# blackle/Megalania

Hardware: NVIDIA B200
Metric: neighbour_cost_evals_per_sec (higher is better)
Workload: dtype u16 probabilities / u64 cost (integer)

## Files before the change

### include/megalania_cuda.h

```cpp
#ifndef MEGALANIA_CUDA_H
#define MEGALANIA_CUDA_H

#include <stddef.h>
#include <stdint.h>

#include "output_interface.h"

#if defined(__GNUC__)
#define MG_API __attribute__((visibility("default")))
#else
#define MG_API
#endif

#ifdef __cplusplus
extern "C" {
#endif


#ifndef MG_HAVE_LZMA_PACKET
#define MG_HAVE_LZMA_PACKET
#define INVALID 0
#define LITERAL 1
#define MATCH 2
#define SHORT_REP 3
// ... 34 lines not shown


MG_API int mg_ctx_create(const uint8_t* data, size_t n, LZMAProperties props, int device, mg_ctx** out);
MG_API void mg_ctx_destroy(mg_ctx* ctx);
MG_API size_t mg_ctx_size(const mg_ctx* ctx);
MG_API int mg_ctx_device(const mg_ctx* ctx);
MG_API int mg_ctx_set_finder_limits(mg_ctx* ctx, size_t window, uint32_t max_occurrences);
MG_API uint32_t mg_ctx_full_wave(const mg_ctx* ctx);
MG_API uint32_t mg_ctx_sm_clock_khz(const mg_ctx* ctx);


MG_API int mg_score_slabs(mg_ctx* ctx, const LZMAPacket* slabs, size_t nslabs, uint64_t* out_cost);


MG_API int mg_find_topk(mg_ctx* ctx, const LZMAPacket* slab, int state_mode, const uint64_t* positions,
                 size_t npos, int k, LZMAPacket* out_pops, uint32_t* out_prices, int32_t* out_counts);

MG_API int mg_find_topk_stats(const mg_ctx* ctx, double* kernel_ms, uint64_t* candidates);


MG_API int mg_encode_slab(mg_ctx* ctx, const LZMAPacket* slab, OutputInterface* out);
MG_API int mg_encode_slab_buffer(mg_ctx* ctx, const LZMAPacket* slab, uint8_t* out, size_t cap, size_t* out_len);
MG_API int mg_encode_stats(const mg_ctx* ctx, double* kernel_ms, uint64_t* events);


MG_API int mg_decode_stream(mg_ctx* ctx, const uint8_t* stream, size_t len, LZMAPacket* out_slab);
MG_API int mg_decode_stats(const mg_ctx* ctx, double* kernel_ms, uint64_t* events);


enum {
	MG_SCHEDULE_REFERENCE = 0,
	MG_SCHEDULE_TEMPERATURE = 1
};

typedef struct {
	uint32_t chains;
	uint32_t top_k;
	uint32_t checkpoint_stride;
	uint32_t edit_log_capacity;
	uint32_t track_best;
	uint32_t trace_capacity;
	uint64_t seed;
} mg_anneal_params;

typedef struct {
	uint32_t evals;
	uint32_t max_attempts;
	uint32_t schedule;
	uint32_t step;
	uint32_t num_iters;
	uint32_t first_eval;
	const float* temperatures;
	uint64_t packet_budget;
	uint32_t no_early_exit;
	uint32_t suspend;
	uint64_t cycle_budget;
	const uint32_t* regions;
} mg_anneal_run_params;
#define MG_CONTINUE_EVALS 0xffffffffu

typedef struct {
	uint64_t evals;
	uint64_t attempts;
	uint64_t accepted;
	uint64_t new_best;
	uint64_t packets_scored;
	uint64_t bits_scored;
	uint64_t slab_bytes_read;
	uint64_t checkpoint_bytes;
	uint64_t finder_calls;
	uint64_t finder_candidates;
	uint64_t edits;
	uint64_t log_overflows;
	uint64_t rejoined;
	uint64_t finder_cycles;
	uint64_t chain_cycles;
	uint64_t finder_chunks;
	uint64_t max_chain_cycles;
	uint64_t finder_gave_up;
	double kernel_ms;
	uint32_t launches;
} mg_anneal_stats;

typedef struct {
	uint64_t cost;
	uint32_t flags;
	uint32_t undo_count;
} mg_trace_rec;

MG_API int mg_anneal_create(mg_ctx* ctx, const mg_anneal_params* params, mg_anneal** out);
MG_API void mg_anneal_destroy(mg_anneal* an);
MG_API size_t mg_anneal_chain_bytes(const mg_ctx* ctx, const mg_anneal_params* params);

MG_API int mg_anneal_set_slab(mg_anneal* an, uint32_t first, uint32_t count, const LZMAPacket* slab,
                       int adopt_cost, int reset_best);

MG_API int mg_anneal_greedy_init(mg_anneal* an, uint32_t nregions, uint32_t dst_chain, uint64_t* cost_out);

MG_API int mg_anneal_optimal_init(mg_anneal* an, uint32_t nregions, uint32_t max_occ, uint32_t dst_chain,
                                  uint64_t* cost_out);
MG_API int mg_optimal_stats(const mg_ctx* ctx, double* kernel_ms, uint64_t* nodes);

MG_API int mg_anneal_merge_regions(mg_anneal* an, uint32_t nregions, const uint32_t* bounds, const uint32_t* owners,
                                   uint32_t dst_chain, uint64_t* cost_out);
#define MG_NO_OWNER 0xffffffffu
MG_API int mg_anneal_merge_export(mg_anneal* an, uint32_t nregions, const uint32_t* bounds, const uint32_t* owners,
                                  void* dev_slab, void* dev_abs);
MG_API int mg_anneal_merge_import(mg_anneal* an, const void* dev_slab, const void* dev_abs, uint32_t dst_chain,
                                  uint64_t* cost_out);
MG_API int mg_anneal_broadcast_chain(mg_anneal* an, uint32_t src_chain);

MG_API int mg_anneal_run(mg_anneal* an, const mg_anneal_run_params* run, mg_anneal_stats* stats);

MG_API int mg_anneal_costs(mg_anneal* an, uint64_t* cur_cost, uint64_t* best_cost);
MG_API int mg_anneal_get_slab(mg_anneal* an, uint32_t chain, int which, LZMAPacket* out_slab);
MG_API int mg_anneal_get_trace(mg_anneal* an, uint32_t chain, mg_trace_rec* out, size_t cap, size_t* count);
MG_API int mg_anneal_swap_chains(mg_anneal* an, uint32_t a, uint32_t b);
MG_API int mg_anneal_device_slab(mg_anneal* an, uint32_t chain, int which, void** dev_ptr, size_t* bytes);
MG_API int mg_anneal_export_slab(mg_anneal* an, uint32_t chain, int which, void* dev_dst);
MG_API int mg_anneal_import_slab(mg_anneal* an, uint32_t chain, const void* dev_src, int adopt_cost);
MG_API int mg_anneal_refresh_chain(mg_anneal* an, uint32_t chain, int adopt_cost);

MG_API int mg_anneal_oneshot(mg_ctx* ctx, const mg_anneal_params* params, const mg_anneal_run_params* run,
                      const LZMAPacket* init, LZMAPacket* best_slab_out, uint64_t* best_cost,
                      mg_anneal_stats* stats);


#define MG_COMM_ID_BYTES 128
MG_API int mg_comm_unique_id(void* id_out);
MG_API int mg_comm_init(mg_ctx* ctx, int rank, int nranks, const void* nccl_id);
MG_API void mg_comm_destroy(mg_ctx* ctx);
MG_API int mg_comm_rank(const mg_ctx* ctx);
MG_API int mg_comm_size(const mg_ctx* ctx);
MG_API int mg_comm_exchange_best(mg_anneal* an, int* winner_rank, uint64_t* best_cost, uint32_t* chain_out);
MG_API int mg_comm_temper_exchange(mg_anneal* an, float* temps, uint32_t round_index, uint64_t seed);
MG_API int mg_temper_decide(const uint64_t* costs, const float* temps, size_t count, uint32_t round_index,
                            uint64_t seed, float* out_temps);
MG_API int mg_comm_merge_regions(mg_anneal* an, uint32_t nregions, const uint32_t* bounds, const uint32_t* owners,
                                 uint32_t dst_chain, uint64_t* cost_out);
MG_API int mg_comm_broadcast_chain(mg_anneal* an, int root, uint32_t src_chain, uint32_t dst_chain);
MG_API int mg_comm_allgather_u64(mg_ctx* ctx, uint64_t value, uint64_t* out);
MG_API int mg_comm_stats(const mg_ctx* ctx, uint64_t* exchanges, uint64_t* installs_by_copy, uint64_t* installs_by_rescore);


typedef struct {
	uint16_t probs[2615];
	uint8_t ctx_state;
	uint32_t dists[4];
	uint64_t position;
	uint64_t cost;
} mg_model_dump;
MG_API int mg_debug_model_after_prefix(mg_ctx* ctx, const LZMAPacket* slab, size_t stop, mg_model_dump* out);
MG_API int mg_debug_index(mg_ctx* ctx, uint32_t* occ_start, uint32_t* occ);

#ifdef __cplusplus
}
#endif
#endif
```

### megalania_b200/api.py

```python
from __future__ import annotations

import ctypes as C
import os

import numpy as np

from . import build as _build

PACKET_DTYPE = np.dtype({"names": ["type", "dist", "len"], "formats": ["u1", "<u4", "<u2"],
                         "offsets": [0, 4, 8], "itemsize": 12})
TRACE_DTYPE = np.dtype([("cost", "<u8"), ("flags", "<u4"), ("undo_count", "<u4")])
MODEL_DTYPE = np.dtype({"names": ["probs", "ctx_state", "dists", "position", "cost"],
                        "formats": [("<u2", 2615), "u1", ("<u4", 4), "<u8", "<u8"],
                        "offsets": [0, 5230, 5232, 5248, 5256], "itemsize": 5264})
INVALID, LITERAL, MATCH, SHORT_REP, LONG_REP = 0, 1, 2, 3, 4
SCHEDULE_REFERENCE, SCHEDULE_TEMPERATURE = 0, 1
CONTINUE_EVALS = 0xFFFFFFFF
NO_OWNER = 0xFFFFFFFF

ERRORS = {-1: "MG_EINVAL", -2: "MG_ECUDA", -3: "MG_ENOMEM", -4: "MG_ESLAB", -5: "MG_EOUTPUT", -6: "MG_ESTATE"}


class MegalaniaError(RuntimeError):
    def __init__(self, code: int, message: str):
        super().__init__(f"{ERRORS.get(code, code)}: {message}")
        self.code = code


class LZMAProperties(C.Structure):
    _fields_ = [("lc", C.c_uint8), ("lp", C.c_uint8), ("pb", C.c_uint8)]


class AnnealParams(C.Structure):
    _fields_ = [("chains", C.c_uint32), ("top_k", C.c_uint32), ("checkpoint_stride", C.c_uint32),
                ("edit_log_capacity", C.c_uint32), ("track_best", C.c_uint32), ("trace_capacity", C.c_uint32),
                ("seed", C.c_uint64)]


class AnnealRunParams(C.Structure):
    _fields_ = [("evals", C.c_uint32), ("max_attempts", C.c_uint32), ("schedule", C.c_uint32),
                ("step", C.c_uint32), ("num_iters", C.c_uint32), ("first_eval", C.c_uint32),
                ("temperatures", C.POINTER(C.c_float)), ("packet_budget", C.c_uint64), ("no_early_exit", C.c_uint32),
                ("suspend", C.c_uint32), ("cycle_budget", C.c_uint64), ("regions", C.POINTER(C.c_uint32))]


class AnnealStats(C.Structure):
    _fields_ = [(name, C.c_uint64) for name in (
        "evals", "attempts", "accepted", "new_best", "packets_scored", "bits_scored", "slab_bytes_read",
        "checkpoint_bytes", "finder_calls", "finder_candidates", "edits", "log_overflows", "rejoined", "finder_cycles", "chain_cycles",
        "finder_chunks", "max_chain_cycles", "finder_gave_up")] + [
        ("kernel_ms", C.c_double), ("launches", C.c_uint32)]

    def as_dict(self) -> dict:
        return {name: getattr(self, name) for name, _ in self._fields_}


WRITE_FN = C.CFUNCTYPE(C.c_bool, C.c_void_p, C.c_void_p, C.c_size_t)


class OutputInterface(C.Structure):
    _fields_ = [("write", WRITE_FN), ("private_data", C.c_void_p)]


EXPORTS = [
    "mg_last_error", "mg_version", "mg_ctx_create", "mg_ctx_destroy", "mg_ctx_size", "mg_ctx_device",
    "mg_score_slabs", "mg_find_topk", "mg_encode_slab", "mg_encode_slab_buffer", "mg_anneal_create",
    "mg_anneal_destroy", "mg_anneal_chain_bytes", "mg_anneal_set_slab", "mg_anneal_run", "mg_anneal_costs",
    "mg_anneal_get_slab", "mg_anneal_get_trace", "mg_anneal_swap_chains", "mg_anneal_device_slab",
    "mg_anneal_refresh_chain", "mg_anneal_oneshot", "mg_debug_model_after_prefix", "mg_anneal_export_slab",
    "mg_anneal_import_slab", "mg_anneal_merge_regions", "mg_anneal_broadcast_chain", "mg_find_topk_stats",
    "mg_anneal_merge_export", "mg_anneal_merge_import", "mg_debug_index", "mg_encode_stats", "mg_ctx_full_wave", "mg_ctx_sm_clock_khz",
    "mg_comm_unique_id", "mg_comm_init", "mg_comm_destroy", "mg_comm_rank", "mg_comm_size", "mg_comm_exchange_best",
    "mg_comm_temper_exchange", "mg_temper_decide", "mg_comm_merge_regions", "mg_comm_stats", "mg_pool_trim",
    "mg_comm_broadcast_chain", "mg_comm_allgather_u64", "mg_ctx_set_finder_limits", "mg_anneal_greedy_init",
    "mg_decode_stream", "mg_decode_stats", "mg_anneal_optimal_init", "mg_optimal_stats",
]

_lib = None


def library_path() -> str:
    return os.environ.get("MEGALANIA_CUDA_LIB") or _build.LIB


def load_library(build_if_missing: bool = True) -> C.CDLL:
    global _lib
    if _lib is not None:
        return _lib
    path = library_path()
    if not os.path.exists(path):
        if not build_if_missing:
            raise MegalaniaError(-2, f"{path} is missing: run `python -m megalania_b200.build`")
        _build.build_library()
    L = C.CDLL(path)
    vp, sz, u32, u64, i32 = C.c_void_p, C.c_size_t, C.c_uint32, C.c_uint64, C.c_int
    L.mg_last_error.restype = C.c_char_p
    L.mg_version.restype = u32
    L.mg_ctx_create.argtypes = [vp, sz, LZMAProperties, i32, C.POINTER(vp)]
    L.mg_ctx_destroy.argtypes = [vp]
    L.mg_ctx_destroy.restype = None
    L.mg_ctx_size.argtypes = [vp]
    L.mg_ctx_size.restype = sz
    L.mg_ctx_device.argtypes = [vp]
    L.mg_ctx_set_finder_limits.argtypes = [vp, sz, u32]
    L.mg_ctx_full_wave.argtypes = [vp]
    L.mg_ctx_full_wave.restype = u32
    L.mg_ctx_sm_clock_khz.argtypes = [vp]
    L.mg_ctx_sm_clock_khz.restype = u32
    L.mg_score_slabs.argtypes = [vp, vp, sz, vp]
    L.mg_find_topk.argtypes = [vp, vp, i32, vp, sz, i32, vp, vp, vp]
    L.mg_find_topk_stats.argtypes = [vp, C.POINTER(C.c_double), C.POINTER(u64)]
    L.mg_encode_slab.argtypes = [vp, vp, C.POINTER(OutputInterface)]
    L.mg_encode_slab_buffer.argtypes = [vp, vp, vp, sz, C.POINTER(sz)]
    L.mg_anneal_create.argtypes = [vp, C.POINTER(AnnealParams), C.POINTER(vp)]
    L.mg_anneal_destroy.argtypes = [vp]
    L.mg_anneal_destroy.restype = None
    L.mg_anneal_chain_bytes.argtypes = [vp, C.POINTER(AnnealParams)]
    L.mg_anneal_chain_bytes.restype = sz
    L.mg_anneal_set_slab.argtypes = [vp, u32, u32, vp, i32, i32]
    L.mg_anneal_run.argtypes = [vp, C.POINTER(AnnealRunParams), C.POINTER(AnnealStats)]
    L.mg_anneal_costs.argtypes = [vp, vp, vp]
    L.mg_anneal_get_slab.argtypes = [vp, u32, i32, vp]
    L.mg_anneal_get_trace.argtypes = [vp, u32, vp, sz, C.POINTER(sz)]
    L.mg_anneal_swap_chains.argtypes = [vp, u32, u32]
    L.mg_anneal_device_slab.argtypes = [vp, u32, i32, C.POINTER(vp), C.POINTER(sz)]
    L.mg_anneal_refresh_chain.argtypes = [vp, u32, i32]
    L.mg_anneal_merge_regions.argtypes = [vp, u32, vp, vp, u32, C.POINTER(u64)]
    L.mg_anneal_broadcast_chain.argtypes = [vp, u32]
    L.mg_anneal_greedy_init.argtypes = [vp, u32, u32, C.POINTER(u64)]
    L.mg_anneal_merge_export.argtypes = [vp, u32, vp, vp, vp, vp]
    L.mg_anneal_merge_import.argtypes = [vp, vp, vp, u32, C.POINTER(u64)]
    L.mg_anneal_export_slab.argtypes = [vp, u32, i32, vp]
    L.mg_anneal_import_slab.argtypes = [vp, u32, vp, i32]
    L.mg_anneal_oneshot.argtypes = [vp, C.POINTER(AnnealParams), C.POINTER(AnnealRunParams), vp, vp,
                                    C.POINTER(u64), C.POINTER(AnnealStats)]
    L.mg_debug_model_after_prefix.argtypes = [vp, vp, sz, vp]
    L.mg_debug_index.argtypes = [vp, vp, vp]
    L.mg_pool_trim.restype = None
    L.mg_comm_unique_id.argtypes = [vp]
    L.mg_comm_init.argtypes = [vp, i32, i32, vp]
    L.mg_comm_destroy.argtypes = [vp]
    L.mg_comm_destroy.restype = None
    L.mg_comm_rank.argtypes = [vp]
    L.mg_comm_size.argtypes = [vp]
    L.mg_comm_exchange_best.argtypes = [vp, C.POINTER(i32), C.POINTER(u64), C.POINTER(u32)]
    L.mg_comm_temper_exchange.argtypes = [vp, vp, u32, u64]
    L.mg_temper_decide.argtypes = [vp, vp, sz, u32, u64, vp]
    L.mg_comm_merge_regions.argtypes = [vp, u32, vp, vp, u32, C.POINTER(u64)]
    L.mg_comm_stats.argtypes = [vp, C.POINTER(u64), C.POINTER(u64), C.POINTER(u64)]
    L.mg_comm_broadcast_chain.argtypes = [vp, i32, u32, u32]
    L.mg_comm_allgather_u64.argtypes = [vp, u64, vp]
    L.mg_encode_stats.argtypes = [vp, C.POINTER(C.c_double), C.POINTER(u64)]
    L.mg_decode_stream.argtypes = [vp, vp, sz, vp]
    L.mg_decode_stats.argtypes = [vp, C.POINTER(C.c_double), C.POINTER(u64)]
    L.mg_anneal_optimal_init.argtypes = [vp, u32, u32, u32, C.POINTER(u64)]
    L.mg_optimal_stats.argtypes = [vp, C.POINTER(C.c_double), C.POINTER(u64)]
    _lib = L
    return L


def _check(rc: int) -> None:
    if rc != 0:
        raise MegalaniaError(rc, load_library().mg_last_error().decode(errors="replace"))


def literal_slab(n: int) -> np.ndarray:
    slab = np.zeros(n, dtype=PACKET_DTYPE)
    slab["type"] = LITERAL
    slab["len"] = 1
    return slab


def as_slab(slab: np.ndarray) -> np.ndarray:
    if slab.dtype == PACKET_DTYPE and slab.flags["C_CONTIGUOUS"]:
        return slab
    out = np.zeros(slab.shape, dtype=PACKET_DTYPE)
    for name in ("type", "dist", "len"):
        out[name] = slab[name]
    return out


def _slab_ptr(slab: np.ndarray, n: int, count: int = 1):
    if slab.dtype != PACKET_DTYPE or not slab.flags["C_CONTIGUOUS"] or slab.size != n * count:
        raise ValueError(f"slab must be a contiguous PACKET_DTYPE array of {n * count} packets")
    return slab.ctypes.data_as(C.c_void_p)


class Context:

    def __init__(self, data: bytes, device: int = 0):
        self._lib = load_library()
        self._data = np.ascontiguousarray(np.frombuffer(bytes(data), dtype=np.uint8))
        self.n = int(self._data.size)
        self._h = C.c_void_p()
        self._children = []
        _check(self._lib.mg_ctx_create(self._data.ctypes.data_as(C.c_void_p), self.n, LZMAProperties(0, 0, 0),
                                       device, C.byref(self._h)))

    def close(self) -> None:
        if getattr(self, "_h", None):
            for ref in self._children:
                child = ref()
                if child is not None:
                    child.close()
            self._children = []
            self._lib.mg_ctx_destroy(self._h)
            self._h = None

    def __del__(self):
        try:
            self.close()
        except Exception:
            pass

    def __enter__(self):
        return self

    def __exit__(self, *exc):
        self.close()

    def score_slabs(self, slabs: np.ndarray) -> np.ndarray:
        slabs = as_slab(np.asarray(slabs))
        count = slabs.size // self.n
        out = np.zeros(count, dtype=np.uint64)
        _check(self._lib.mg_score_slabs(self._h, _slab_ptr(slabs.reshape(-1), self.n, count), count,
                                        out.ctypes.data_as(C.c_void_p)))
        return out

    def score_slab(self, slab: np.ndarray) -> int:
        return int(self.score_slabs(slab)[0])

    def find_topk(self, slab: np.ndarray, positions, state_mode: int = 0, k: int = 20):
        pos = np.ascontiguousarray(positions, dtype=np.uint64)
        slab = as_slab(slab)
        pops = np.zeros((pos.size, k), dtype=PACKET_DTYPE)
        prices = np.zeros((pos.size, k), dtype=np.uint32)
        counts = np.zeros(pos.size, dtype=np.int32)
        _check(self._lib.mg_find_topk(self._h, _slab_ptr(slab, self.n), state_mode, pos.ctypes.data_as(C.c_void_p),
                                      pos.size, k, pops.ctypes.data_as(C.c_void_p),
                                      prices.ctypes.data_as(C.c_void_p), counts.ctypes.data_as(C.c_void_p)))
        return pops, prices, counts

    def find_topk_stats(self) -> dict:
        ms, cand = C.c_double(0), C.c_uint64(0)
        _check(self._lib.mg_find_topk_stats(self._h, C.byref(ms), C.byref(cand)))
        return {"kernel_ms": ms.value, "candidates": int(cand.value)}

    def encode_slab(self, slab: np.ndarray) -> bytes:
        chunks: list[bytes] = []

        def _write(_iface, ptr, size):
            chunks.append(C.string_at(ptr, size))
            return True

        iface = OutputInterface(WRITE_FN(_write), None)
        _check(self._lib.mg_encode_slab(self._h, _slab_ptr(slab, self.n), C.byref(iface)))
        return b"".join(chunks)

    def encode_stats(self) -> dict:
        ms, ev = C.c_double(0), C.c_uint64(0)
        _check(self._lib.mg_encode_stats(self._h, C.byref(ms), C.byref(ev)))
        return {"kernel_ms": ms.value, "events": int(ev.value)}

    def encode_slab_buffer(self, slab: np.ndarray) -> bytes:
        cap = self.n * 2 + 8192
        out = np.zeros(cap, dtype=np.uint8)
        got = C.c_size_t(0)
        _check(self._lib.mg_encode_slab_buffer(self._h, _slab_ptr(slab, self.n), out.ctypes.data_as(C.c_void_p), cap,
                                               C.byref(got)))
        return out[:got.value].tobytes()

    def decode_stream(self, stream: bytes) -> np.ndarray:
        buf = np.ascontiguousarray(np.frombuffer(bytes(stream), dtype=np.uint8))
        out = np.zeros(self.n, dtype=PACKET_DTYPE)
        _check(self._lib.mg_decode_stream(self._h, buf.ctypes.data_as(C.c_void_p), buf.size,
                                          out.ctypes.data_as(C.c_void_p)))
        return out

    def decode_stats(self) -> dict:
        ms, ev = C.c_double(0), C.c_uint64(0)
        _check(self._lib.mg_decode_stats(self._h, C.byref(ms), C.byref(ev)))
        return {"kernel_ms": ms.value, "events": int(ev.value)}

    def optimal_stats(self) -> dict:
        ms, nodes = C.c_double(0), C.c_uint64(0)
        _check(self._lib.mg_optimal_stats(self._h, C.byref(ms), C.byref(nodes)))
        return {"kernel_ms": ms.value, "nodes": int(nodes.value)}

    def model_after_prefix(self, slab: np.ndarray, stop: int):
        out = np.zeros(1, dtype=MODEL_DTYPE)
        _check(self._lib.mg_debug_model_after_prefix(self._h, _slab_ptr(slab, self.n), stop,
                                                     out.ctypes.data_as(C.c_void_p)))
        return out[0]

    @staticmethod
    def comm_unique_id() -> bytes:
        buf = C.create_string_buffer(128)
        _check(load_library().mg_comm_unique_id(buf))
        return buf.raw

    def comm_init(self, rank: int, nranks: int, unique_id: bytes) -> None:
        if len(unique_id) != 128:
            raise ValueError("an NCCL unique id is 128 bytes")
        _check(self._lib.mg_comm_init(self._h, rank, nranks, C.c_char_p(unique_id)))

    def comm_allgather(self, value: int) -> np.ndarray:
        size = int(self._lib.mg_comm_size(self._h))
        out = np.zeros(size, dtype=np.uint64)
        _check(self._lib.mg_comm_allgather_u64(self._h, int(value), out.ctypes.data_as(C.c_void_p)))
        return out

    def comm_stats(self) -> dict:
        a, b, c = C.c_uint64(0), C.c_uint64(0), C.c_uint64(0)
        _check(self._lib.mg_comm_stats(self._h, C.byref(a), C.byref(b), C.byref(c)))
        return {"exchanges": int(a.value), "installs_by_copy": int(b.value), "installs_by_rescore": int(c.value)}

    def set_finder_limits(self, window: int = 0, max_occurrences: int = 0) -> None:
        _check(self._lib.mg_ctx_set_finder_limits(self._h, window, max_occurrences))

    def full_wave(self) -> int:
        return int(self._lib.mg_ctx_full_wave(self._h))

    def sm_clock_khz(self) -> int:
        return int(self._lib.mg_ctx_sm_clock_khz(self._h))

    def bigram_index(self):
        start = np.zeros(65537, dtype=np.uint32)
        occ = np.zeros(max(1, self.n - 1), dtype=np.uint32)
        _check(self._lib.mg_debug_index(self._h, start.ctypes.data_as(C.c_void_p), occ.ctypes.data_as(C.c_void_p)))
        return start, occ[:max(0, self.n - 1)]

    def chain_bytes(self, **params) -> int:
        p = AnnealParams(**params)
        return int(self._lib.mg_anneal_chain_bytes(self._h, C.byref(p)))


class Annealer:

    def __init__(self, ctx: Context, chains: int, *, top_k: int = 20, checkpoint_stride: int = 0,
                 edit_log_capacity: int = 0, track_best: bool = True, trace_capacity: int = 0, seed: int = 1673551):
        self.ctx = ctx
        self._lib = ctx._lib
        self.chains = chains
        self.params = AnnealParams(chains, top_k, checkpoint_stride, edit_log_capacity, int(track_best),
                                   trace_capacity, seed)
        self._h = C.c_void_p()
        _check(self._lib.mg_anneal_create(ctx._h, C.byref(self.params), C.byref(self._h)))
        import weakref
        ctx._children.append(weakref.ref(self))

    def close(self) -> None:
        if getattr(self, "_h", None):
            self._lib.mg_anneal_destroy(self._h)
            self._h = None

    def __del__(self):
        try:
            self.close()
        except Exception:
            pass

    def set_slab(self, slab: np.ndarray | None = None, first: int = 0, count: int | None = None,
                 adopt_cost: bool | None = None, reset_best: bool = True) -> None:
        if count is None:
            count = self.chains - first
        if adopt_cost is None:
            adopt_cost = slab is not None
        ptr = _slab_ptr(slab, self.ctx.n) if slab is not None else None
        _check(self._lib.mg_anneal_set_slab(self._h, first, count, ptr, int(adopt_cost), int(reset_best)))

    def run(self, evals: int, *, schedule: int = SCHEDULE_REFERENCE, step: int = 0, num_iters: int = 0,
            first_eval: int = 0, max_attempts: int = 0, temperatures=None, packet_budget: int = 0,
            early_exit: bool = True, suspend: bool = False, cycle_budget: int = 0, regions=None) -> dict:
        temps = None
        tptr = None
        if temperatures is not None:
            temps = np.ascontiguousarray(temperatures, dtype=np.float32)
            if temps.size != self.chains:
                raise ValueError("one temperature per chain")
            tptr = temps.ctypes.data_as(C.POINTER(C.c_float))
        rptr = None
        if regions is not None:
            regs = np.ascontiguousarray(regions, dtype=np.uint32)
            if regs.shape != (self.chains, 2):
                raise ValueError("regions must be a [chains][2] array of byte ranges")
            rptr = regs.ctypes.data_as(C.POINTER(C.c_uint32))
        rp = AnnealRunParams(evals, max_attempts, schedule, step, num_iters, first_eval, tptr, packet_budget,
                             0 if early_exit else 1, int(suspend), cycle_budget, rptr)
        st = AnnealStats()
        _check(self._lib.mg_anneal_run(self._h, C.byref(rp), C.byref(st)))
        return st.as_dict()

    def costs(self):
        cur = np.zeros(self.chains, dtype=np.uint64)
        best = np.zeros(self.chains, dtype=np.uint64)
        _check(self._lib.mg_anneal_costs(self._h, cur.ctypes.data_as(C.c_void_p), best.ctypes.data_as(C.c_void_p)))
        return cur, best

    def get_slab(self, chain: int, best: bool = False) -> np.ndarray:
        out = np.zeros(self.ctx.n, dtype=PACKET_DTYPE)
        _check(self._lib.mg_anneal_get_slab(self._h, chain, int(best), out.ctypes.data_as(C.c_void_p)))
        return out

    def trace(self, chain: int) -> np.ndarray:
        cap = self.params.trace_capacity
        out = np.zeros(cap, dtype=TRACE_DTYPE)
        count = C.c_size_t(0)
        _check(self._lib.mg_anneal_get_trace(self._h, chain, out.ctypes.data_as(C.c_void_p), cap, C.byref(count)))
        return out[:min(cap, count.value)]

    def swap_chains(self, a: int, b: int) -> None:
        _check(self._lib.mg_anneal_swap_chains(self._h, a, b))

    def device_slab(self, chain: int, best: bool = False):
        ptr, size = C.c_void_p(), C.c_size_t()
        _check(self._lib.mg_anneal_device_slab(self._h, chain, int(best), C.byref(ptr), C.byref(size)))
        return ptr.value, size.value

    def export_slab(self, chain: int, best: bool, device_ptr: int) -> None:
        _check(self._lib.mg_anneal_export_slab(self._h, chain, int(best), C.c_void_p(device_ptr)))

    def import_slab(self, chain: int, device_ptr: int, adopt_cost: bool = True) -> None:
        _check(self._lib.mg_anneal_import_slab(self._h, chain, C.c_void_p(device_ptr), int(adopt_cost)))

    def merge_regions(self, bounds, owners, dst_chain: int = 0) -> int:
        b = np.ascontiguousarray(bounds, dtype=np.uint32)
        o = np.ascontiguousarray(owners, dtype=np.uint32)
        if b.size != o.size + 1:
            raise ValueError("bounds must hold one more entry than owners")
        cost = C.c_uint64(0)
        _check(self._lib.mg_anneal_merge_regions(self._h, o.size, b.ctypes.data_as(C.c_void_p), o.ctypes.data_as(C.c_void_p),
                                                 dst_chain, C.byref(cost)))
        return int(cost.value)

    def merge_export(self, bounds, owners, dev_slab_ptr: int, dev_abs_ptr: int) -> None:
        b = np.ascontiguousarray(bounds, dtype=np.uint32)
        o = np.ascontiguousarray(owners, dtype=np.uint32)
        if b.size != o.size + 1:
            raise ValueError("bounds must hold one more entry than owners")
        _check(self._lib.mg_anneal_merge_export(self._h, o.size, b.ctypes.data_as(C.c_void_p), o.ctypes.data_as(C.c_void_p),
                                                C.c_void_p(dev_slab_ptr), C.c_void_p(dev_abs_ptr)))

    def merge_import(self, dev_slab_ptr: int, dev_abs_ptr: int, dst_chain: int = 0) -> int:
        cost = C.c_uint64(0)
        _check(self._lib.mg_anneal_merge_import(self._h, C.c_void_p(dev_slab_ptr), C.c_void_p(dev_abs_ptr), dst_chain,
                                                C.byref(cost)))
        return int(cost.value)

    def comm_exchange_best(self):
        w, c, ch = C.c_int(-1), C.c_uint64(0), C.c_uint32(0)
        _check(self._lib.mg_comm_exchange_best(self._h, C.byref(w), C.byref(c), C.byref(ch)))
        return int(w.value), int(c.value), int(ch.value)

    def comm_broadcast_chain(self, root: int, src_chain: int, dst_chain: int) -> None:
        _check(self._lib.mg_comm_broadcast_chain(self._h, root, src_chain, dst_chain))

    def comm_temper_exchange(self, temps: np.ndarray, round_index: int, seed: int = 0) -> np.ndarray:
        t = np.ascontiguousarray(temps, dtype=np.float32).copy()
        if t.size != self.chains:
            raise ValueError("one temperature per chain")
        _check(self._lib.mg_comm_temper_exchange(self._h, t.ctypes.data_as(C.c_void_p), round_index, seed))
        return t

    def comm_merge_regions(self, bounds, owners, dst_chain: int = 0) -> int:
        b = np.ascontiguousarray(bounds, dtype=np.uint32)
        o = np.ascontiguousarray(owners, dtype=np.uint32)
        cost = C.c_uint64(0)
        _check(self._lib.mg_comm_merge_regions(self._h, o.size, b.ctypes.data_as(C.c_void_p), o.ctypes.data_as(C.c_void_p),
                                               dst_chain, C.byref(cost)))
        return int(cost.value)

    def broadcast_chain(self, src_chain: int) -> None:
        _check(self._lib.mg_anneal_broadcast_chain(self._h, src_chain))

    def greedy_init(self, nregions: int = 1, dst_chain: int = 0) -> int:
        cost = C.c_uint64(0)
        _check(self._lib.mg_anneal_greedy_init(self._h, nregions, dst_chain, C.byref(cost)))
        return int(cost.value)

    def optimal_init(self, nregions: int = 1, max_occ: int = 0, dst_chain: int = 0) -> int:
        cost = C.c_uint64(0)
        _check(self._lib.mg_anneal_optimal_init(self._h, nregions, max_occ, dst_chain, C.byref(cost)))
        return int(cost.value)

# ... 27 lines not shown
```

### megalania_b200/csrc/mg_api.cu

```cuda
#include <cmath>
#include <cstdarg>
#include <cstdio>
#include <cstdlib>
#include <cstring>
#include <algorithm>
#include <new>
#include <vector>
#include <unistd.h>

#include "../../include/megalania_cuda.h"
#include "mg_kernels.cuh"

using namespace mg;

static thread_local char g_err[512] = "";

static int fail(int code, const char* fmt, ...)
{
	va_list ap;
	va_start(ap, fmt);
	vsnprintf(g_err, sizeof(g_err), fmt, ap);
	va_end(ap);
	return code;
}

#define CU(call)                                                                                   \
	do {                                                                                           \
		cudaError_t e_ = (call);                                                                   \
		if (e_ != cudaSuccess)                                                                     \
			return fail(e_ == cudaErrorMemoryAllocation ? MG_ENOMEM : MG_ECUDA, "%s: %s", #call,   \
			            cudaGetErrorString(e_));                                                   \
	} while (0)

extern "C" MG_API const char* mg_last_error(void) { return g_err; }
#include <map>
#include <mutex>
#include <unordered_map>
namespace {
struct DevicePool {
	std::mutex lock;
	std::unordered_map<void*, std::pair<int, size_t>> live;
	std::multimap<std::pair<int, size_t>, void*> cached;
};
DevicePool& pool()
{
	static DevicePool* p = new DevicePool;
	return *p;
}
void pool_release_device(int device)
{
	DevicePool& P = pool();
	for (auto it = P.cached.begin(); it != P.cached.end();) {
		if (device < 0 || it->first.first == device) {
			cudaFree(it->second);
			it = P.cached.erase(it);
		} else {
			++it;
		}
	}
}
}

static cudaError_t pool_malloc_raw(void** out, size_t bytes)
{
	if (bytes == 0) bytes = 16;
	int device = 0;
	cudaError_t e = cudaGetDevice(&device);
	if (e != cudaSuccess) return e;
	DevicePool& P = pool();
	std::lock_guard<std::mutex> g(P.lock);
	auto hit = P.cached.find({device, bytes});
	if (hit != P.cached.end()) {
		*out = hit->second;
		P.cached.erase(hit);
	} else {
		e = cudaMalloc(out, bytes);
		if (e == cudaErrorMemoryAllocation) {
			cudaGetLastError();
			pool_release_device(device);
			e = cudaMalloc(out, bytes);
		}
		if (e != cudaSuccess) return e;
	}
	P.live[*out] = {device, bytes};
	return cudaSuccess;
}
template <class T> static cudaError_t pool_malloc(T** out, size_t bytes) { return pool_malloc_raw(reinterpret_cast<void**>(out), bytes); }

static void pool_free(void* p)
{
	if (!p) return;
	DevicePool& P = pool();
	std::lock_guard<std::mutex> g(P.lock);
	auto it = P.live.find(p);
	if (it == P.live.end()) {
		cudaFree(p);
		return;
	}
	P.cached.insert({it->second, p});
	P.live.erase(it);
}

extern "C" MG_API void mg_pool_trim(void)
{
	DevicePool& P = pool();
	std::lock_guard<std::mutex> g(P.lock);
	int device = 0;
	cudaGetDevice(&device);
	for (auto it = P.cached.begin(); it != P.cached.end();) {
		cudaSetDevice(it->first.first);
		cudaFree(it->second);
		it = P.cached.erase(it);
	}
	cudaSetDevice(device);
}

extern "C" MG_API uint32_t mg_version(void) { return (0u << 16) | 3u; }

struct mg_comm_state;

struct mg_ctx {
	mg_comm_state* comm = nullptr;
	int device = 0;
	uint32_t n = 0;
	cudaStream_t stream = nullptr;
	uint8_t* d_data = nullptr;
	uint32_t* d_occ_start = nullptr;
	uint32_t* d_occ = nullptr;
	uint32_t* d_trans = nullptr;
	uint32_t* d_recip = nullptr;
	uint4* d_litq = nullptr;
	Tables tables{};
	int sm_count = 0;
	double index_ms = 0;
	std::vector<mg_anneal*> annealers;
	double last_topk_ms = 0;
	unsigned long long last_topk_candidates = 0;
	FindLimits limits{0, 0};
	double last_encode_ms = 0;
	unsigned long long last_encode_events = 0;
	double last_decode_ms = 0;
	unsigned long long last_decode_events = 0;
	double last_optimal_ms = 0;
	unsigned long long last_optimal_nodes = 0;
};

struct DevBuf {
	void* p = nullptr;
	~DevBuf() { if (p) pool_free(p); }
	template <class T> T* as() { return static_cast<T*>(p); }
};

static int dev_alloc(DevBuf& b, size_t bytes)
{
	CU(pool_malloc(&b.p, bytes ? bytes : 16));
	return 0;
}

static int grid_for(size_t items, int threads, int cap)
{
	size_t g = (items + threads - 1) / threads;
	if (g > (size_t)cap) g = cap;
	return g ? (int)g : 1;
}

static int set_smem_attrs()
{
	CU(cudaFuncSetAttribute(score_kernel, cudaFuncAttributeMaxDynamicSharedMemorySize, (int)sizeof(CtaShared)));
	CU(cudaFuncSetAttribute(topk_kernel, cudaFuncAttributeMaxDynamicSharedMemorySize, (int)sizeof(CtaShared)));
	CU(cudaFuncSetAttribute(anneal_kernel, cudaFuncAttributeMaxDynamicSharedMemorySize, (int)sizeof(CtaShared)));
	CU(cudaFuncSetAttribute(greedy_kernel, cudaFuncAttributeMaxDynamicSharedMemorySize, (int)sizeof(CtaShared)));
	CU(cudaFuncSetAttribute(encode_kernel, cudaFuncAttributeMaxDynamicSharedMemorySize, (int)sizeof(EncodeShared)));
	CU(cudaFuncSetAttribute(score_kernel, cudaFuncAttributePreferredSharedMemoryCarveout, cudaSharedmemCarveoutMaxShared));
	CU(cudaFuncSetAttribute(topk_kernel, cudaFuncAttributePreferredSharedMemoryCarveout, cudaSharedmemCarveoutMaxShared));
	CU(cudaFuncSetAttribute(anneal_kernel, cudaFuncAttributePreferredSharedMemoryCarveout, cudaSharedmemCarveoutMaxShared));
	CU(cudaFuncSetAttribute(greedy_kernel, cudaFuncAttributePreferredSharedMemoryCarveout, cudaSharedmemCarveoutMaxShared));
	return 0;
}

static int build_index(mg_ctx* ctx)
{
	const uint32_t n = ctx->n;
	CU(pool_malloc(&ctx->d_occ_start, sizeof(uint32_t) * (INDEX_KEYS + 1)));
	CU(pool_malloc(&ctx->d_occ, sizeof(uint32_t) * (size_t)(n ? n : 1)));
	if (n < 2) {
		CU(cudaMemsetAsync(ctx->d_occ_start, 0, sizeof(uint32_t) * (INDEX_KEYS + 1), ctx->stream));
		return 0;
	}
	const uint32_t total = n - 1;
	uint32_t nwarps = 256;
	uint32_t per_warp = (total + nwarps - 1) / nwarps;
	per_warp = (per_warp + 31) & ~31u;
	if (per_warp < 32) per_warp = 32;
	nwarps = (total + per_warp - 1) / per_warp;
	DevBuf rows, totals;
	if (int rc = dev_alloc(rows, sizeof(uint32_t) * (size_t)nwarps * INDEX_KEYS)) return rc;
	if (int rc = dev_alloc(totals, sizeof(uint32_t) * INDEX_KEYS)) return rc;
	cudaEvent_t e0, e1;
	CU(cudaEventCreate(&e0));
	CU(cudaEventCreate(&e1));
	CU(cudaEventRecord(e0, ctx->stream));
	CU(cudaMemsetAsync(rows.p, 0, sizeof(uint32_t) * (size_t)nwarps * INDEX_KEYS, ctx->stream));
	const int threads = 128;
	const int blocks = (int)((nwarps * 32 + threads - 1) / threads);
	index_count_kernel<<<blocks, threads, 0, ctx->stream>>>(ctx->d_data, n, rows.as<uint32_t>(), per_warp);
	index_prefix_kernel<<<INDEX_KEYS / 256, 256, 0, ctx->stream>>>(rows.as<uint32_t>(), nwarps, totals.as<uint32_t>());
	index_scan_kernel<<<1, 1024, 0, ctx->stream>>>(totals.as<uint32_t>(), ctx->d_occ_start);
	index_scatter_kernel<<<blocks, threads, 0, ctx->stream>>>(ctx->d_data, n, rows.as<uint32_t>(), per_warp,
	                                                          ctx->d_occ_start, ctx->d_occ);
	CU(cudaEventRecord(e1, ctx->stream));
	CU(cudaStreamSynchronize(ctx->stream));
	CU(cudaGetLastError());
	float ms = 0;
	cudaEventElapsedTime(&ms, e0, e1);
	ctx->index_ms = ms;
	cudaEventDestroy(e0);
	cudaEventDestroy(e1);
	return 0;
}

extern "C" MG_API int mg_ctx_create(const uint8_t* data, size_t n, LZMAProperties props, int device, mg_ctx** out)
{
	if (!data || !out || n == 0) return fail(MG_EINVAL, "mg_ctx_create: data, out and a non-zero size are required");
	if (props.lc || props.lp || props.pb) return fail(MG_EINVAL, "only lc = lp = pb = 0 is supported (as in the reference)");
	if (n >= 0x7fffff00ull) return fail(MG_EINVAL, "inputs of 2 GiB and more are not supported");
	int count = 0;
	cudaError_t probe = cudaErrorUnknown;
	for (int attempt = 0; attempt < 5; attempt++) {
		probe = cudaGetDeviceCount(&count);
		if (probe == cudaSuccess && count > 0) break;
		if (probe == cudaErrorNoDevice || probe == cudaErrorInsufficientDriver) break;
		cudaGetLastError();
		usleep(200 * 1000);
	}
	if (probe != cudaSuccess || count == 0)
		return fail(MG_ECUDA, "no CUDA device available (this library has no CPU path): %s", cudaGetErrorString(probe));
	if (device < 0 || device >= count) return fail(MG_EINVAL, "device %d out of range (%d devices)", device, count);
	CU(cudaSetDevice(device));
	mg_ctx* ctx = new (std::nothrow) mg_ctx;
	if (!ctx) return fail(MG_ENOMEM, "out of host memory");
	ctx->device = device;
	ctx->n = (uint32_t)n;
	cudaDeviceProp prop;
	CU(cudaGetDeviceProperties(&prop, device));
	ctx->sm_count = prop.multiProcessorCount;
	int rc = 0;
	do {
		if ((rc = set_smem_attrs())) break;
#define CUB(call)                                                                 \
	if (cudaError_t e_ = (call); e_ != cudaSuccess) {                             \
		rc = fail(MG_ECUDA, "%s: %s", #call, cudaGetErrorString(e_));             \
		break;                                                                    \
	}
		CUB(cudaStreamCreateWithFlags(&ctx->stream, cudaStreamNonBlocking));
		CUB(pool_malloc(&ctx->d_data, n + 32));
		CUB(cudaMemsetAsync(ctx->d_data + n, 0, 32, ctx->stream));
		CUB(cudaMemcpyAsync(ctx->d_data, data, n, cudaMemcpyHostToDevice, ctx->stream));
		std::vector<uint32_t> price(2048);
		price[0] = 0;
		for (int i = 1; i < 2048; i++) price[i] = (uint32_t)(-(long)(std::log2((double)i / 2048.0) * 2048.0));
		auto step = [&](uint32_t p, uint32_t bit, uint32_t& cost) {
			cost += bit ? price[(2048u - p) & 2047u] : price[p];
			return bit ? p - (p >> 5) : p + ((2048u - p) >> 5);
		};
		std::vector<uint32_t> trans(TRANS_WORDS, 0);
		for (uint32_t p = 1; p < 2048; p++) {
			for (uint32_t bit = 0; bit < 2; bit++) {
				uint32_t cost = 0;
				const uint32_t p1 = step(p, bit, cost);
				trans[bit * 2048 + p] = (p1 << PROB_SHIFT) | (cost << 16);
			}
			for (uint32_t ab = 0; ab < 4; ab++) {
				uint32_t cost = 0;
				const uint32_t p2 = step(step(p, ab >> 1, cost), ab & 1, cost);
				trans[(2 + ab) * 2048 + p] = (p2 << PROB_SHIFT) | (cost << 16);
			}
		}
		std::vector<uint32_t> recip(RECIP_ENTRIES, 0);
		for (uint32_t i = 1; i < RECIP_ENTRIES; i++) recip[i] = 0xffffffffu / i + 1u;
		CUB(pool_malloc(&ctx->d_trans, TRANS_WORDS * sizeof(uint32_t)));
		CUB(pool_malloc(&ctx->d_recip, RECIP_ENTRIES * sizeof(uint32_t)));
		CUB(cudaMemcpyAsync(ctx->d_trans, trans.data(), TRANS_WORDS * sizeof(uint32_t), cudaMemcpyHostToDevice, ctx->stream));
		CUB(cudaMemcpyAsync(ctx->d_recip, recip.data(), RECIP_ENTRIES * sizeof(uint32_t), cudaMemcpyHostToDevice, ctx->stream));
		const uint32_t nwin = (uint32_t)(n / 32);
		if (nwin != 0 && !getenv("MEGALANIA_NO_LITQ")) {
			CUB(pool_malloc(&ctx->d_litq, (size_t)nwin * QUEUE_BLOCKS * 32 * sizeof(uint4)));
			litq_build_kernel<<<(nwin + 7) / 8, 256, 0, ctx->stream>>>(ctx->d_data, (uint32_t)n, nwin, ctx->d_litq);
			CUB(cudaGetLastError());
		}
		CUB(cudaStreamSynchronize(ctx->stream));
		ctx->tables.trans = ctx->d_trans;
		ctx->tables.litq = ctx->d_litq;
		ctx->tables.recip = ctx->d_recip;
		rc = build_index(ctx);
#undef CUB
	} while (0);
	if (rc) {
		mg_ctx_destroy(ctx);
		return rc;
	}
	*out = ctx;
	return MG_OK;
}

extern "C" MG_API void mg_ctx_destroy(mg_ctx* ctx)
{
	if (!ctx) return;
	cudaSetDevice(ctx->device);
	mg_comm_destroy(ctx);
	while (!ctx->annealers.empty()) mg_anneal_destroy(ctx->annealers.back());
	if (ctx->stream) cudaStreamSynchronize(ctx->stream);
	pool_free(ctx->d_data);
	pool_free(ctx->d_occ_start);
	pool_free(ctx->d_occ);
	pool_free(ctx->d_trans);
	pool_free(ctx->d_recip);
	pool_free(ctx->d_litq);
	if (ctx->stream) cudaStreamDestroy(ctx->stream);
	delete ctx;
}

extern "C" MG_API size_t mg_ctx_size(const mg_ctx* ctx) { return ctx ? ctx->n : 0; }
extern "C" MG_API int mg_find_topk_stats(const mg_ctx* ctx, double* kernel_ms, uint64_t* candidates)
{
	if (!ctx) return fail(MG_EINVAL, "mg_find_topk_stats: null context");
	if (kernel_ms) *kernel_ms = ctx->last_topk_ms;
	if (candidates) *candidates = ctx->last_topk_candidates;
	return MG_OK;
}
extern "C" MG_API int mg_ctx_device(const mg_ctx* ctx) { return ctx ? ctx->device : -1; }
extern "C" MG_API int mg_ctx_set_finder_limits(mg_ctx* ctx, size_t window, uint32_t max_occurrences)
{
	if (!ctx) return fail(MG_EINVAL, "mg_ctx_set_finder_limits: null context");
	ctx->limits.window = window > 0xffffffffull ? 0xffffffffu : (uint32_t)window;
	ctx->limits.max_occ = max_occurrences;
	return MG_OK;
}
extern "C" MG_API uint32_t mg_ctx_full_wave(const mg_ctx* ctx) { return ctx ? (uint32_t)ctx->sm_count * (uint32_t)WARPS_PER_CTA : 0u; }
extern "C" MG_API uint32_t mg_ctx_sm_clock_khz(const mg_ctx* ctx)
{
	int khz = 0;
	if (!ctx || cudaDeviceGetAttribute(&khz, cudaDevAttrClockRate, ctx->device) != cudaSuccess || khz <= 0) return 0u;
	return (uint32_t)khz;
}
extern "C" MG_API int mg_encode_stats(const mg_ctx* ctx, double* kernel_ms, uint64_t* events)
{
	if (!ctx) return fail(MG_EINVAL, "mg_encode_stats: null context");
	if (kernel_ms) *kernel_ms = ctx->last_encode_ms;
	if (events) *events = ctx->last_encode_events;
	return MG_OK;
}

extern "C" MG_API int mg_debug_index(mg_ctx* ctx, uint32_t* occ_start, uint32_t* occ)
{
	if (!ctx || !occ_start || !occ) return fail(MG_EINVAL, "mg_debug_index: null argument");
	CU(cudaSetDevice(ctx->device));
	CU(cudaMemcpyAsync(occ_start, ctx->d_occ_start, sizeof(uint32_t) * (INDEX_KEYS + 1), cudaMemcpyDeviceToHost, ctx->stream));
	if (ctx->n > 1) CU(cudaMemcpyAsync(occ, ctx->d_occ, sizeof(uint32_t) * (size_t)(ctx->n - 1), cudaMemcpyDeviceToHost, ctx->stream));
	CU(cudaStreamSynchronize(ctx->stream));
	return MG_OK;
}

static int upload_packed(mg_ctx* ctx, const LZMAPacket* host, size_t count, uint64_t* dst)
{
	static_assert(sizeof(LZMAPacket) == 12, "LZMAPacket must keep the reference layout");
	const size_t chunk = (size_t)8 << 20;
	DevBuf raw;
	const size_t stage = count < chunk ? count : chunk;
	if (int rc = dev_alloc(raw, stage * 12)) return rc;
	for (size_t off = 0; off < count; off += stage) {
		const size_t c = count - off < stage ? count - off : stage;
		CU(cudaMemcpyAsync(raw.p, host + off, c * 12, cudaMemcpyHostToDevice, ctx->stream));
		pack_kernel<<<grid_for(c, 256, ctx->sm_count * 8), 256, 0, ctx->stream>>>(raw.as<uint32_t>(), dst + off, c);
		CU(cudaStreamSynchronize(ctx->stream));
	}
	CU(cudaGetLastError());
	return 0;
}

static int download_unpacked(mg_ctx* ctx, const uint64_t* src, size_t count, LZMAPacket* host)
{
	DevBuf raw;
	if (int rc = dev_alloc(raw, count * 12)) return rc;
	unpack_kernel<<<grid_for(count, 256, ctx->sm_count * 8), 256, 0, ctx->stream>>>(src, raw.as<uint32_t>(), count);
	CU(cudaGetLastError());
	CU(cudaMemcpyAsync(host, raw.p, count * 12, cudaMemcpyDeviceToHost, ctx->stream));
	CU(cudaStreamSynchronize(ctx->stream));
	return 0;
}

static const char* walk_error(uint32_t err)
{
	if (err & ERR_BAD_PACKET) return "slab holds a packet that cannot be coded at its position";
	if (err & ERR_NOT_BOUNDARY) return "position is not a live packet boundary of the slab";
	if (err & ERR_OUTPUT_FULL) return "output buffer too small";
	return "unknown";
}

static uint32_t default_stride(uint32_t n)
{
	uint32_t s = n / 256;
	if (s < 512) s = 512;
	return (s + 31) & ~31u;
}

static int score_device(mg_ctx* ctx, const uint64_t* d_slabs, uint32_t nslabs, uint32_t stop_pos, uint64_t* d_cost,
                        uint32_t* d_count, uint32_t* d_err, Record* ck, uint32_t* ck_pos, CkMeta* ck_meta,
                        uint32_t stride, uint32_t nslots, Record* final_model)
{
	ScoreArgs a;
	a.data = ctx->d_data;
	a.n = ctx->n;
	a.slabs = d_slabs;
	a.nslabs = nslabs;
	a.stop_pos = stop_pos;
	a.out_cost = d_cost;
	a.out_count = d_count;
	a.out_err = d_err;
	a.ck = ck;
	a.ck_pos = ck_pos;
	a.ck_meta = ck_meta;
	a.stride = stride;
	a.nslots = nslots ? nslots : 1;
	a.ck_chain_stride = a.nslots - 1;
	a.final_model = final_model;
	a.tables = ctx->tables;
	const int blocks = (int)((nslabs + WARPS_PER_CTA - 1) / WARPS_PER_CTA);
	score_kernel<<<blocks, CTA_THREADS, sizeof(CtaShared), ctx->stream>>>(a);
	CU(cudaGetLastError());
	return 0;
}

extern "C" MG_API int mg_score_slabs(mg_ctx* ctx, const LZMAPacket* slabs, size_t nslabs, uint64_t* out_cost)
{
	if (!ctx || !slabs || !out_cost) return fail(MG_EINVAL, "mg_score_slabs: null argument");
	if (nslabs == 0) return MG_OK;
	CU(cudaSetDevice(ctx->device));
	const size_t n = ctx->n;
	size_t batch = ((size_t)2 << 30) / (n * 8);
	if (batch < 1) batch = 1;
	if (batch > nslabs) batch = nslabs;
	DevBuf packed, cost, err;
	if (int rc = dev_alloc(packed, batch * n * 8)) return rc;
	if (int rc = dev_alloc(cost, batch * 8)) return rc;
	if (int rc = dev_alloc(err, batch * 4)) return rc;
	std::vector<uint32_t> herr(batch);
	for (size_t off = 0; off < nslabs; off += batch) {
		const size_t c = nslabs - off < batch ? nslabs - off : batch;
		if (int rc = upload_packed(ctx, slabs + off * n, c * n, packed.as<uint64_t>())) return rc;
		if (int rc = score_device(ctx, packed.as<uint64_t>(), (uint32_t)c, ctx->n, cost.as<uint64_t>(), nullptr,
		                          err.as<uint32_t>(), nullptr, nullptr, nullptr, default_stride(ctx->n), 1, nullptr))
			return rc;
		CU(cudaMemcpyAsync(out_cost + off, cost.p, c * 8, cudaMemcpyDeviceToHost, ctx->stream));
		CU(cudaMemcpyAsync(herr.data(), err.p, c * 4, cudaMemcpyDeviceToHost, ctx->stream));
		CU(cudaStreamSynchronize(ctx->stream));
		for (size_t i = 0; i < c; i++)
			if (herr[i]) return fail(MG_ESLAB, "slab %zu: %s", off + i, walk_error(herr[i]));
	}
	return MG_OK;
}

static void export_model(const Record& r, mg_model_dump* out)
{
	for (int i = 0; i < 2615; i++) out->probs[i] = 1024;
	auto put = [&](uint32_t ref_index, uint32_t slot) { out->probs[ref_index] = (uint16_t)(r.probs[slot] >> PROB_SHIFT); };
	for (uint32_t node = 0; node < 768; node++)
		if (node & 0xff) put(node, lit_slot(node));
	const uint32_t ref_len[2] = {768, 768 + 514};
	const uint32_t dev_len[2] = {S_LEN, S_REPLEN};
	for (int t = 0; t < 2; t++) {
		put(ref_len[t] + 0, dev_len[t] + 0);
		put(ref_len[t] + 1, dev_len[t] + 1);
		for (uint32_t i = 0; i < 8; i++) {
			put(ref_len[t] + 2 + i, dev_len[t] + LEN_LOW + i);
			put(ref_len[t] + 2 + 128 + i, dev_len[t] + LEN_MID + i);
		}
		for (uint32_t i = 0; i < 256; i++) put(ref_len[t] + 2 + 256 + i, dev_len[t] + LEN_HIGH + i);
	}
	const uint32_t ref_dist = 768 + 2 * 514;
	for (uint32_t i = 0; i < 256 + 16 + 115; i++) put(ref_dist + i, S_POSSLOT + i);
	const uint32_t ref_ctx = ref_dist + 387;
	for (uint32_t s = 0; s < 12; s++) {
		put(ref_ctx + (s << 4), S_ISMATCH + s);
		put(ref_ctx + 192 + s, S_ISREP + s);
		put(ref_ctx + 204 + s, S_ISREPG0 + s);
		put(ref_ctx + 216 + s, S_ISREPG1 + s);
		put(ref_ctx + 228 + s, S_ISREPG2 + s);
		put(ref_ctx + 240 + (s << 4), S_ISREP0LONG + s);
	}
	out->ctx_state = (uint8_t)r.ctx;
	for (int i = 0; i < 4; i++) out->dists[i] = r.rep[i];
	out->position = r.pos;
	out->cost = r.cost;
}

extern "C" MG_API int mg_debug_model_after_prefix(mg_ctx* ctx, const LZMAPacket* slab, size_t stop, mg_model_dump* out)
{
	if (!ctx || !slab || !out || stop > ctx->n) return fail(MG_EINVAL, "mg_debug_model_after_prefix: bad argument");
	CU(cudaSetDevice(ctx->device));
	DevBuf packed, cost, err, model;
	if (int rc = dev_alloc(packed, (size_t)ctx->n * 8)) return rc;
	if (int rc = dev_alloc(cost, 8)) return rc;
	if (int rc = dev_alloc(err, 4)) return rc;
	if (int rc = dev_alloc(model, sizeof(Record))) return rc;
	if (int rc = upload_packed(ctx, slab, ctx->n, packed.as<uint64_t>())) return rc;
	if (int rc = score_device(ctx, packed.as<uint64_t>(), 1, (uint32_t)stop, cost.as<uint64_t>(), nullptr, err.as<uint32_t>(),
	                          nullptr, nullptr, nullptr, default_stride(ctx->n), 1, model.as<Record>()))
		return rc;
	Record r;
	uint32_t herr = 0;
	CU(cudaMemcpyAsync(&r, model.p, sizeof(Record), cudaMemcpyDeviceToHost, ctx->stream));
	CU(cudaMemcpyAsync(&herr, err.p, 4, cudaMemcpyDeviceToHost, ctx->stream));
	CU(cudaStreamSynchronize(ctx->stream));
	if (herr) return fail(MG_ESLAB, "%s", walk_error(herr));
	memset(out, 0, sizeof(*out));
	export_model(r, out);
	return MG_OK;
}

extern "C" MG_API int mg_find_topk(mg_ctx* ctx, const LZMAPacket* slab, int state_mode, const uint64_t* positions,
                            size_t npos, int k, LZMAPacket* out_pops, uint32_t* out_prices, int32_t* out_counts)
{
	if (!ctx || !slab || !positions || !out_pops || !out_counts) return fail(MG_EINVAL, "mg_find_topk: null argument");
	if (k < 1 || k > MAX_K) return fail(MG_EINVAL, "mg_find_topk: k must be in 1..%d", MAX_K);
	if (state_mode != 0 && state_mode != 1) return fail(MG_EINVAL, "mg_find_topk: state_mode must be 0 or 1");
	if (npos == 0) return MG_OK;
	if (npos > 0xffffffffull / (size_t)k) return fail(MG_EINVAL, "mg_find_topk: too many queries");
	CU(cudaSetDevice(ctx->device));
	const uint32_t n = ctx->n;
	std::vector<uint32_t> pos32(npos);
	for (size_t i = 0; i < npos; i++) {
		if (positions[i] >= n) return fail(MG_EINVAL, "mg_find_topk: position %llu outside the input", (unsigned long long)positions[i]);
		pos32[i] = (uint32_t)positions[i];
	}
	const uint32_t stride = default_stride(n);
	const uint32_t nslots = (n + stride - 1) / stride;
	DevBuf packed, dpos, opk, oprice, ocount, oerr, cost, serr, ck, ckpos, cand;
	if (int rc = dev_alloc(packed, (size_t)n * 8)) return rc;
	if (int rc = dev_alloc(dpos, npos * 4)) return rc;
	if (int rc = dev_alloc(opk, npos * k * 8)) return rc;
	if (int rc = dev_alloc(oprice, npos * k * 4)) return rc;
	if (int rc = dev_alloc(ocount, npos * 4)) return rc;
	if (int rc = dev_alloc(oerr, npos * 4)) return rc;
	if (int rc = dev_alloc(cand, 8)) return rc;
	if (int rc = upload_packed(ctx, slab, n, packed.as<uint64_t>())) return rc;
	CU(cudaMemcpyAsync(dpos.p, pos32.data(), npos * 4, cudaMemcpyHostToDevice, ctx->stream));
	CU(cudaMemsetAsync(cand.p, 0, 8, ctx->stream));
	if (state_mode == 1) {
		if (int rc = dev_alloc(cost, 8)) return rc;
		if (int rc = dev_alloc(serr, 4)) return rc;
		if (int rc = dev_alloc(ck, sizeof(Record) * (size_t)nslots)) return rc;
		if (int rc = dev_alloc(ckpos, 4 * (size_t)nslots)) return rc;
		if (int rc = score_device(ctx, packed.as<uint64_t>(), 1, n, cost.as<uint64_t>(), nullptr, serr.as<uint32_t>(),
		                          ck.as<Record>(), ckpos.as<uint32_t>(), nullptr, stride, nslots, nullptr))
			return rc;
		uint32_t herr = 0;
		CU(cudaMemcpyAsync(&herr, serr.p, 4, cudaMemcpyDeviceToHost, ctx->stream));
		CU(cudaStreamSynchronize(ctx->stream));
		if (herr) return fail(MG_ESLAB, "mg_find_topk: %s", walk_error(herr));
	}
	TopkArgs a;
	a.data = ctx->d_data;
	a.n = n;
	a.occ_start = ctx->d_occ_start;
	a.occ = ctx->d_occ;
	a.slab = packed.as<uint64_t>();
	a.state_mode = state_mode;
	a.positions = dpos.as<uint32_t>();
	a.npos = (uint32_t)npos;
	a.k = (uint32_t)k;
	a.ck = ck.as<Record>();
	a.ck_pos = ckpos.as<uint32_t>();
	a.nslots = nslots;
	a.stride = stride;
	a.out_pk = opk.as<uint64_t>();
	a.out_price = oprice.as<uint32_t>();
	a.out_count = ocount.as<int32_t>();
	a.out_err = oerr.as<uint32_t>();
	a.candidates = cand.as<unsigned long long>();
	a.limits = ctx->limits;
	a.tables = ctx->tables;
	size_t blocks = (npos + WARPS_PER_CTA - 1) / WARPS_PER_CTA;
	const size_t cap = (size_t)ctx->sm_count * 4 * 8;
	if (blocks > cap) blocks = cap;
	cudaEvent_t t0, t1;
	CU(cudaEventCreate(&t0));
	CU(cudaEventCreate(&t1));
	CU(cudaEventRecord(t0, ctx->stream));
	topk_kernel<<<(int)blocks, CTA_THREADS, sizeof(CtaShared), ctx->stream>>>(a);
	CU(cudaEventRecord(t1, ctx->stream));
	CU(cudaGetLastError());
	std::vector<uint64_t> hpk(npos * k);
	std::vector<uint32_t> hprice(npos * k), herr(npos);
	CU(cudaMemcpyAsync(hpk.data(), opk.p, npos * k * 8, cudaMemcpyDeviceToHost, ctx->stream));
	CU(cudaMemcpyAsync(hprice.data(), oprice.p, npos * k * 4, cudaMemcpyDeviceToHost, ctx->stream));
	CU(cudaMemcpyAsync(out_counts, ocount.p, npos * 4, cudaMemcpyDeviceToHost, ctx->stream));
	CU(cudaMemcpyAsync(herr.data(), oerr.p, npos * 4, cudaMemcpyDeviceToHost, ctx->stream));
	CU(cudaMemcpyAsync(&ctx->last_topk_candidates, cand.p, 8, cudaMemcpyDeviceToHost, ctx->stream));
	CU(cudaStreamSynchronize(ctx->stream));
	{
		float ms = 0;
		cudaEventElapsedTime(&ms, t0, t1);
		ctx->last_topk_ms = ms;
		cudaEventDestroy(t0);
		cudaEventDestroy(t1);
	}
	for (size_t q = 0; q < npos; q++) {
		if (herr[q]) return fail(MG_ESLAB, "mg_find_topk: query %zu (position %u): %s", q, pos32[q], walk_error(herr[q]));
		for (int i = 0; i < k; i++) {
			LZMAPacket p;
			memset(&p, 0, sizeof(p));
			uint32_t price = 0;
			if (i < out_counts[q]) {
				const uint64_t v = hpk[q * k + i];
				p.type = (uint8_t)pk_type(v);
				p.dist = pk_dist(v);
				p.len = (uint16_t)pk_len(v);
				price = hprice[q * k + i];
			}
			out_pops[q * k + i] = p;
			if (out_prices) out_prices[q * k + i] = price;
		}
	}
	return MG_OK;
}

static int encode_to_host(mg_ctx* ctx, const LZMAPacket* slab, std::vector<uint8_t>& payload)
{
	const uint32_t n = ctx->n;
	const uint32_t cap = n + n / 2 + 4096;
	DevBuf packed, out, len, err;
	if (int rc = dev_alloc(packed, (size_t)n * 8)) return rc;
	if (int rc = dev_alloc(out, cap)) return rc;
	if (int rc = dev_alloc(len, 32)) return rc;
	if (int rc = dev_alloc(err, 4)) return rc;
	if (int rc = upload_packed(ctx, slab, n, packed.as<uint64_t>())) return rc;
	EncodeArgs a;
	a.data = ctx->d_data;
	a.n = n;
	a.slab = packed.as<uint64_t>();
	a.out = out.as<uint8_t>();
	a.cap = cap;
	a.out_len = len.as<uint32_t>();
	a.out_err = err.as<uint32_t>();
	a.out_events = len.as<uint32_t>() + 1;
	const bool debug_wait = getenv("MEGALANIA_ENCODE_DEBUG") != nullptr;
	a.out_wait = debug_wait ? reinterpret_cast<unsigned long long*>(len.as<uint32_t>() + 2) : nullptr;
	a.tables = ctx->tables;
	cudaEvent_t t0, t1;
	CU(cudaEventCreate(&t0));
	CU(cudaEventCreate(&t1));
	CU(cudaEventRecord(t0, ctx->stream));
	encode_kernel<<<1, 96, sizeof(EncodeShared), ctx->stream>>>(a);
	CU(cudaEventRecord(t1, ctx->stream));
	CU(cudaGetLastError());
	uint32_t hlen2[8] = {0, 0, 0, 0, 0, 0, 0, 0}, herr = 0;
	CU(cudaMemcpyAsync(hlen2, len.p, 32, cudaMemcpyDeviceToHost, ctx->stream));
	CU(cudaMemcpyAsync(&herr, err.p, 4, cudaMemcpyDeviceToHost, ctx->stream));
	CU(cudaStreamSynchronize(ctx->stream));
	{
		float ms = 0;
		cudaEventElapsedTime(&ms, t0, t1);
		ctx->last_encode_ms = ms;
		ctx->last_encode_events = hlen2[1];
		if (debug_wait) {
			unsigned long long w[3];
			memcpy(w, hlen2 + 2, sizeof(w));
			fprintf(stderr, "mg_encode_slab: %.2f ms, %u events; clocks waiting: producer %llu, range %llu, low %llu\n", ms, hlen2[1], w[0], w[1], w[2]);
		}
		cudaEventDestroy(t0);
		cudaEventDestroy(t1);
	}
	const uint32_t hlen = hlen2[0];
	if (herr) return fail(MG_ESLAB, "mg_encode_slab: %s", walk_error(herr));
	payload.resize(hlen);
	CU(cudaMemcpyAsync(payload.data(), out.p, hlen, cudaMemcpyDeviceToHost, ctx->stream));
	CU(cudaStreamSynchronize(ctx->stream));
	return 0;
}

static void make_header(const mg_ctx* ctx, uint8_t hdr[13])
{
	hdr[0] = 0;
	uint32_t dict = 0x400000;
	while (dict < ctx->n && dict < 0x80000000u) dict <<= 1;
	for (int i = 0; i < 4; i++) hdr[1 + i] = (uint8_t)(dict >> (8 * i));
	const uint64_t size = ctx->n;
	for (int i = 0; i < 8; i++) hdr[5 + i] = (uint8_t)(size >> (8 * i));
}

extern "C" MG_API int mg_encode_slab(mg_ctx* ctx, const LZMAPacket* slab, OutputInterface* out)
{
	if (!ctx || !slab || !out || !out->write) return fail(MG_EINVAL, "mg_encode_slab: null argument");
	CU(cudaSetDevice(ctx->device));
	std::vector<uint8_t> payload;
	if (int rc = encode_to_host(ctx, slab, payload)) return rc;
	uint8_t hdr[13];
	make_header(ctx, hdr);
	bool ok = out->write(out, hdr, 1) && out->write(out, hdr + 1, 4) && out->write(out, hdr + 5, 8);
	if (ok && !payload.empty()) ok = out->write(out, payload.data(), payload.size());
	if (!ok) return fail(MG_EOUTPUT, "mg_encode_slab: OutputInterface.write failed");
	return MG_OK;
}

extern "C" MG_API int mg_encode_slab_buffer(mg_ctx* ctx, const LZMAPacket* slab, uint8_t* out, size_t cap, size_t* out_len)
{
	if (!ctx || !slab || !out_len || (!out && cap)) return fail(MG_EINVAL, "mg_encode_slab_buffer: null argument");
	CU(cudaSetDevice(ctx->device));
	std::vector<uint8_t> payload;
	if (int rc = encode_to_host(ctx, slab, payload)) return rc;
	*out_len = 13 + payload.size();
	if (*out_len > cap) return fail(MG_EINVAL, "mg_encode_slab_buffer: need %zu bytes, have %zu", *out_len, cap);
	make_header(ctx, out);
	memcpy(out + 13, payload.data(), payload.size());
	return MG_OK;
}

static const char* decode_error(uint32_t err)
// ... 225 lines not shown
		if (e_ != cudaSuccess) rc = fail(MG_ECUDA, "mg_anneal_create: %s", cudaGetErrorString(e_));
	}
	if (rc) {
		mg_anneal_destroy(an);
		return rc;
	}
	an->have_slab.assign(C, 0);
	ctx->annealers.push_back(an);
	*out = an;
	return MG_OK;
}

static int replicate(mg_ctx* ctx, const void* src, void* dst, size_t bytes, size_t stride_bytes, uint32_t copies)
{
	if (copies == 0 || bytes == 0) return 0;
	const bool aligned = (((uintptr_t)src | (uintptr_t)dst | bytes | stride_bytes) & 15) == 0;
	if (aligned) {
		const size_t words = bytes / 16;
		replicate_kernel<<<grid_for(words, 256, ctx->sm_count * 16), 256, 0, ctx->stream>>>(
		    static_cast<const uint4*>(src), static_cast<uint4*>(dst), words, stride_bytes / 16, copies);
		CU(cudaGetLastError());
		return 0;
	}
	for (uint32_t c = 0; c < copies; c++)
		CU(cudaMemcpyAsync(static_cast<char*>(dst) + (size_t)c * stride_bytes, src, bytes, cudaMemcpyDeviceToDevice, ctx->stream));
	return 0;
}

static int refresh_chains(mg_anneal* an, uint32_t first, uint32_t count, int adopt_cost, int reset_best)
{
	mg_ctx* ctx = an->ctx;
	const size_t n = ctx->n, nck = an->nck;
	CU(cudaMemsetAsync(an->d_bad, 0, 4, ctx->stream));
	for (uint32_t c = first; c < first + count; c++)
		validate_kernel<<<grid_for(n, 256, ctx->sm_count * 4), 256, 0, ctx->stream>>>(an->d_slabs + (size_t)c * n, ctx->n, an->d_bad);
	CU(cudaGetLastError());
	for (uint32_t c = first; c < first + count; c++) {
		ScoreArgs a;
		a.data = ctx->d_data;
		a.n = ctx->n;
		a.slabs = an->d_slabs + (size_t)c * n;
		a.nslabs = 1;
		a.stop_pos = ctx->n;
		a.out_cost = an->d_cost + c;
		a.out_count = an->d_count + c;
		a.out_err = an->d_err + c;
		a.ck = an->d_ck + (size_t)c * 2 * nck;
		a.ck_pos = nullptr;
		a.ck_meta = an->d_ck_meta + (size_t)c * 2 * nck;
		a.stride = an->stride;
		a.nslots = an->nslots;
		a.ck_chain_stride = 0;
		a.final_model = nullptr;
		a.tables = ctx->tables;
		score_kernel<<<1, CTA_THREADS, sizeof(CtaShared), ctx->stream>>>(a);
	}
	CU(cudaGetLastError());
	CU(cudaMemsetAsync(an->d_ck_live + (size_t)first * nck, 0, (size_t)count * nck, ctx->stream));
	std::vector<uint64_t> cost(count);
	std::vector<uint32_t> live(count), err(count);
	uint32_t bad = 0;
	CU(cudaMemcpyAsync(cost.data(), an->d_cost + first, count * 8, cudaMemcpyDeviceToHost, ctx->stream));
	CU(cudaMemcpyAsync(live.data(), an->d_count + first, count * 4, cudaMemcpyDeviceToHost, ctx->stream));
	CU(cudaMemcpyAsync(err.data(), an->d_err + first, count * 4, cudaMemcpyDeviceToHost, ctx->stream));
	CU(cudaMemcpyAsync(&bad, an->d_bad, 4, cudaMemcpyDeviceToHost, ctx->stream));
	std::vector<ChainState> st(count);
	CU(cudaMemcpyAsync(st.data(), an->d_state + first, count * sizeof(ChainState), cudaMemcpyDeviceToHost, ctx->stream));
	CU(cudaStreamSynchronize(ctx->stream));
	if (bad) return fail(MG_ESLAB, "slab holds %u undecodable slot(s)", bad);
	for (uint32_t i = 0; i < count; i++) {
		if (err[i]) return fail(MG_ESLAB, "chain %u: %s", first + i, walk_error(err[i]));
		st[i].cur_cost = adopt_cost ? cost[i] : 0;
		st[i].slab_cost = cost[i];
		st[i].live_count = live[i];
		st[i].err = 0;
		st[i].eval_index = 0;
		st[i].susp_slot = 0;
		st[i].journal_count = 0;
		st[i].journal_overflow = reset_best ? 0 : 1;
		if (reset_best) st[i].best_cost = 0;
	}
	CU(cudaMemcpyAsync(an->d_state + first, st.data(), count * sizeof(ChainState), cudaMemcpyHostToDevice, ctx->stream));
	CU(cudaStreamSynchronize(ctx->stream));
	for (uint32_t i = 0; i < count; i++) an->have_slab[first + i] = 1;
	return 0;
}

extern "C" MG_API int mg_anneal_set_slab(mg_anneal* an, uint32_t first, uint32_t count, const LZMAPacket* slab,
                                  int adopt_cost, int reset_best)
{
	if (!an) return fail(MG_EINVAL, "mg_anneal_set_slab: null handle");
	if (count == 0 || first >= an->p.chains || count > an->p.chains - first)
		return fail(MG_EINVAL, "mg_anneal_set_slab: chain range out of bounds");
	mg_ctx* ctx = an->ctx;
	CU(cudaSetDevice(ctx->device));
	const size_t n = ctx->n;
	uint64_t* dst0 = an->d_slabs + (size_t)first * n;
	if (slab) {
		if (int rc = upload_packed(ctx, slab, n, dst0)) return rc;
	} else {
		fill_literal_kernel<<<grid_for(n, 256, ctx->sm_count * 8), 256, 0, ctx->stream>>>(dst0, n);
		CU(cudaGetLastError());
	}
	if (int rc = replicate(ctx, dst0, dst0 + n, n * 8, n * 8, count - 1)) return rc;
	if (an->d_bests && reset_best)
		if (int rc = replicate(ctx, dst0, an->d_bests + (size_t)first * n, n * 8, n * 8, count)) return rc;
	if (int rc = refresh_chains(an, first, 1, adopt_cost, reset_best)) return rc;
	if (count > 1) {
		const size_t nck = an->nck;
		if (int rc = replicate(ctx, an->d_ck + (size_t)first * 2 * nck, an->d_ck + (size_t)(first + 1) * 2 * nck,
		                       nck * sizeof(Record), 2 * nck * sizeof(Record), count - 1))
			return rc;
		if (int rc = replicate(ctx, an->d_ck_meta + (size_t)first * 2 * nck, an->d_ck_meta + (size_t)(first + 1) * 2 * nck,
		                       nck * sizeof(CkMeta), 2 * nck * sizeof(CkMeta), count - 1))
			return rc;
		CU(cudaMemsetAsync(an->d_ck_live + (size_t)first * nck, 0, (size_t)count * nck, ctx->stream));
		std::vector<ChainState> st(count);
		CU(cudaMemcpyAsync(st.data(), an->d_state + first, count * sizeof(ChainState), cudaMemcpyDeviceToHost, ctx->stream));
		CU(cudaStreamSynchronize(ctx->stream));
		for (uint32_t i = 1; i < count; i++) {
			st[i].cur_cost = st[0].cur_cost;
			st[i].slab_cost = st[0].slab_cost;
			st[i].live_count = st[0].live_count;
			st[i].err = 0;
			st[i].eval_index = 0;
			st[i].susp_slot = 0;
			st[i].journal_count = 0;
			st[i].journal_overflow = reset_best ? 0 : 1;
			if (reset_best) st[i].best_cost = 0;
			an->have_slab[first + i] = 1;
		}
		CU(cudaMemcpyAsync(an->d_state + first, st.data(), count * sizeof(ChainState), cudaMemcpyHostToDevice, ctx->stream));
		CU(cudaStreamSynchronize(ctx->stream));
	}
	return MG_OK;
}

extern "C" MG_API int mg_anneal_refresh_chain(mg_anneal* an, uint32_t chain, int adopt_cost)
{
	if (!an || chain >= an->p.chains) return fail(MG_EINVAL, "mg_anneal_refresh_chain: bad argument");
	CU(cudaSetDevice(an->ctx->device));
	if (int rc = refresh_chains(an, chain, 1, adopt_cost, 0)) return rc;
	return MG_OK;
}

static void anneal_common_args(mg_anneal* an, AnnealArgs& a)
{
	mg_ctx* ctx = an->ctx;
	const uint32_t C = an->p.chains;
	a.data = ctx->d_data;
	a.n = ctx->n;
	a.occ_start = ctx->d_occ_start;
	a.occ = ctx->d_occ;
	a.tables = ctx->tables;
	a.limits = ctx->limits;
	a.chains = C;
	a.k = an->p.top_k;
	a.stride = an->stride;
	a.nslots = an->nck + 1;
	a.log_cap = an->p.edit_log_capacity;
	a.track_best = an->p.track_best && an->d_bests;
	a.slabs = an->d_slabs;
	a.bests = an->d_bests;
	a.ck = an->d_ck;
	a.ck_meta = an->d_ck_meta;
	a.ck_live = an->d_ck_live;
	a.logs = an->d_logs;
	a.journal = an->d_journal;
	a.state = an->d_state;
	a.stats = an->d_stats;
	a.trace = an->d_trace;
	a.trace_cap = an->p.trace_capacity;
	a.attempts_out = an->d_attempts;
	a.regions = nullptr;
	a.abs_dist = nullptr;
	a.chain_first = 0;
	a.repair_only = 0;
	a.suspend = 0;
	a.cycle_budget = 0;
	a.packet_budget = 0;
	a.early_exit = 0;
	a.temps = nullptr;
	a.schedule = 0;
	a.step = 0;
	a.num_iters = ctx->n;
	a.first_eval = 0xffffffffu;
	a.evals = 0;
	a.max_attempts = 0;
	if (an->nslots <= 1) a.nslots = 1;
}

extern "C" MG_API int mg_anneal_run(mg_anneal* an, const mg_anneal_run_params* run, mg_anneal_stats* stats)
{
	if (!an || !run) return fail(MG_EINVAL, "mg_anneal_run: null argument");
	mg_ctx* ctx = an->ctx;
	for (uint8_t h : an->have_slab)
		if (!h) return fail(MG_ESTATE, "mg_anneal_run: every chain needs mg_anneal_set_slab first");
	if (run->schedule > 1) return fail(MG_EINVAL, "mg_anneal_run: unknown schedule");
	if (run->schedule == MG_SCHEDULE_TEMPERATURE && !run->temperatures)
		return fail(MG_EINVAL, "mg_anneal_run: temperatures required");
	CU(cudaSetDevice(ctx->device));
	const uint32_t C = an->p.chains;
	if (run->temperatures) CU(cudaMemcpyAsync(an->d_temps, run->temperatures, (size_t)C * 4, cudaMemcpyHostToDevice, ctx->stream));
	AnnealArgs a;
	anneal_common_args(an, a);
	a.evals = run->evals;
	a.max_attempts = run->max_attempts ? run->max_attempts : run->evals * 64u + 1024u;
	a.schedule = run->schedule;
	a.step = run->step;
	a.num_iters = run->num_iters ? run->num_iters : ctx->n;
	a.first_eval = run->first_eval;
	a.packet_budget = run->packet_budget;
	a.early_exit = run->no_early_exit ? 0u : 1u;
	a.suspend = run->suspend ? 1u : 0u;
	a.cycle_budget = run->cycle_budget;
	a.temps = run->temperatures ? an->d_temps : nullptr;
	if (run->regions) {
		for (uint32_t c = 0; c < C; c++)
			if (run->regions[2 * c] >= run->regions[2 * c + 1] || run->regions[2 * c + 1] > ctx->n)
				return fail(MG_EINVAL, "mg_anneal_run: chain %u has an empty or out-of-range region", c);
		if (!an->d_regions) CU(pool_malloc(&an->d_regions, (size_t)C * 8));
		CU(cudaMemcpyAsync(an->d_regions, run->regions, (size_t)C * 8, cudaMemcpyHostToDevice, ctx->stream));
		a.regions = an->d_regions;
	}
	int blocks = (int)((C + WARPS_PER_CTA - 1) / WARPS_PER_CTA);
	if (blocks < ctx->sm_count) blocks = (int)(C < (uint32_t)ctx->sm_count ? C : (uint32_t)ctx->sm_count);
	CU(cudaEventRecord(an->e0, ctx->stream));
	anneal_kernel<<<blocks, CTA_THREADS, sizeof(CtaShared), ctx->stream>>>(a);
	CU(cudaEventRecord(an->e1, ctx->stream));
	CU(cudaGetLastError());
	CU(cudaStreamSynchronize(ctx->stream));
	float ms = 0;
	CU(cudaEventElapsedTime(&ms, an->e0, an->e1));
	std::vector<ChainStats> cs(C);
	std::vector<ChainState> st(C);
	CU(cudaMemcpy(cs.data(), an->d_stats, (size_t)C * sizeof(ChainStats), cudaMemcpyDeviceToHost));
	CU(cudaMemcpy(st.data(), an->d_state, (size_t)C * sizeof(ChainState), cudaMemcpyDeviceToHost));
	for (uint32_t c = 0; c < C; c++)
		if (st[c].err) return fail(MG_ESLAB, "mg_anneal_run: chain %u stopped: %s", c, walk_error(st[c].err));
	if (stats) {
		memset(stats, 0, sizeof(*stats));
		for (uint32_t c = 0; c < C; c++) {
			stats->evals += cs[c].evals;
			stats->attempts += cs[c].attempts;
			stats->accepted += cs[c].accepted;
			stats->new_best += cs[c].new_best;
			stats->packets_scored += cs[c].packets;
			stats->bits_scored += cs[c].bits;
			stats->slab_bytes_read += cs[c].slab_bytes;
			stats->checkpoint_bytes += cs[c].ck_bytes;
			stats->finder_calls += cs[c].finds;
			stats->finder_candidates += cs[c].candidates;
			stats->edits += cs[c].edits;
			stats->log_overflows += cs[c].overflows;
			stats->rejoined += cs[c].rejoined;
			stats->finder_cycles += cs[c].find_cycles;
			stats->finder_chunks += cs[c].chunks;
			stats->finder_gave_up += cs[c].gave_up;
			stats->chain_cycles += cs[c].chain_cycles;
			if (cs[c].chain_cycles > stats->max_chain_cycles) stats->max_chain_cycles = cs[c].chain_cycles;
		}
		stats->kernel_ms = ms;
		stats->launches = 1;
	}
	return MG_OK;
}

extern "C" MG_API int mg_anneal_costs(mg_anneal* an, uint64_t* cur_cost, uint64_t* best_cost)
{
	if (!an) return fail(MG_EINVAL, "mg_anneal_costs: null handle");
	CU(cudaSetDevice(an->ctx->device));
	const uint32_t C = an->p.chains;
	std::vector<ChainState> st(C);
	CU(cudaStreamSynchronize(an->ctx->stream));
	CU(cudaMemcpy(st.data(), an->d_state, (size_t)C * sizeof(ChainState), cudaMemcpyDeviceToHost));
	for (uint32_t c = 0; c < C; c++) {
		if (cur_cost) cur_cost[c] = st[c].cur_cost;
		if (best_cost) best_cost[c] = st[c].best_cost;
	}
	return MG_OK;
}

extern "C" MG_API int mg_anneal_get_slab(mg_anneal* an, uint32_t chain, int which, LZMAPacket* out_slab)
{
	if (!an || !out_slab || chain >= an->p.chains) return fail(MG_EINVAL, "mg_anneal_get_slab: bad argument");
	if (which == 1 && !an->d_bests) return fail(MG_ESTATE, "mg_anneal_get_slab: chains were created without track_best");
	CU(cudaSetDevice(an->ctx->device));
	const size_t n = an->ctx->n;
	const uint64_t* src = (which == 1 ? an->d_bests : an->d_slabs) + (size_t)chain * n;
	if (int rc = download_unpacked(an->ctx, src, n, out_slab)) return rc;
	return MG_OK;
}

extern "C" MG_API int mg_anneal_get_trace(mg_anneal* an, uint32_t chain, mg_trace_rec* out, size_t cap, size_t* count)
{
	if (!an || chain >= an->p.chains || !count) return fail(MG_EINVAL, "mg_anneal_get_trace: bad argument");
	if (!an->d_trace) return fail(MG_ESTATE, "mg_anneal_get_trace: chains were created without trace_capacity");
	CU(cudaSetDevice(an->ctx->device));
	uint32_t attempts = 0;
	CU(cudaMemcpy(&attempts, an->d_attempts + chain, 4, cudaMemcpyDeviceToHost));
	*count = attempts;
	size_t c = attempts < an->p.trace_capacity ? attempts : an->p.trace_capacity;
	if (c > cap) c = cap;
	static_assert(sizeof(mg_trace_rec) == sizeof(TraceRec), "trace record layout");
	if (c && out)
		CU(cudaMemcpy(out, an->d_trace + (size_t)chain * an->p.trace_capacity, c * sizeof(TraceRec), cudaMemcpyDeviceToHost));
// ... 33 lines not shown

extern "C" MG_API int mg_anneal_swap_chains(mg_anneal* an, uint32_t x, uint32_t y)
{
	if (!an || x >= an->p.chains || y >= an->p.chains) return fail(MG_EINVAL, "mg_anneal_swap_chains: bad argument");
	if (x == y) return MG_OK;
	mg_ctx* ctx = an->ctx;
	CU(cudaSetDevice(ctx->device));
	const size_t n = ctx->n, nck = an->nck;
	DevBuf tmp;
	size_t big = n * 8;
	if (2 * nck * sizeof(Record) > big) big = 2 * nck * sizeof(Record);
	if (int rc = dev_alloc(tmp, big)) return rc;
	auto swap_region = [&](void* pa, void* pb, size_t bytes) -> cudaError_t {
		cudaError_t e = cudaMemcpyAsync(tmp.p, pa, bytes, cudaMemcpyDeviceToDevice, ctx->stream);
		if (e == cudaSuccess) e = cudaMemcpyAsync(pa, pb, bytes, cudaMemcpyDeviceToDevice, ctx->stream);
		if (e == cudaSuccess) e = cudaMemcpyAsync(pb, tmp.p, bytes, cudaMemcpyDeviceToDevice, ctx->stream);
		return e;
	};
	CU(swap_region(an->d_slabs + (size_t)x * n, an->d_slabs + (size_t)y * n, n * 8));
	CU(swap_region(an->d_ck + (size_t)x * 2 * nck, an->d_ck + (size_t)y * 2 * nck, 2 * nck * sizeof(Record)));
	CU(swap_region(an->d_ck_meta + (size_t)x * 2 * nck, an->d_ck_meta + (size_t)y * 2 * nck, 2 * nck * sizeof(CkMeta)));
	CU(swap_region(an->d_ck_live + (size_t)x * nck, an->d_ck_live + (size_t)y * nck, nck));
	ChainState sx, sy;
	CU(cudaStreamSynchronize(ctx->stream));
	CU(cudaMemcpy(&sx, an->d_state + x, sizeof(ChainState), cudaMemcpyDeviceToHost));
	CU(cudaMemcpy(&sy, an->d_state + y, sizeof(ChainState), cudaMemcpyDeviceToHost));
	ChainState nx = sx, ny = sy;
	nx.cur_cost = sy.cur_cost;
	nx.slab_cost = sy.slab_cost;
	nx.live_count = sy.live_count;
	ny.cur_cost = sx.cur_cost;
	ny.slab_cost = sx.slab_cost;
	ny.live_count = sx.live_count;
	nx.journal_count = ny.journal_count = 0;
	nx.susp_slot = ny.susp_slot = 0;
	nx.journal_overflow = ny.journal_overflow = 1;
	CU(cudaMemcpy(an->d_state + x, &nx, sizeof(ChainState), cudaMemcpyHostToDevice));
	CU(cudaMemcpy(an->d_state + y, &ny, sizeof(ChainState), cudaMemcpyHostToDevice));
	return MG_OK;
}

extern "C" MG_API int mg_anneal_merge_export(mg_anneal* an, uint32_t nregions, const uint32_t* bounds, const uint32_t* owners,
                                      void* dev_slab, void* dev_abs)
{
	if (!an || !bounds || !owners || nregions == 0 || !dev_slab || !dev_abs)
		return fail(MG_EINVAL, "mg_anneal_merge_export: bad argument");
	mg_ctx* ctx = an->ctx;
	const size_t n = ctx->n;
	if (bounds[0] != 0 || bounds[nregions] != n) return fail(MG_EINVAL, "mg_anneal_merge_export: regions must cover the input");
	for (uint32_t r = 0; r < nregions; r++) {
		if (bounds[r] >= bounds[r + 1]) return fail(MG_EINVAL, "mg_anneal_merge_export: region %u is empty", r);
		if (owners[r] != MG_NO_OWNER && owners[r] >= an->p.chains)
			return fail(MG_EINVAL, "mg_anneal_merge_export: region %u has no such owner", r);
	}
	CU(cudaSetDevice(ctx->device));
	DevBuf d_bounds, d_owners;
	if (int rc = dev_alloc(d_bounds, (size_t)(nregions + 1) * 4)) return rc;
	if (int rc = dev_alloc(d_owners, (size_t)nregions * 4)) return rc;
	CU(cudaMemcpyAsync(d_bounds.p, bounds, (size_t)(nregions + 1) * 4, cudaMemcpyHostToDevice, ctx->stream));
	CU(cudaMemcpyAsync(d_owners.p, owners, (size_t)nregions * 4, cudaMemcpyHostToDevice, ctx->stream));
	CU(cudaMemsetAsync(dev_slab, 0, n * 8, ctx->stream));
	CU(cudaMemsetAsync(dev_abs, 0, n * 4, ctx->stream));
	region_abs_reps_kernel<<<grid_for(nregions, 128, 1 << 20), 128, 0, ctx->stream>>>(
	    an->d_slabs, (uint32_t)n, d_bounds.as<uint32_t>(), d_owners.as<uint32_t>(), nregions, an->d_ck, an->d_ck_meta, an->d_ck_live,
	    (uint32_t)an->nck, an->nslots > 1 ? 1u : 0u, an->stride, static_cast<uint32_t*>(dev_abs));
	CU(cudaGetLastError());
	merge_regions_kernel<<<grid_for(nregions, 1, ctx->sm_count * 8), 256, 0, ctx->stream>>>(
	    an->d_slabs, (uint32_t)n, d_bounds.as<uint32_t>(), d_owners.as<uint32_t>(), nregions, static_cast<uint64_t*>(dev_slab));
	CU(cudaGetLastError());
	CU(cudaStreamSynchronize(ctx->stream));
	return MG_OK;
}

extern "C" MG_API int mg_anneal_merge_import(mg_anneal* an, const void* dev_slab, const void* dev_abs, uint32_t dst_chain,
                                      uint64_t* cost_out)
{
	if (!an || !dev_slab || !dev_abs || dst_chain >= an->p.chains) return fail(MG_EINVAL, "mg_anneal_merge_import: bad argument");
	mg_ctx* ctx = an->ctx;
	const size_t n = ctx->n;
	CU(cudaSetDevice(ctx->device));
	CU(cudaMemsetAsync(an->d_bad, 0, 4, ctx->stream));
	validate_kernel<<<grid_for(n, 256, ctx->sm_count * 4), 256, 0, ctx->stream>>>(static_cast<const uint64_t*>(dev_slab), ctx->n, an->d_bad);
	CU(cudaGetLastError());
	uint32_t bad = 0;
	CU(cudaMemcpyAsync(&bad, an->d_bad, 4, cudaMemcpyDeviceToHost, ctx->stream));
	CU(cudaMemcpyAsync(an->d_slabs + (size_t)dst_chain * n, dev_slab, n * 8, cudaMemcpyDeviceToDevice, ctx->stream));
	ChainState st;
	CU(cudaStreamSynchronize(ctx->stream));
	if (bad) return fail(MG_ESLAB, "mg_anneal_merge_import: merged slab holds %u undecodable slot(s)", bad);
	CU(cudaMemcpy(&st, an->d_state + dst_chain, sizeof(ChainState), cudaMemcpyDeviceToHost));
	st.susp_slot = 0;
	st.journal_count = 0;
	st.journal_overflow = 1;
	st.err = 0;
	CU(cudaMemcpy(an->d_state + dst_chain, &st, sizeof(ChainState), cudaMemcpyHostToDevice));
	AnnealArgs a;
	anneal_common_args(an, a);
	a.chains = 1;
	a.chain_first = dst_chain;
	a.repair_only = 1;
	a.abs_dist = static_cast<const uint32_t*>(dev_abs);
	a.evals = 1;
	a.max_attempts = 1;
	anneal_kernel<<<1, CTA_THREADS, sizeof(CtaShared), ctx->stream>>>(a);
	CU(cudaGetLastError());
	CU(cudaStreamSynchronize(ctx->stream));
	CU(cudaMemcpy(&st, an->d_state + dst_chain, sizeof(ChainState), cudaMemcpyDeviceToHost));
	if (st.err) return fail(MG_ESLAB, "mg_anneal_merge_import: merged slab: %s", walk_error(st.err));
	an->have_slab[dst_chain] = 1;
	if (cost_out) *cost_out = st.slab_cost;
	return MG_OK;
}

extern "C" MG_API int mg_anneal_merge_regions(mg_anneal* an, uint32_t nregions, const uint32_t* bounds, const uint32_t* owners,
                                       uint32_t dst_chain, uint64_t* cost_out)
{
	if (!an || !bounds || !owners || nregions == 0 || dst_chain >= an->p.chains)
		return fail(MG_EINVAL, "mg_anneal_merge_regions: bad argument");
	for (uint32_t r = 0; r < nregions; r++)
		if (owners[r] == MG_NO_OWNER) return fail(MG_EINVAL, "mg_anneal_merge_regions: region %u has no owner", r);
	CU(cudaSetDevice(an->ctx->device));
	DevBuf slab, abs;
	if (int rc = dev_alloc(slab, (size_t)an->ctx->n * 8)) return rc;
	if (int rc = dev_alloc(abs, (size_t)an->ctx->n * 4)) return rc;
	if (int rc = mg_anneal_merge_export(an, nregions, bounds, owners, slab.p, abs.p)) return rc;
	return mg_anneal_merge_import(an, slab.p, abs.p, dst_chain, cost_out);
}

extern "C" MG_API int mg_anneal_greedy_init(mg_anneal* an, uint32_t nregions, uint32_t dst_chain, uint64_t* cost_out)
{
	if (!an || dst_chain >= an->p.chains) return fail(MG_EINVAL, "mg_anneal_greedy_init: bad argument");
	mg_ctx* ctx = an->ctx;
	const uint32_t n = ctx->n;
	if (nregions == 0) nregions = 1;
	if (nregions > n / 64 + 1) nregions = n / 64 + 1;
	CU(cudaSetDevice(ctx->device));
	std::vector<uint32_t> bounds(nregions + 1);
	for (uint32_t r = 0; r <= nregions; r++) bounds[r] = (uint32_t)((uint64_t)n * r / nregions);
	DevBuf slab, abs, dbounds, derr;
	if (int rc = dev_alloc(slab, (size_t)n * 8)) return rc;
	if (int rc = dev_alloc(abs, (size_t)n * 4)) return rc;
	if (int rc = dev_alloc(dbounds, sizeof(uint32_t) * (nregions + 1))) return rc;
	if (int rc = dev_alloc(derr, 4)) return rc;
	CU(cudaMemcpyAsync(dbounds.p, bounds.data(), sizeof(uint32_t) * (nregions + 1), cudaMemcpyHostToDevice, ctx->stream));
	CU(cudaMemsetAsync(abs.p, 0, (size_t)n * 4, ctx->stream));
	CU(cudaMemsetAsync(derr.p, 0, 4, ctx->stream));
	fill_literal_kernel<<<grid_for(n, 256, ctx->sm_count * 8), 256, 0, ctx->stream>>>(slab.as<uint64_t>(), n);
	CU(cudaGetLastError());
	GreedyArgs g;
	g.data = ctx->d_data;
	g.n = n;
	g.occ_start = ctx->d_occ_start;
	g.occ = ctx->d_occ;
	g.tables = ctx->tables;
	g.limits = ctx->limits;
	g.k = an->p.top_k;
	g.bounds = dbounds.as<uint32_t>();
	g.nregions = nregions;
	g.slab = slab.as<uint64_t>();
	g.abs_dist = abs.as<uint32_t>();
	g.err = derr.as<uint32_t>();
	int blocks = (int)((nregions + WARPS_PER_CTA - 1) / WARPS_PER_CTA);
	if (blocks > ctx->sm_count) blocks = ctx->sm_count;
	greedy_kernel<<<blocks, CTA_THREADS, sizeof(CtaShared), ctx->stream>>>(g);
	CU(cudaGetLastError());
	uint32_t herr = 0;
	CU(cudaMemcpyAsync(&herr, derr.p, 4, cudaMemcpyDeviceToHost, ctx->stream));
	CU(cudaStreamSynchronize(ctx->stream));
	if (herr) return fail(MG_ESLAB, "mg_anneal_greedy_init: %s", walk_error(herr));
	return mg_anneal_merge_import(an, slab.p, abs.p, dst_chain, cost_out);
}

extern "C" MG_API int mg_anneal_optimal_init(mg_anneal* an, uint32_t nregions, uint32_t max_occ, uint32_t dst_chain,
                                             uint64_t* cost_out)
{
	if (!an || dst_chain >= an->p.chains) return fail(MG_EINVAL, "mg_anneal_optimal_init: bad argument");
	mg_ctx* ctx = an->ctx;
	const uint32_t n = ctx->n;
	if (nregions == 0) nregions = 1;
	if (nregions > n / 64 + 1) nregions = n / 64 + 1;
	if (max_occ == 0) max_occ = 64;
	CU(cudaSetDevice(ctx->device));
	std::vector<uint32_t> bounds(nregions + 1);
	for (uint32_t r = 0; r <= nregions; r++) bounds[r] = (uint32_t)((uint64_t)n * r / nregions);
	uint32_t blocks = (uint32_t)ctx->sm_count * 8;
	if (blocks > nregions) blocks = nregions;
	DevBuf slab, abs, dbounds, lists, counts, nodes, dnodes;
	if (int rc = dev_alloc(slab, (size_t)n * 8)) return rc;
	if (int rc = dev_alloc(abs, (size_t)n * 4)) return rc;
	if (int rc = dev_alloc(dbounds, sizeof(uint32_t) * (nregions + 1))) return rc;
	if (int rc = dev_alloc(lists, (size_t)n * OPT_LIST * sizeof(uint2))) return rc;
	if (int rc = dev_alloc(counts, n)) return rc;
	if (int rc = dev_alloc(nodes, (size_t)blocks * (OPT_BLOCK + 1) * 2 * sizeof(uint4))) return rc;
	if (int rc = dev_alloc(dnodes, sizeof(unsigned long long))) return rc;
	CU(cudaMemcpyAsync(dbounds.p, bounds.data(), sizeof(uint32_t) * (nregions + 1), cudaMemcpyHostToDevice, ctx->stream));
	CU(cudaMemsetAsync(abs.p, 0, (size_t)n * 4, ctx->stream));
	CU(cudaMemsetAsync(dnodes.p, 0, sizeof(unsigned long long), ctx->stream));
	fill_literal_kernel<<<grid_for(n, 256, ctx->sm_count * 8), 256, 0, ctx->stream>>>(slab.as<uint64_t>(), n);
	CU(cudaGetLastError());
	MatchListArgs ml;
	ml.data = ctx->d_data;
	ml.n = n;
	ml.occ_start = ctx->d_occ_start;
	ml.occ = ctx->d_occ;
	ml.max_occ = max_occ;
	ml.lists = lists.as<uint2>();
	ml.counts = counts.as<uint8_t>();
	OptimalArgs o;
	o.data = ctx->d_data;
	o.n = n;
	o.trans = ctx->d_trans;
	o.lists = lists.as<uint2>();
	o.counts = counts.as<uint8_t>();
	o.bounds = dbounds.as<uint32_t>();
	o.nregions = nregions;
	o.nodes = nodes.as<uint4>();
	o.slab = slab.as<uint64_t>();
	o.abs_dist = abs.as<uint32_t>();
	o.nodes_relaxed = dnodes.as<unsigned long long>();
	cudaEvent_t t0, t1;
	CU(cudaEventCreate(&t0));
	CU(cudaEventCreate(&t1));
	CU(cudaEventRecord(t0, ctx->stream));
	matchlist_kernel<<<grid_for((size_t)n * 32, 256, ctx->sm_count * 64), 256, 0, ctx->stream>>>(ml);
	optimal_kernel<<<blocks, 32, 0, ctx->stream>>>(o);
	CU(cudaEventRecord(t1, ctx->stream));
	CU(cudaGetLastError());
	unsigned long long relaxed = 0;
	CU(cudaMemcpyAsync(&relaxed, dnodes.p, sizeof(relaxed), cudaMemcpyDeviceToHost, ctx->stream));
	CU(cudaStreamSynchronize(ctx->stream));
	{
		float ms = 0;
		cudaEventElapsedTime(&ms, t0, t1);
		ctx->last_optimal_ms = ms;
		ctx->last_optimal_nodes = relaxed;
		cudaEventDestroy(t0);
		cudaEventDestroy(t1);
	}
	return mg_anneal_merge_import(an, slab.p, abs.p, dst_chain, cost_out);
}

extern "C" MG_API int mg_optimal_stats(const mg_ctx* ctx, double* kernel_ms, uint64_t* nodes)
{
	if (!ctx) return fail(MG_EINVAL, "mg_optimal_stats: null context");
	if (kernel_ms) *kernel_ms = ctx->last_optimal_ms;
	if (nodes) *nodes = ctx->last_optimal_nodes;
	return MG_OK;
}

extern "C" MG_API int mg_anneal_broadcast_chain(mg_anneal* an, uint32_t src_chain)
{
	if (!an || src_chain >= an->p.chains) return fail(MG_EINVAL, "mg_anneal_broadcast_chain: bad argument");
	mg_ctx* ctx = an->ctx;
	CU(cudaSetDevice(ctx->device));
	const size_t n = ctx->n, nck = an->nck;
	const uint32_t C = an->p.chains;
	if (C == 1) return MG_OK;
	if (src_chain != 0) {
		CU(cudaMemcpyAsync(an->d_slabs, an->d_slabs + (size_t)src_chain * n, n * 8, cudaMemcpyDeviceToDevice, ctx->stream));
		if (nck) {
			CU(cudaMemcpyAsync(an->d_ck, an->d_ck + (size_t)src_chain * 2 * nck, 2 * nck * sizeof(Record), cudaMemcpyDeviceToDevice, ctx->stream));
			CU(cudaMemcpyAsync(an->d_ck_meta, an->d_ck_meta + (size_t)src_chain * 2 * nck, 2 * nck * sizeof(CkMeta), cudaMemcpyDeviceToDevice, ctx->stream));
			CU(cudaMemcpyAsync(an->d_ck_live, an->d_ck_live + (size_t)src_chain * nck, nck, cudaMemcpyDeviceToDevice, ctx->stream));
		}
	}
	if (int rc = replicate(ctx, an->d_slabs, an->d_slabs + n, n * 8, n * 8, C - 1)) return rc;
	if (nck) {
		if (int rc = replicate(ctx, an->d_ck, an->d_ck + 2 * nck, 2 * nck * sizeof(Record), 2 * nck * sizeof(Record), C - 1)) return rc;
		if (int rc = replicate(ctx, an->d_ck_meta, an->d_ck_meta + 2 * nck, 2 * nck * sizeof(CkMeta), 2 * nck * sizeof(CkMeta), C - 1)) return rc;
		if (int rc = replicate(ctx, an->d_ck_live, an->d_ck_live + nck, nck, nck, C - 1)) return rc;
	}
	std::vector<ChainState> st(C);
	CU(cudaStreamSynchronize(ctx->stream));
	CU(cudaMemcpy(st.data(), an->d_state, (size_t)C * sizeof(ChainState), cudaMemcpyDeviceToHost));
	const ChainState src = st[src_chain];
	for (uint32_t c = 0; c < C; c++) {
		st[c].cur_cost = src.slab_cost;
		st[c].slab_cost = src.slab_cost;
		st[c].live_count = src.live_count;
		st[c].susp_slot = 0;
		st[c].err = 0;
		st[c].journal_count = 0;
		st[c].journal_overflow = 1;
		an->have_slab[c] = 1;
	}
	CU(cudaMemcpy(an->d_state, st.data(), (size_t)C * sizeof(ChainState), cudaMemcpyHostToDevice));
	return MG_OK;
}

extern "C" MG_API int mg_anneal_oneshot(mg_ctx* ctx, const mg_anneal_params* params, const mg_anneal_run_params* run,
                                 const LZMAPacket* init, LZMAPacket* best_slab_out, uint64_t* best_cost,
                                 mg_anneal_stats* stats)
{
	if (!ctx || !params || !run || !best_slab_out) return fail(MG_EINVAL, "mg_anneal_oneshot: null argument");
	mg_anneal_params p = *params;
	p.track_best = 1;
	mg_anneal* an = nullptr;
	int rc = mg_anneal_create(ctx, &p, &an);
	if (rc) return rc;
	rc = mg_anneal_set_slab(an, 0, p.chains, init, init ? 1 : 0, 1);
	if (!rc) rc = mg_anneal_run(an, run, stats);
	if (!rc) {
		std::vector<uint64_t> best(p.chains);
		rc = mg_anneal_costs(an, nullptr, best.data());
		if (!rc) {
			uint32_t arg = 0;
// ... 16 lines not shown
```

### megalania_b200/csrc/mg_finder.cuh

```cuda
#pragma once
#include "mg_device.cuh"

namespace mg {

constexpr int MAX_K = 32;
struct FindLimits {
	uint32_t window;
	uint32_t max_occ;
};
constexpr uint32_t FIND_GAVE_UP = 0xffffffffu;
constexpr uint32_t MAX_MATCH = 273;
#ifndef MG_FINDER_PM
#define MG_FINDER_PM 1
#endif

struct FindScratch {
	uint64_t ent_pk[MAX_K];
	uint32_t ent_price[MAX_K];
	uint32_t len_price[2][MAX_MATCH - 1];
	uint32_t hkey[MAX_K];
	uint8_t pop_order[MAX_K];
	uint32_t count;
	uint32_t pops;
	uint32_t candidates;
	uint32_t chunks;
};

constexpr uint32_t QUEUE_ROUNDS = 16;
constexpr uint32_t MATCH_DESC_OFFSET = 0;
constexpr uint32_t STAGE_OFFSET = MATCH_DESC_OFFSET + 32 * 16;
constexpr uint32_t STAGE_BYTES = 32 * 8 + 32;
static_assert(STAGE_OFFSET % 16 == 0 && STAGE_OFFSET + STAGE_BYTES <= sizeof(uint32_t) * 2 * (MAX_MATCH - 1), "window mirrors must fit in len_price");

__device__ __forceinline__ uint32_t per_byte(uint32_t cost, uint32_t len, SmemU32 recip)
{
	return len == 1 ? cost : __umulhi(cost, recip.get(len));
}


__device__ __forceinline__ void heap_sink(FindScratch* fs, uint32_t p, uint32_t key, uint32_t count)
{
	const uint32_t price = key >> 5;
	for (;;) {
		const uint32_t l = 2 * p + 1;
		if (l >= count) break;
		const uint32_t kl = fs->hkey[l];
		const uint32_t kr = l + 1 < count ? fs->hkey[l + 1] : 0u;
		uint32_t big = l, kb = kl;
		if ((kr >> 5) > (kl >> 5)) {
			big = l + 1;
			kb = kr;
		}
		if ((kb >> 5) <= price) break;
		fs->hkey[p] = kb;
		p = big;
	}
	fs->hkey[p] = key;
}

__device__ __forceinline__ void heap_rise(FindScratch* fs, uint32_t p, uint32_t key)
{
	const uint32_t price = key >> 5;
	while (p > 0) {
		const uint32_t parent = (p - 1) / 2;
		const uint32_t kp = fs->hkey[parent];
		if (price <= (kp >> 5)) break;
		fs->hkey[p] = kp;
		p = parent;
	}
	fs->hkey[p] = key;
}

__device__ __noinline__ void heap_offer(FindScratch* fs, uint32_t k, uint64_t pk, uint32_t price, uint64_t excluded)
{
	if (pk == excluded) return;
	const uint32_t count = fs->count;
	if (count < k) {
		fs->ent_pk[count] = pk;
		fs->ent_price[count] = price;
		fs->count = count + 1;
		heap_rise(fs, count, (price << 5) | count);
		return;
	}
	const uint32_t top = fs->hkey[0];
	if (price <= (top >> 5)) {
		const uint32_t en = top & 31u;
		fs->ent_pk[en] = pk;
		fs->ent_price[en] = price;
		heap_sink(fs, 0, (price << 5) | en, count);
	}
}

__device__ __forceinline__ uint32_t tree_price(SmemU16 probs, SmemU32 price, uint32_t base,
                                               uint32_t nbits, uint32_t value)
{
	uint32_t c = 0, node = 1;
	for (uint32_t i = nbits; i-- > 0;) {
		uint32_t bit = (value >> i) & 1;
		c += bit_price(probs, price, base + node, bit);
		node = (node << 1) | bit;
	}
	return c;
}

__device__ __forceinline__ uint32_t length_price(SmemU16 probs, SmemU32 price, uint32_t base,
                                                 uint32_t len)
{
	uint32_t v = len - 2;
	if (v < 8) return bit_price(probs, price, base, 0) + tree_price(probs, price, base + LEN_LOW, 3, v);
	uint32_t c = bit_price(probs, price, base, 1);
	if (v < 16) return c + bit_price(probs, price, base + 1, 0) + tree_price(probs, price, base + LEN_MID, 3, v - 8);
	return c + bit_price(probs, price, base + 1, 1) + tree_price(probs, price, base + LEN_HIGH, 8, v - 16);
}

__device__ __forceinline__ uint32_t literal_price(SmemU16 probs, SmemU32 price, uint32_t ctx,
                                                  uint32_t byte, uint32_t mbyte)
{
	uint32_t c = bit_price(probs, price, S_ISMATCH + ctx, 0);
	for (uint32_t d = 0; d < 8; d++) {
		uint32_t slot, bit;
		lit_event(d, byte, ctx >= 7, mbyte, slot, bit);
		c += bit_price(probs, price, slot, bit);
	}
	return c;
}

__device__ __forceinline__ uint32_t dist_tail_price(SmemU16 probs, SmemU32 price, const DistParts& d)
{
	uint32_t c = d.direct << 11, node = 1, v = d.low;
	for (uint32_t i = 0; i < d.rbits; i++) {
		uint32_t bit = v & 1;
		c += bit_price(probs, price, d.rbase + node, bit);
		node = (node << 1) | bit;
		v >>= 1;
	}
	return c;
}

__device__ __forceinline__ uint32_t load_u32_unaligned(const uint8_t* __restrict__ p)
{
	const uintptr_t a = reinterpret_cast<uintptr_t>(p);
	const uint32_t* w = reinterpret_cast<const uint32_t*>(a & ~(uintptr_t)3);
	return __funnelshift_r(w[0], w[1], (uint32_t)(a & 3) * 8);
}

__device__ __noinline__ uint32_t warp_find(int lane, SmemU16 probs, SmemU32 price,
                                           SmemU32 recip, FindScratch* fs, const uint8_t* __restrict__ data,
                                           uint32_t n, const uint32_t* __restrict__ occ_start,
                                           const uint32_t* __restrict__ occ, const Model m, uint64_t excluded,
                                           uint32_t k, long long give_up_at = 0, FindLimits limits = FindLimits{0, 0})
{
	uint32_t candidates = 0, chunks = 0;
	asm volatile("cp.async.wait_group 0;" ::: "memory");
	__syncwarp();
	const uint32_t pos = m.pos, ctx = m.ctx;
	if (lane == 0) {
		fs->count = 0;
		fs->pops = 0;
	}
	const uint32_t p_match = bit_price(probs, price, S_ISMATCH + ctx, 1);
	const uint32_t hdr_match = p_match + bit_price(probs, price, S_ISREP + ctx, 0);
	const uint32_t hdr_rep = p_match + bit_price(probs, price, S_ISREP + ctx, 1);
	const uint32_t g0_0 = bit_price(probs, price, S_ISREPG0 + ctx, 0), g0_1 = bit_price(probs, price, S_ISREPG0 + ctx, 1);
	const uint32_t g1_0 = bit_price(probs, price, S_ISREPG1 + ctx, 0), g1_1 = bit_price(probs, price, S_ISREPG1 + ctx, 1);
	const uint32_t g2_0 = bit_price(probs, price, S_ISREPG2 + ctx, 0), g2_1 = bit_price(probs, price, S_ISREPG2 + ctx, 1);
	const uint32_t r0l_0 = bit_price(probs, price, S_ISREP0LONG + ctx, 0);
	const uint32_t r0l_1 = bit_price(probs, price, S_ISREP0LONG + ctx, 1);
	const uint32_t hdr_lrep0 = hdr_rep + g0_0 + r0l_1;
	const uint32_t hdr_lrep1 = hdr_rep + g0_1 + g1_0;
	const uint32_t hdr_lrep2 = hdr_rep + g0_1 + g1_1 + g2_0;
	const uint32_t hdr_lrep3 = hdr_rep + g0_1 + g1_1 + g2_1;

	const uint32_t byte = data[pos];
	const uint32_t rep_byte = pos > 0 ? data[pos - m.rep0 - 1] : 0;
	__syncwarp();
	if (lane == 0) {
		heap_offer(fs, k, PK_LITERAL, literal_price(probs, price, ctx, byte, rep_byte), excluded);
		if (pos > 0 && byte == rep_byte) heap_offer(fs, k, PK_SHORT_REP, hdr_rep + g0_0 + r0l_0, excluded);
	}
	if (lane == 0) candidates += 1 + (pos > 0 && byte == rep_byte);
	__syncwarp();

	if (pos != 0 && pos != n - 1) {
		const uint32_t key = ((uint32_t)byte << 8) | data[pos + 1];
		uint32_t begin = occ_start[key];
		const uint32_t end = occ_start[key + 1];
		if (limits.window | limits.max_occ) {
			auto first_at_least = [&](uint32_t value) {
				uint32_t lo = begin, hi = end;
				while (lo < hi) {
					const uint32_t mid = lo + (hi - lo) / 2;
					if (occ[mid] < value) lo = mid + 1;
					else hi = mid;
				}
				return lo;
			};
			const uint32_t upper = first_at_least(pos);
			if (limits.window != 0 && pos > limits.window) begin = first_at_least(pos - limits.window);
			if (limits.max_occ != 0 && upper - begin > limits.max_occ) begin = upper - limits.max_occ;
		}
		const uint32_t max_len = n - pos < MAX_MATCH ? n - pos : MAX_MATCH;
		uint32_t have_len[2] = {1, 1};
		uint32_t min_lp[2] = {0xffffffffu, 0xffffffffu};
		uint32_t slot_cached = 0xffffffffu, slot_price2 = 0, slot_price3 = 0, slot_price4 = 0, slot_price5 = 0;
		int32_t pm_prefix = INT32_MAX, pm_short = INT32_MAX;
		int32_t pm_t2 = INT32_MAX, pm_t3 = INT32_MAX, pm_t4 = INT32_MAX;
		uint32_t pm_root = 0xffffffffu, pm_have = 0;
		DistParts ap;
		ap.pslot = 14;
		ap.nlow = 4;
		ap.low = (uint32_t)lane & 15;
		ap.rbase = S_ALIGN;
		ap.rbits = 4;
		ap.direct = 0;
		const uint32_t align_tab = dist_tail_price(probs, price, ap);
		const uint32_t q2 = load_u32_unaligned(data + pos + 2);
		uint32_t o_next = begin + (uint32_t)lane < end ? occ[begin + (uint32_t)lane] : 0xffffffffu;
		uint32_t r2_next = o_next < pos ? load_u32_unaligned(data + o_next + 2) : 0u;
		for (uint32_t chunk = begin; chunk < end; chunk += 32) {
			const uint32_t o = o_next, r2 = r2_next;
			{
				const uint32_t idxn = chunk + 32u + (uint32_t)lane;
				o_next = idxn < end ? occ[idxn] : 0xffffffffu;
				r2_next = o_next < pos ? load_u32_unaligned(data + o_next + 2) : 0u;
			}
			const bool valid = o < pos;
			const uint32_t valid_mask = __ballot_sync(FULL, valid);
			if (valid_mask == 0) break;
			chunks++;
			if (give_up_at != 0 && (chunks & 63u) == 0 && clock64() >= give_up_at) {
				__syncwarp();
				return FIND_GAVE_UP;
			}
			uint32_t L = 0;
			if (valid) {
				const uint32_t x2 = q2 ^ r2;
				if (x2) {
					L = 2 + (((uint32_t)__ffs((int)x2) - 1u) >> 3);
				} else {
					L = 6;
					const uint8_t* q = data + pos;
					const uint8_t* r = data + o;
					while (L < max_len) {
						const uint32_t x = load_u32_unaligned(q + L) ^ load_u32_unaligned(r + L);
						if (x) {
							L += ((uint32_t)__ffs((int)x) - 1u) >> 3;
							break;
						}
						L += 4;
					}
				}
				L = L < max_len ? L : max_len;
			}
			const uint32_t dist = pos - o - 1;
			uint32_t rep_mask = 0;
			if (valid) {
				rep_mask = (dist == m.rep0 ? 1u : 0u) | (dist == m.rep1 ? 2u : 0u) | (dist == m.rep2 ? 4u : 0u) |
				           (dist == m.rep3 ? 8u : 0u);
			}
			const uint32_t need0 = __reduce_max_sync(FULL, L);
			const uint32_t need1 = __reduce_max_sync(FULL, rep_mask ? L : 0u);
			if (need0 > have_len[0]) {
				uint32_t mn = 0xffffffffu;
				for (uint32_t l = have_len[0] + 1 + (uint32_t)lane; l <= need0; l += 32) {
					const uint32_t v = length_price(probs, price, S_LEN, l);
					fs->len_price[0][l - 2] = v;
					mn = min(mn, v);
				}
				min_lp[0] = min(min_lp[0], __reduce_min_sync(FULL, mn));
				have_len[0] = need0;
			}
			if (need1 > have_len[1]) {
				uint32_t mn = 0xffffffffu;
				for (uint32_t l = have_len[1] + 1 + (uint32_t)lane; l <= need1; l += 32) {
					const uint32_t v = length_price(probs, price, S_REPLEN, l);
					fs->len_price[1][l - 2] = v;
					mn = min(mn, v);
				}
				min_lp[1] = min(min_lp[1], __reduce_min_sync(FULL, mn));
				have_len[1] = need1;
			}
			__syncwarp();
			const DistParts dp = dist_parts(valid ? dist : 0);
			const uint32_t align_price = __shfl_sync(FULL, align_tab, (int)(dp.low & 15));
			uint32_t base2 = 0, base3 = 0, base4 = 0, base5 = 0;
			if (valid) {
				uint32_t tail = hdr_match;
				if (dp.pslot >= 14)
					tail += (dp.direct << 11) + align_price;
				else
					tail += dist_tail_price(probs, price, dp);
				if (dp.pslot != slot_cached) {
					slot_cached = dp.pslot;
					slot_price2 = tree_price(probs, price, S_POSSLOT, 6, dp.pslot);
					slot_price3 = tree_price(probs, price, S_POSSLOT + 64, 6, dp.pslot);
					slot_price4 = tree_price(probs, price, S_POSSLOT + 128, 6, dp.pslot);
					slot_price5 = tree_price(probs, price, S_POSSLOT + 192, 6, dp.pslot);
				}
				base2 = tail + slot_price2;
				base3 = tail + slot_price3;
				base4 = tail + slot_price4;
				base5 = tail + slot_price5;
			}
			const uint32_t hdr_r0 = hdr_lrep0, hdr_r1 = hdr_lrep1, hdr_r2 = hdr_lrep2, hdr_r3 = hdr_lrep3;
			const bool full = fs->count >= k;
			const uint32_t root = full ? fs->hkey[0] >> 5 : 0xffffffffu;
			if (MG_FINDER_PM && full && (root != pm_root || have_len[0] != pm_have)) {
				int32_t q = INT32_MIN, s5 = INT32_MIN;
				pm_t2 = pm_t3 = pm_t4 = INT32_MAX;
				if (root < 0x400000u) {
					for (uint32_t j = 0; j < 9; j++) {
						const uint32_t len = 2u + 9u * (uint32_t)lane + j;
						if (len <= have_len[0]) q = max(q, (int32_t)((root + 1u) * len - 1u) - (int32_t)fs->len_price[0][len - 2]);
					}
					if (lane >= 5 && (uint32_t)lane <= have_len[0])
						s5 = (int32_t)((root + 1u) * (uint32_t)lane - 1u) - (int32_t)fs->len_price[0][lane - 2];
					if (have_len[0] >= 2) pm_t2 = (int32_t)((root + 1u) * 2u - 1u) - (int32_t)fs->len_price[0][0];
					if (have_len[0] >= 3) pm_t3 = (int32_t)((root + 1u) * 3u - 1u) - (int32_t)fs->len_price[0][1];
					if (have_len[0] >= 4) pm_t4 = (int32_t)((root + 1u) * 4u - 1u) - (int32_t)fs->len_price[0][2];
				} else {
					q = INT32_MAX;
					s5 = lane >= 5 ? INT32_MAX : INT32_MIN;
				}
				for (int o = 1; o < 32; o <<= 1) {
					const int32_t t = __shfl_up_sync(FULL, q, o);
					const int32_t t5 = __shfl_up_sync(FULL, s5, o);
					if (lane >= o) {
						q = max(q, t);
						s5 = max(s5, t5);
					}
				}
				pm_prefix = q;
				pm_short = s5;
				pm_root = root;
				pm_have = have_len[0];
			}
			const int32_t pm_at = __shfl_sync(FULL, pm_prefix, valid ? (int)((L - 2u) / 9u) : 0);
			const int32_t pm_sh = __shfl_sync(FULL, pm_short, valid && L < 31u ? (int)L : 31);
			uint32_t cheapest = 0xffffffffu;
			uint32_t live_lens = 0;
			uint32_t first_live = 2;
			if (valid) {
				uint32_t rep_hdr_best = 0xffffffffu;
				if (rep_mask & 1) rep_hdr_best = min(rep_hdr_best, hdr_r0);
				if (rep_mask & 2) rep_hdr_best = min(rep_hdr_best, hdr_r1);
				if (rep_mask & 4) rep_hdr_best = min(rep_hdr_best, hdr_r2);
				if (rep_mask & 8) rep_hdr_best = min(rep_hdr_best, hdr_r3);
				uint32_t lo = base2;
				if (L > 2) lo = min(lo, base3);
				if (L > 3) lo = min(lo, base4);
				if (L > 4) lo = min(lo, base5);
				uint32_t bound = per_byte(lo + min_lp[0], L, recip);
				if (rep_mask) bound = min(bound, per_byte(rep_hdr_best + min_lp[1], L, recip));
				if (!full) {
					cheapest = 0;
					live_lens = 0xffffffffu;
				} else if (bound <= root &&
				           (!MG_FINDER_PM || rep_mask != 0 || pm_root != root ||
				            (L > 31u ? (int32_t)lo <= pm_at
				                     : ((int32_t)base2 <= pm_t2 || (L >= 3u && (int32_t)base3 <= pm_t3) || (L >= 4u && (int32_t)base4 <= pm_t4) ||
				                        (L >= 5u && (int32_t)base5 <= pm_sh))))) {
					first_live = 0xffffffffu;
					for (uint32_t len = 2; len <= L; len++) {
						const uint32_t b = len == 2 ? base2 : len == 3 ? base3 : len == 4 ? base4 : base5;
						const uint32_t pm = per_byte(b + fs->len_price[0][len - 2], len, recip);
						uint32_t pr = 0xffffffffu;
						if (rep_mask) pr = per_byte(rep_hdr_best + fs->len_price[1][len - 2], len, recip);
						cheapest = min(cheapest, min(pm, pr));
						if (min(pm, pr) <= root) {
							live_lens |= 1u << ((len - 2) & 31);
							first_live = min(first_live, len);
						}
					}
				}
				candidates += (L - 1) * (1 + __popc(rep_mask));
			}
			uint32_t pass = __ballot_sync(FULL, valid && cheapest <= root);
			const uint32_t ex_type = pk_type(excluded), ex_idx = pk_dist(excluded), ex_len = pk_len(excluded);
			const bool ex_here = valid && ex_len >= 2 && ex_len <= L &&
			                     ((ex_type == T_MATCH && ex_idx == dist) ||
			                      (ex_type == T_LONG_REP && ex_idx < 4 && ((rep_mask >> ex_idx) & 1u)));
			if (full && pass && !__any_sync(FULL, ex_here)) {
				const uint32_t less = __ballot_sync(FULL, valid && cheapest < root);
				if (less == 0) {
					const int who = 31 - __clz((int)pass);
					uint32_t done = 0;
					if (lane == who) {
						uint64_t last = 0;
						for (uint32_t len = 2; len <= L; len++) {
							const uint32_t b = len == 2 ? base2 : len == 3 ? base3 : len == 4 ? base4 : base5;
							if (per_byte(b + fs->len_price[0][len - 2], len, recip) == root && pk_pack(T_MATCH, dist, len) != excluded)
								last = pk_pack(T_MATCH, dist, len);
							if (rep_mask) {
								const uint32_t lp = fs->len_price[1][len - 2];
								if ((rep_mask & 1) && per_byte(hdr_r0 + lp, len, recip) == root && pk_pack(T_LONG_REP, 0, len) != excluded) last = pk_pack(T_LONG_REP, 0, len);
								if ((rep_mask & 2) && per_byte(hdr_r1 + lp, len, recip) == root && pk_pack(T_LONG_REP, 1, len) != excluded) last = pk_pack(T_LONG_REP, 1, len);
								if ((rep_mask & 4) && per_byte(hdr_r2 + lp, len, recip) == root && pk_pack(T_LONG_REP, 2, len) != excluded) last = pk_pack(T_LONG_REP, 2, len);
								if ((rep_mask & 8) && per_byte(hdr_r3 + lp, len, recip) == root && pk_pack(T_LONG_REP, 3, len) != excluded) last = pk_pack(T_LONG_REP, 3, len);
							}
						}
						if (last != 0) {
							fs->ent_pk[fs->hkey[0] & 31u] = last;
							done = 1;
						}
					}
					if (__shfl_sync(FULL, done, who)) pass = 0;
					__syncwarp();
				} else {
					pass &= ~((1u << (__ffs((int)less) - 1)) - 1u);
				}
			}
			while (pass) {
				const int who = __ffs(pass) - 1;
				pass &= pass - 1;
				if (lane == who) {
					uint32_t todo = L <= 33 ? live_lens : 0xffffffffu;
					for (uint32_t len = L <= 33 ? 2u : first_live; len <= L; len++) {
						if (L <= 33) {
							if (todo == 0) break;
							len = 2 + (uint32_t)__ffs((int)todo) - 1;
							todo &= todo - 1;
						}
						const uint32_t b = len == 2 ? base2 : len == 3 ? base3 : len == 4 ? base4 : base5;
						heap_offer(fs, k, pk_pack(T_MATCH, dist, len), per_byte(b + fs->len_price[0][len - 2], len, recip),
						           excluded);
						if (rep_mask) {
							const uint32_t lp = fs->len_price[1][len - 2];
							if (rep_mask & 1) heap_offer(fs, k, pk_pack(T_LONG_REP, 0, len), per_byte(hdr_r0 + lp, len, recip), excluded);
							if (rep_mask & 2) heap_offer(fs, k, pk_pack(T_LONG_REP, 1, len), per_byte(hdr_r1 + lp, len, recip), excluded);
							if (rep_mask & 4) heap_offer(fs, k, pk_pack(T_LONG_REP, 2, len), per_byte(hdr_r2 + lp, len, recip), excluded);
							if (rep_mask & 8) heap_offer(fs, k, pk_pack(T_LONG_REP, 3, len), per_byte(hdr_r3 + lp, len, recip), excluded);
						}
					}
				}
				__syncwarp();
			}
			if (valid_mask != FULL) break;
		}
	}
	__syncwarp();
	candidates = __reduce_add_sync(FULL, candidates);
	if (lane == 0) {
		fs->candidates = candidates;
		fs->chunks = chunks;
		uint32_t pops = 0;
		uint32_t count = fs->count;
		while (count > 0) {
			fs->pop_order[pops++] = (uint8_t)(fs->hkey[0] & 31u);
			count--;
			if (count) heap_sink(fs, 0, fs->hkey[count], count);
		}
		fs->count = 0;
		fs->pops = pops;
	}
	__syncwarp();
	return fs->pops;
}

}
```

### megalania_b200/csrc/mg_kernels.cuh

```cuda
#pragma once
#include "mg_device.cuh"
#include "mg_finder.cuh"

namespace mg {

#ifndef MG_WARPS_PER_CTA
#define MG_WARPS_PER_CTA 26
#endif
constexpr int WARPS_PER_CTA = MG_WARPS_PER_CTA;
constexpr int CTA_THREADS = WARPS_PER_CTA * 32;
constexpr uint32_t RECIP_ENTRIES = 288;
#ifndef MG_WALK_VARIANT
#define MG_WALK_VARIANT 0
#endif

struct ChainStats {
	unsigned long long evals, attempts, accepted, new_best, packets, bits, slab_bytes, ck_bytes, finds, candidates,
	    edits, overflows, rejoined, find_cycles, chain_cycles, chunks, gave_up;
};

struct ChainState {
	uint64_t rng;
	uint64_t cur_cost;
	uint64_t best_cost;
// ... 564 lines not shown
				const uint4 d = lds_v4(e.ev_addr + MATCH_DESC_OFFSET + 16u * (k.pos - k.w.base));
				if (d.x != 0) {
					const uint32_t len = meta_len(meta), dist = d.w, amask = d.z & 0x3ffffffu;
					uint32_t shb, mask2, base, sel;
					asm volatile("ld.shared.v4.u32 {%0, %1, %2, %3}, [%4];"
					             : "=r"(shb), "=r"(mask2), "=r"(base), "=r"(sel)
					             : "r"(e.lane_tab_addr));
					const uint32_t nwb = (d.x >> shb) & mask2;
					const uint32_t slot = base + __byte_perm(d.y | k.ctx, 0, sel) + (nwb >> 1);
					if ((amask >> e.lane) & 1u) code_bit(e.probs, e.trans, slot, nwb & 1u, k.t.acc);
					if (e.lane == 0) k.t.acc += (d.z >> 26) << 11;
					k.t.bits += (uint32_t)__popc(amask) - 9u;
					const uint32_t r0 = e.reps.get(0), r1 = e.reps.get(1), r2 = e.reps.get(2);
					e.reps.set(0, dist);
					e.reps.set(1, r0);
					e.reps.set(2, r1);
					e.reps.set(3, r2);
					__syncwarp();
					k.ctx = k.ctx < 7 ? 7 : 10;
					k.pos += len;
					k.delta += len - 1;
					k.mb = MB_UNKNOWN;
					continue;
				}
			}
			Model m = walker_model(e, k);
			uint32_t type = meta_type(meta), len = meta_len(meta), dist = 0;
			const uint32_t byte = meta_byte(meta) & 0xff;
			if (type == T_MATCH || type == T_LONG_REP) dist = window_dist(k.w, k.pos);
			if (MODE == WALK_REPAIR_HEAD && k.pos == override_pos) {
				type = pk_type(override_pk);
				len = pk_len(override_pk);
				dist = pk_dist(override_pk);
			}
			if (MODE != WALK_PLAIN) {
				const uint64_t old = pk_pack(type, dist, len);
				if (type == T_SHORT_REP || type == T_LITERAL) {
					const uint32_t rep_byte = (m.rep0 < m.pos) ? e.data[m.pos - m.rep0 - 1] : 0x100u;
					if (byte == rep_byte) {
						if (MODE == WALK_REPAIR_HEAD) type = T_SHORT_REP;
					} else {
						type = T_LITERAL;
					}
					dist = 0;
					len = 1;
				} else if (type == T_LONG_REP) {
					if (len < 2 || len > e.n - m.pos || dist > 3) {
						err = ERR_BAD_PACKET;
						return WALK_ERROR;
					}
					bool good = model_rep(m, dist) < m.pos && rep_matches(e.lane, e.data, m.pos, model_rep(m, dist), len);
					for (uint32_t idx = 0; idx < 4 && !good; idx++) {
						dist = idx;
						good = model_rep(m, dist) < m.pos && rep_matches(e.lane, e.data, m.pos, model_rep(m, dist), len);
					}
					if (!good && e.abs_dist) {
						const uint32_t d = e.abs_dist[m.pos] - 1u;
						if (d < m.pos && rep_matches(e.lane, e.data, m.pos, d, len)) {
							type = T_MATCH;
							dist = d;
							good = true;
						}
					}
					if (!good) {
						pending = pk_pack(T_LONG_REP, dist, len);
						pending_old = old;
						return WALK_NEED_FIND;
					}
				}
				const uint64_t now = pk_pack(type, dist, len);
				if (now != old) log_put(e.lane, *lg, m.pos, now);
			}
			if (!packet_ok(m, e.n, type, len, dist)) {
				err = ERR_BAD_PACKET;
				return WALK_ERROR;
			}
			walker_apply(e, k, m, type, len, dist, byte);
			break;
		}
	}
}

__device__ __forceinline__ uint64_t walker_bits(const Walker& k, uint32_t pidx_from)
{
	return (uint64_t)(walker_pidx(k) - pidx_from) * 9 + (int64_t)(int32_t)k.t.bits;
}

struct ScoreArgs {
	const uint8_t* data;
	uint32_t n;
	const uint64_t* slabs;
	uint32_t nslabs;
	uint32_t stop_pos;
	uint64_t* out_cost;
	uint32_t* out_count;
	uint32_t* out_err;
	Record* ck;
	uint32_t* ck_pos;
	CkMeta* ck_meta;
	uint32_t stride, nslots;
	uint32_t ck_chain_stride;
	Record* final_model;
	Tables tables;
};

__global__ void __launch_bounds__(CTA_THREADS) score_kernel(ScoreArgs a)
{
	extern __shared__ __align__(128) unsigned char smem_raw[];
	CtaShared* sh = reinterpret_cast<CtaShared*>(smem_raw);
	cta_tables_load(sh, a.tables);
	const int lane = threadIdx.x & 31, warp = threadIdx.x >> 5;
	const uint32_t s = blockIdx.x * WARPS_PER_CTA + warp;
	if (s >= a.nslabs) return;
	WarpShared* ws = warp_block(sh, warp);
	const WalkEnv e = make_env(lane, ws, sh, a.slabs + (size_t)s * a.n, a.data, a.n, a.tables.litq);
	Walker k;
	walker_init(e, k);
	const size_t ckoff = (size_t)s * a.ck_chain_stride;
	CkSink ck;
	ck.ck = a.ck ? a.ck + ckoff : nullptr;
	ck.ck_pos = a.ck_pos ? a.ck_pos + ckoff : nullptr;
	ck.meta = a.ck_meta ? a.ck_meta + ckoff : nullptr;
	ck.live = nullptr;
	ck.nck = 0;
	ck.stride = a.stride;
	ck.next = a.stride;
	ck.written = 0;
	ck.last_pidx = 0;
	ck.last_cost = 0;
	ck.test = 0;
	ck.converged = 0;
	ck.suspend_pidx = 0xffffffffu;
	ck.deadline = 0;
	uint64_t pending = 0, pending_old = 0;
	uint32_t err = 0;
	if (!a.ck) ck.next = 0xffffffffu;
	walk(WALK_PLAIN, e, k, a.stop_pos, 0xffffffffu, ck, nullptr, 0xffffffffu, 0, pending, pending_old, err);
	tally_flush(k.t);
	asm volatile("cp.async.wait_group 0;" ::: "memory");
	if (!err && k.pos != a.stop_pos) err = ERR_NOT_BOUNDARY;
	if (a.final_model) walker_store(e, k, a.final_model + s);
	if (lane == 0) {
		a.out_cost[s] = k.t.total;
		if (a.out_count) a.out_count[s] = walker_pidx(k);
		a.out_err[s] = err;
	}
}

struct TopkArgs {
	const uint8_t* data;
	uint32_t n;
	const uint32_t* occ_start;
	const uint32_t* occ;
	const uint64_t* slab;
	int state_mode;
	const uint32_t* positions;
	uint32_t npos, k;
	const Record* ck;
	const uint32_t* ck_pos;
	uint32_t nslots, stride;
	uint64_t* out_pk;
	uint32_t* out_price;
	int32_t* out_count;
	uint32_t* out_err;
	unsigned long long* candidates;
	FindLimits limits;
	Tables tables;
};

__global__ void __launch_bounds__(CTA_THREADS) topk_kernel(TopkArgs a)
{
	extern __shared__ __align__(128) unsigned char smem_raw[];
	CtaShared* sh = reinterpret_cast<CtaShared*>(smem_raw);
	cta_tables_load(sh, a.tables);
	const int lane = threadIdx.x & 31, warp = threadIdx.x >> 5;
	WarpShared* ws = warp_block(sh, warp);
	const WalkEnv e = make_env(lane, ws, sh, a.slab, a.data, a.n, a.tables.litq);
	uint32_t parity = 0;
	unsigned long long cand = 0;
	for (uint32_t q = blockIdx.x * WARPS_PER_CTA + warp; q < a.npos; q += gridDim.x * WARPS_PER_CTA) {
		const uint32_t qpos = a.positions[q];
		Walker k;
		uint32_t err = 0;
		if (qpos >= a.n) {
			err = ERR_NOT_BOUNDARY;
		} else if (a.state_mode == 0) {
			walker_init(e, k);
			k.pos = k.delta = qpos;
		} else {
			uint32_t below = 0;
			for (uint32_t j = lane; j + 1 < a.nslots; j += 32) below += a.ck_pos[j] <= qpos ? 1u : 0u;
			below = __reduce_add_sync(FULL, below);
			if (below == 0)
				walker_init(e, k);
			else
				walker_load(e, k, a.ck + (below - 1), &ws->bar, parity);
			CkSink ck = {};
			ck.next = 0xffffffffu;
			ck.suspend_pidx = 0xffffffffu;
			ck.deadline = 0;
			uint64_t pending = 0, pending_old = 0;
			walk(WALK_PLAIN, e, k, qpos, 0xffffffffu, ck, nullptr, 0xffffffffu, 0, pending, pending_old, err);
			if (!err && k.pos != qpos) err = ERR_NOT_BOUNDARY;
		}
		uint32_t pops = 0;
		if (!err) {
			pops = warp_find(lane, e.probs, e.trans, e.recip, &ws->fs, a.data, a.n, a.occ_start, a.occ,
			                 walker_model(e, k), a.slab[qpos], a.k, 0, a.limits);
			cand += ws->fs.candidates;
			for (uint32_t i = lane; i < pops; i += 32) {
				const uint32_t en = ws->fs.pop_order[i];
				a.out_pk[(size_t)q * a.k + i] = ws->fs.ent_pk[en];
				a.out_price[(size_t)q * a.k + i] = ws->fs.ent_price[en];
			}
		}
		if (lane == 0) {
			a.out_count[q] = (int32_t)pops;
			a.out_err[q] = err;
		}
		__syncwarp();
	}
	asm volatile("cp.async.wait_group 0;" ::: "memory");
	if (lane == 0 && cand) atomicAdd(a.candidates, cand);
}

struct GreedyArgs {
	const uint8_t* data;
	uint32_t n;
	const uint32_t* occ_start;
	const uint32_t* occ;
	Tables tables;
	FindLimits limits;
	uint32_t k;
	const uint32_t* bounds;
	uint32_t nregions;
	uint64_t* slab;
	uint32_t* abs_dist;
	uint32_t* err;
};

__global__ void __launch_bounds__(CTA_THREADS) greedy_kernel(GreedyArgs a)
{
	extern __shared__ __align__(128) unsigned char smem_raw[];
	CtaShared* sh = reinterpret_cast<CtaShared*>(smem_raw);
	cta_tables_load(sh, a.tables);
	const int lane = threadIdx.x & 31, warp = threadIdx.x >> 5;
	WarpShared* ws = warp_block(sh, warp);
	const WalkEnv e = make_env(lane, ws, sh, a.slab, a.data, a.n, nullptr);
	for (uint32_t r = (uint32_t)warp * gridDim.x + blockIdx.x; r < a.nregions; r += gridDim.x * WARPS_PER_CTA) {
		const uint32_t lo = a.bounds[r], hi = a.bounds[r + 1];
		Walker k;
		walker_init(e, k);
		k.pos = k.delta = lo;
		while (k.pos < hi) {
			Model m = walker_model(e, k);
			const uint32_t count = warp_find(lane, e.probs, e.trans, e.recip, &ws->fs, a.data, a.n, a.occ_start, a.occ, m, 0, a.k, 0,
			                                 a.limits);
			uint64_t pk = count ? ws->fs.ent_pk[ws->fs.pop_order[count - 1]] : PK_LITERAL;
			__syncwarp();
			uint32_t type = pk_type(pk), len = pk_len(pk), dist = pk_dist(pk);
			if (len > hi - k.pos) {
				if ((type == T_MATCH || type == T_LONG_REP) && hi - k.pos >= 2) {
					len = hi - k.pos;
				} else {
					type = T_LITERAL;
					len = 1;
					dist = 0;
				}
				pk = pk_pack(type, dist, len);
			}
			if (!packet_ok(m, a.n, type, len, dist)) {
				if (lane == 0) atomicOr(a.err, ERR_BAD_PACKET);
				break;
			}
			if (lane == 0) {
				a.slab[k.pos] = pk;
				if (type == T_LONG_REP) a.abs_dist[k.pos] = model_rep(m, dist) + 1u;
			}
			walker_apply(e, k, m, type, len, dist, a.data[k.pos]);
		}
	}
}



struct TraceRec {
	uint64_t cost;
	uint32_t flags;
	uint32_t undo_count;
};

struct AnnealArgs {
	const uint8_t* data;
	uint32_t n;
	const uint32_t* occ_start;
	const uint32_t* occ;
	Tables tables;
	FindLimits limits;
	uint32_t chains, k, stride, nslots, log_cap, track_best;
	uint64_t* slabs;
	uint64_t* bests;
	Record* ck;
	CkMeta* ck_meta;
	uint8_t* ck_live;
	Edit* logs;
	Edit* journal;
	ChainState* state;
	ChainStats* stats;
	TraceRec* trace;
	uint32_t trace_cap;
	uint32_t* attempts_out;
	uint32_t evals, max_attempts, schedule, step, num_iters, first_eval;
	unsigned long long packet_budget;
	unsigned long long cycle_budget;
	uint32_t early_exit;
	const uint32_t* abs_dist;
	const uint32_t* regions;
	uint32_t chain_first;
	uint32_t repair_only;
	uint32_t suspend;
	const float* temps;
};

#ifndef MG_ANNEAL_MIN_CTAS
#define MG_ANNEAL_MIN_CTAS 1
#endif
__global__ void __launch_bounds__(CTA_THREADS, MG_ANNEAL_MIN_CTAS) anneal_kernel(AnnealArgs a)
{
	extern __shared__ __align__(128) unsigned char smem_raw[];
	CtaShared* sh = reinterpret_cast<CtaShared*>(smem_raw);
	cta_tables_load(sh, a.tables);
	const int lane = threadIdx.x & 31, warp = threadIdx.x >> 5;
	if ((uint32_t)warp * gridDim.x + blockIdx.x >= a.chains) return;
	const uint32_t c = a.chain_first + (uint32_t)warp * gridDim.x + blockIdx.x;
	WarpShared* ws = warp_block(sh, warp);
	const uint32_t n = a.n, nck = a.nslots - 1;
	const uint32_t reg_lo = a.regions ? a.regions[2 * c] : 0u, reg_hi = a.regions ? a.regions[2 * c + 1] : 0u;
	uint64_t* slab = a.slabs + (size_t)c * n;
	WalkEnv e_init = make_env(lane, ws, sh, slab, a.data, n, a.tables.litq);
	e_init.abs_dist = a.abs_dist;
	WalkEnv e = e_init;
	Record* ck_base = a.ck + (size_t)c * 2 * nck;
	CkMeta* ck_meta = a.ck_meta + (size_t)c * 2 * nck;
	uint8_t* ck_live = a.ck_live + (size_t)c * nck;
	ChainState st = a.state[c];
	uint64_t rng = a.repair_only ? 0x6D65726765ull : st.rng;
	uint32_t parity = 0;
	ChainStats& cs = ws->stats;
	if (lane == 0) cs = ChainStats{0, 0, 0, 0, 0, 0, 0, 0, 0, 0, 0, 0, 0, 0, 0, 0, 0};
	const long long t_start = clock64();
	unsigned long long packets_done = 0;
	EditLog lg;
	lg.e = a.logs + (size_t)c * a.log_cap;
	lg.cap = a.log_cap;
	const float temp = a.temps ? a.temps[c] : 0.f;

	uint32_t done = 0, attempts = 0;
	const uint32_t first_eval = a.first_eval == 0xffffffffu ? st.eval_index : a.first_eval;
	const long long deadline = a.cycle_budget ? t_start + (long long)a.cycle_budget : 0;
	while (done < a.evals && attempts < a.max_attempts && st.err == 0 &&
	       (a.packet_budget == 0 || packets_done < a.packet_budget) && (deadline == 0 || clock64() < deadline)) {
		attempts++;
		const uint64_t rng_at_start = rng;
		Walker k;
		CkSink ck;
		ck.ck = ck_base;
		ck.ck_pos = nullptr;
		ck.meta = ck_meta;
		ck.live = ck_live;
		ck.nck = nck;
		ck.stride = a.stride;
		ck.written = 0;
		ck.converged = 0;
		uint32_t j0 = 0, target = 0;
		uint32_t phase = 0, mode = WALK_PLAIN;
		const bool resumed = st.susp_slot != 0;
		if (resumed) {
			const uint32_t slot = st.susp_slot;
			j0 = st.susp_j0;
			lg.stored = st.susp_stored;
			lg.count = st.susp_count;
			lg.overflow = st.susp_overflow != 0;
			lg.dup_pos = 0xffffffffu;
			lg.dup_index = 0;
			st.susp_slot = 0;
			walker_load(e, k, ck_base + (size_t)(ck_live[slot - 1] ^ 1u) * nck + (slot - 1), &ws->bar, parity);
			if (lane == 0) cs.ck_bytes += sizeof(Record);
			ck.next = (slot + 1) * a.stride;
			ck.last_pidx = walker_pidx(k);
			ck.last_cost = k.t.total;
			ck.test = a.early_exit;
			phase = 2;
			mode = WALK_REPAIR;
		} else {
			lg.stored = lg.count = 0;
			lg.dup_pos = 0xffffffffu;
			lg.dup_index = 0;
			lg.overflow = false;

			const bool by_pos = a.regions != nullptr;
			if (by_pos)
				target = reg_lo + rng31(rng) % (reg_hi - reg_lo);
			else if (!a.repair_only)
				target = rng31(rng) % st.live_count;
			uint32_t pidx0 = 0;
			uint64_t cost0 = 0;
			if (!a.repair_only) {
				uint32_t carry_p = 0;
				uint64_t carry_c = 0;
				for (uint32_t base = 0; base < nck; base += 32) {
					const uint32_t i = base + lane;
					CkMeta mt = {0, 0, 0};
					if (i < nck) mt = ck_meta[(size_t)ck_live[i] * nck + i];
					uint32_t p = mt.dpidx;
					uint64_t cc = mt.dcost;
					for (int o = 1; o < 32; o <<= 1) {
						const uint32_t tp = __shfl_up_sync(FULL, p, o);
						const uint64_t tc = __shfl_up_sync(FULL, cc, o);
						if (lane >= o) {
							p += tp;
							cc += tc;
						}
					}
					p += carry_p;
					cc += carry_c;
					const uint32_t cnt = __popc(__ballot_sync(FULL, i < nck && (by_pos ? mt.pos : p) <= target));
					if (cnt) {
						j0 = base + cnt;
						pidx0 = __shfl_sync(FULL, p, (int)cnt - 1);
						cost0 = __shfl_sync(FULL, cc, (int)cnt - 1);
					}
					carry_p = __shfl_sync(FULL, p, 31);
					carry_c = __shfl_sync(FULL, cc, 31);
					if (cnt < 32) break;
				}
			}
			if (j0 == 0) {
				walker_init(e, k);
			} else {
				walker_load(e, k, ck_base + (size_t)ck_live[j0 - 1] * nck + (j0 - 1), &ws->bar, parity);
				k.delta = k.pos - pidx0;
				k.t.total = cost0;
				if (lane == 0) cs.ck_bytes += sizeof(Record);
			}
			ck.next = 0xffffffffu;
			ck.last_pidx = pidx0;
			ck.last_cost = cost0;
			ck.test = 0;
			if (a.repair_only) {
				ck.next = a.stride;
				phase = 2;
				mode = WALK_REPAIR;
			}
		}
		const uint32_t start_pos = k.pos, start_pidx = walker_pidx(k);
		ck.suspend_pidx = 0xffffffffu;
		ck.deadline = a.suspend ? deadline : 0;
		if (a.suspend && a.packet_budget) {
			const unsigned long long lim = (unsigned long long)start_pidx + (a.packet_budget - packets_done);
			ck.suspend_pidx = lim < 0xffffffffull ? (uint32_t)lim : 0xffffffffu;
		}
		uint64_t pending = 0, pending_old = 0;
		uint32_t err = 0;

		const bool by_pos = a.regions != nullptr;
		uint32_t stop_pidx = (resumed || by_pos || a.repair_only) ? 0xffffffffu : target;
		uint32_t stop_pos = (by_pos && phase == 0) ? target : n;
		uint32_t pos = 0, byte0 = 0;
		uint64_t first = 0, newpk = 0, override_pk = 0, excluded = 0;
		uint32_t override_pos = 0xffffffffu;
		uint32_t want_find = 0;
		bool pick_best = false, failed = false, suspended = false, gave_up = false;
		for (;;) {
			const uint32_t res = walk(mode, e, k, stop_pos, stop_pidx, ck, &lg, override_pos, override_pk, pending, pending_old, err);
			if (res == WALK_ERROR) {
				st.err = err;
				break;
			}
			if (res == WALK_REJOINED) break;
			if (res == WALK_SUSPENDED) {
				suspended = true;
				break;
			}
			if (res == WALK_NEED_FIND) {
				pick_best = rng31(rng) % 4 == 0;
				excluded = pending;
				want_find = 2;
			} else if (phase == 0) {
				if (by_pos && (k.pos >= n || k.pos >= reg_hi)) {
					failed = true;
					break;
				}
				if (k.pos >= n) {
					st.err = ERR_NOT_BOUNDARY;
					break;
				}
				stop_pos = n;
				pos = k.pos;
				if (pos - k.w.base >= 32u) {
					tally_flush(k.t);
					window_seek(lane, k.w, slab, a.data, n, pos, e.stage_addr);
				}
				const uint32_t meta0 = window_meta(k.w, pos);
				const uint32_t dist0 = window_dist(k.w, pos);
				first = pk_pack(meta_type(meta0), dist0, meta_len(meta0));
				byte0 = meta_byte(meta0) & 0xff;
				want_find = 1;
				excluded = first;
				pick_best = false;
				if (pos + 1 < n && rng31(rng) % 2 == 0) {
					const uint64_t second = slab[pos + 1];
					const uint32_t ft = pk_type(first), flen = pk_len(first);
					const uint32_t stype = pk_type(second), slen = pk_len(second), sdist = pk_dist(second);
					if ((ft == T_LONG_REP || ft == T_MATCH) && flen > 2) {
						newpk = PK_LITERAL;
						override_pos = pos + 1;
						override_pk = pk_pack(ft, pk_dist(first), flen - 1);
						log_put(lane, lg, pos, newpk);
						lg.dup_index = lg.stored;
						log_put(lane, lg, pos + 1, override_pk);
						lg.dup_pos = pos + 1;
						want_find = 0;
					} else if ((ft == T_LITERAL || ft == T_SHORT_REP) && (stype == T_MATCH || stype == T_LONG_REP)) {
						const int64_t src =
						    (int64_t)pos - (int64_t)(stype == T_LONG_REP ? model_rep(walker_model(e, k), sdist & 3) : sdist);
						if (slen < MAX_MATCH && src > 0 && byte0 == a.data[src - 1]) {
							newpk = pk_pack(stype, sdist, slen + 1);
							log_put(lane, lg, pos, newpk);
							want_find = 0;
						}
					}
				}
				ck.next = (j0 + 1) * a.stride;
			} else if (phase == 1) {
				phase = 2;
				mode = WALK_REPAIR;
				stop_pidx = 0xffffffffu;
				ck.test = a.early_exit;
				continue;
			} else {
				break;
			}

			if (want_find) {
				if (lane == 0) cs.finds++;
				const long long t_find = clock64();
				const Model fm = walker_model(e, k);
				struct Parked { Walker k; CkSink ck; EditLog lg; ChainState st; } parked = {k, ck, lg, st};
				asm volatile("" ::"l"(&parked) : "memory");
				const uint32_t count = warp_find(lane, e.probs, e.trans, e.recip, &ws->fs, a.data, n, a.occ_start, a.occ, fm,
				                                 excluded, a.k, (a.suspend && attempts > 1) ? deadline : 0, a.limits);
				asm volatile("" ::"l"(&parked) : "memory");
				k = parked.k;
				ck = parked.ck;
				lg = parked.lg;
				st = parked.st;
				e = make_env(lane, ws, sh, slab, a.data, n, a.tables.litq);
				e.abs_dist = a.abs_dist;
				k.w.md_base = WINDOW_NONE;
				k.w.pf_base = WINDOW_NONE;
				if (count == FIND_GAVE_UP) {
					gave_up = true;
					break;
				}
				if (lane == 0) {
					cs.candidates += ws->fs.candidates;
					cs.chunks += ws->fs.chunks;
					cs.find_cycles += (unsigned long long)(clock64() - t_find);
				}
				uint64_t chosen = 0;
				bool have = false;
				if (count != 0) {
					uint32_t choice = rng31(rng) % count;
					for (int i = 1; i < 8; i++) {
						const uint32_t r = rng31(rng) % count;
						choice = r > choice ? r : choice;
					}
					if (rng31(rng) % 8 == 0 || pick_best) choice = count - 1;
					chosen = ws->fs.ent_pk[ws->fs.pop_order[choice]];
					have = true;
				}
				if (want_find == 1) {
					if (!have) {
						failed = true;
						break;
					}
					newpk = chosen;
					log_put(lane, lg, pos, newpk);
				} else {
					newpk = have ? chosen : pending;
					if (newpk != pending_old) log_put(lane, lg, k.pos, newpk);
				}
				want_find = 0;
			}

			{
				const uint32_t type = pk_type(newpk), len = pk_len(newpk), dist = pk_dist(newpk);
				Model m = walker_model(e, k);
				if (!packet_ok(m, n, type, len, dist)) {
					st.err = ERR_BAD_PACKET;
					break;
				}
				const uint32_t byte = phase == 0 ? byte0 : a.data[k.pos];
				walker_apply(e, k, m, type, len, dist, byte);
			}
			if (phase == 0) {
				phase = 1;
				mode = WALK_REPAIR_HEAD;
				stop_pidx = walker_pidx(k) + 3;
			}
		}
		if (st.err) break;
		tally_flush(k.t);
		packets_done += walker_pidx(k) - start_pidx;
		if (lane == 0) {
			cs.packets += walker_pidx(k) - start_pidx;
			cs.bits += walker_bits(k, start_pidx);
			cs.slab_bytes += (uint64_t)(k.pos - start_pos) * 9;
			cs.ck_bytes += (uint64_t)ck.written * sizeof(Record);
		}
		if (gave_up) {
			rng = rng_at_start;
			attempts--;
			if (lane == 0) cs.gave_up++;
			break;
		}
		if (suspended) {
			st.susp_slot = k.pos / a.stride;
			st.susp_j0 = j0;
			st.susp_stored = lg.stored;
			st.susp_count = lg.count;
			st.susp_overflow = lg.overflow ? 1u : 0u;
			attempts--;
			break;
		}
		if (failed) {
			if (a.trace && attempts <= a.trace_cap && lane == 0) {
				TraceRec r = {0, 0, 0};
				a.trace[(size_t)c * a.trace_cap + attempts - 1] = r;
			}
			continue;
		}
		if (lane == 0) cs.edits += lg.count;
		if (lg.overflow) {
			if (lane == 0) cs.overflows++;
			if (a.trace && attempts <= a.trace_cap && lane == 0) {
				TraceRec r = {0, 0, lg.count};
				a.trace[(size_t)c * a.trace_cap + attempts - 1] = r;
			}
			continue;
		}

		uint64_t cost = k.t.total;
		uint32_t live_new = walker_pidx(k);
		uint32_t flip_end = nck;
		if (ck.converged) {
			uint32_t old_pidx;
			uint64_t old_cost;
			ck_absolute(lane, ck_meta, ck_live, nck, ck.converged, old_pidx, old_cost);
			cost += st.slab_cost - old_cost;
			live_new += st.live_count - old_pidx;
			flip_end = ck.converged;
			if (lane == 0) cs.rejoined++;
		}

		const uint32_t r = rng31(rng);
		bool uphill;
		if (a.schedule == 0) {
			const uint64_t i = (uint64_t)first_eval + done;
			const uint64_t mod = i * i + 1 + (uint64_t)a.step * (uint64_t)a.num_iters / 2;
			const uint64_t x = (uint64_t)r % mod;
			uphill = x * x < (uint64_t)a.num_iters;
		} else {
			const float ex = -__logf(((float)r + 0.5f) * (1.0f / 2147483648.0f));
			uphill = (float)(cost - st.cur_cost) <= temp * ex;
		}
		uint32_t flags = 1;
		if (st.cur_cost == 0 || cost < st.cur_cost || uphill || a.repair_only) {
			flags |= 2;
			st.cur_cost = cost;
			st.slab_cost = cost;
			st.live_count = live_new;
			__syncwarp();
			for (uint32_t i = lane; i < lg.stored; i += 32) slab[lg.e[i].pos] = lg.e[i].pk;
			for (uint32_t j = j0 + lane; j < flip_end; j += 32) ck_live[j] ^= 1;
			__syncwarp();
			if (lane == 0) cs.accepted++;
			Edit* jl = a.track_best ? a.journal + (size_t)c * JOURNAL_CAP : nullptr;
			if (jl && !st.journal_overflow) {
				if (st.journal_count + lg.stored <= JOURNAL_CAP) {
					for (uint32_t i = lane; i < lg.stored; i += 32) jl[st.journal_count + i] = lg.e[i];
					st.journal_count += lg.stored;
				} else {
					st.journal_overflow = 1;
				}
			}
			if (st.best_cost == 0 || cost < st.best_cost) {
				st.best_cost = cost;
				flags |= 4;
				if (lane == 0) cs.new_best++;
				if (jl) {
					uint64_t* best = a.bests + (size_t)c * n;
					__syncwarp();
// ... 599 lines not shown
	}
}

__global__ void __launch_bounds__(256) litq_build_kernel(const uint8_t* __restrict__ data, uint32_t n, uint32_t nwin, uint4* __restrict__ out)
{
	const int lane = threadIdx.x & 31;
	const uint32_t w = (blockIdx.x * blockDim.x + threadIdx.x) >> 5;
	if (w >= nwin) return;
	const uint32_t base = w * 32u;
	const uint32_t b = data[base + (uint32_t)lane];
	const uint32_t spare = 2u * (2u * (uint32_t)lane + 1u);
	uint32_t ent[QUEUE_MAX_ROUNDS];
	uint32_t count = 0;
#pragma unroll
	for (uint32_t i = 0; i < QUEUE_MAX_ROUNDS; i++) ent[i] = spare;
	auto put = [&](uint32_t off, uint32_t section) {
#pragma unroll
		for (uint32_t i = 0; i < QUEUE_MAX_ROUNDS; i++)
			if (i == count) ent[i] = off | (section << 13);
		count++;
	};
	auto emit = [&](uint32_t off, uint32_t members, uint32_t bits) {
		while (members) {
			const uint32_t i0 = (uint32_t)__ffs((int)members) - 1u;
			members &= members - 1;
			const uint32_t b0 = (bits >> i0) & 1u;
			if (members) {
				const uint32_t i1 = (uint32_t)__ffs((int)members) - 1u;
				members &= members - 1;
				put(off, 2u + (b0 << 1) + ((bits >> i1) & 1u));
			} else {
				put(off, b0);
			}
		}
	};
	if (lane == 0) emit(2u * S_ISMATCH, FULL, 0);
	for (uint32_t d = 0; d < 8; d++) {
		const uint32_t prefix = b >> (8 - d);
		const uint32_t slot = S_LIT0 + lit0_slot(d, prefix);
		const uint32_t bits = __ballot_sync(FULL, (b >> (7 - d)) & 1u);
		uint32_t todo = FULL;
		while (todo) {
			const int leader = __ffs((int)todo) - 1;
			const uint32_t s = __shfl_sync(FULL, slot, leader);
			const uint32_t members = __ballot_sync(FULL, slot == s);
			todo &= ~members;
			if ((int)((s >> 1) & 31u) == lane) emit(2u * s, members, bits);
		}
	}
	const uint32_t most = __reduce_max_sync(FULL, count);
	if (lane == 0) {
		if (most > QUEUE_MAX_ROUNDS) ent[0] = QUEUE_UNUSABLE;
		else if (most > QUEUE_ROUNDS) ent[0] |= QUEUE_MORE;
	}
	uint4 lo, hi, ex;
	lo.x = ent[0] | ent[1] << 16;
	lo.y = ent[2] | ent[3] << 16;
	lo.z = ent[4] | ent[5] << 16;
	lo.w = ent[6] | ent[7] << 16;
	hi.x = ent[8] | ent[9] << 16;
	hi.y = ent[10] | ent[11] << 16;
	hi.z = ent[12] | ent[13] << 16;
	hi.w = ent[14] | ent[15] << 16;
	ex.x = ent[16] | ent[17] << 16;
	ex.y = ent[18] | ent[19] << 16;
	ex.z = ent[20] | ent[21] << 16;
	ex.w = ent[22] | ent[23] << 16;
	out[(size_t)w * QUEUE_BLOCKS * 32 + (uint32_t)lane] = lo;
	out[(size_t)w * QUEUE_BLOCKS * 32 + 32 + (uint32_t)lane] = hi;
	out[(size_t)w * QUEUE_BLOCKS * 32 + 64 + (uint32_t)lane] = ex;
	(void)n;
}

constexpr uint32_t INDEX_KEYS = 65536;

__device__ __forceinline__ void index_walk(const uint8_t* __restrict__ data, uint32_t n, uint32_t* row, uint32_t begin,
                                           uint32_t end, const uint32_t* start, uint32_t* occ)
{
	const int lane = threadIdx.x & 31;
	const uint32_t lt = (1u << lane) - 1;
	for (uint32_t base = begin; base < end; base += 32) {
		const uint32_t i = base + lane;
		const bool in = i < end;
		const uint32_t key = in ? ((uint32_t)data[i] << 8 | data[i + 1]) : 0xffffffffu;
		const uint32_t peers = __match_any_sync(FULL, key);
		const uint32_t rank = __popc(peers & lt);
		uint32_t slot = 0;
		if (in && rank == 0) {
			slot = row[key];
			row[key] = slot + __popc(peers);
		}
		slot = __shfl_sync(FULL, slot, __ffs(peers) - 1);
		if (in && occ) occ[start[key] + slot + rank] = i;
		__syncwarp();
	}
	(void)n;
}

__global__ void index_count_kernel(const uint8_t* __restrict__ data, uint32_t n, uint32_t* rows, uint32_t per_warp)
{
	const uint32_t wid = (blockIdx.x * blockDim.x + threadIdx.x) >> 5;
	const uint32_t begin = wid * per_warp;
	const uint32_t total = n - 1;
	if (begin >= total) return;
	const uint32_t end = begin + per_warp < total ? begin + per_warp : total;
	index_walk(data, n, rows + (size_t)wid * INDEX_KEYS, begin, end, nullptr, nullptr);
}

__global__ void index_prefix_kernel(uint32_t* rows, uint32_t nwarps, uint32_t* totals)
{
	const uint32_t key = blockIdx.x * blockDim.x + threadIdx.x;
	if (key >= INDEX_KEYS) return;
	uint32_t run = 0;
	for (uint32_t w = 0; w < nwarps; w++) {
		const uint32_t c = rows[(size_t)w * INDEX_KEYS + key];
		rows[(size_t)w * INDEX_KEYS + key] = run;
		run += c;
	}
	totals[key] = run;
}

__global__ void __launch_bounds__(1024) index_scan_kernel(const uint32_t* totals, uint32_t* start)
{
	__shared__ uint32_t part[1024];
	const uint32_t tid = threadIdx.x;
	uint32_t local[64];
	uint32_t sum = 0;
	for (int i = 0; i < 64; i++) {
		local[i] = sum;
		sum += totals[tid * 64 + i];
	}
	part[tid] = sum;
	__syncthreads();
	for (uint32_t off = 1; off < 1024; off <<= 1) {
		uint32_t v = tid >= off ? part[tid - off] : 0;
		__syncthreads();
		part[tid] += v;
		__syncthreads();
	}
	const uint32_t base = part[tid] - sum;
	for (int i = 0; i < 64; i++) start[tid * 64 + i] = base + local[i];
	if (tid == 1023) start[INDEX_KEYS] = part[1023];
}

__global__ void index_scatter_kernel(const uint8_t* __restrict__ data, uint32_t n, uint32_t* rows, uint32_t per_warp,
                                     const uint32_t* start, uint32_t* occ)
{
	const uint32_t wid = (blockIdx.x * blockDim.x + threadIdx.x) >> 5;
	const uint32_t begin = wid * per_warp;
	const uint32_t total = n - 1;
	if (begin >= total) return;
	const uint32_t end = begin + per_warp < total ? begin + per_warp : total;
	index_walk(data, n, rows + (size_t)wid * INDEX_KEYS, begin, end, start, occ);
}

constexpr uint32_t DS_LIT = 0, DS_LEN = 768, DS_REPLEN = DS_LEN + 514, DS_POSSLOT = DS_REPLEN + 514;
constexpr uint32_t DS_ALIGN = DS_POSSLOT + 256, DS_POSCODER = DS_ALIGN + 16, DS_ISMATCH = DS_POSCODER + 115;
constexpr uint32_t DS_ISREP = DS_ISMATCH + 192, DS_ISREPG0 = DS_ISREP + 12, DS_ISREPG1 = DS_ISREPG0 + 12;
constexpr uint32_t DS_ISREPG2 = DS_ISREPG1 + 12, DS_ISREP0LONG = DS_ISREPG2 + 12, DS_TOTAL = DS_ISREP0LONG + 192;
constexpr uint32_t DL_CHOICE2 = 1, DL_LOW = 2, DL_MID = 2 + 128, DL_HIGH = 2 + 256;
static_assert(DS_TOTAL == 2615, "the decoder's model is the reference's");

enum : uint32_t {
	DEC_OK = 0,
	DEC_FIRST_BYTE = 1,
	DEC_LITERAL = 2,
	DEC_SOURCE = 3,
	DEC_PAST_END = 4,
	DEC_COPY = 5,
	DEC_MARKER = 6,
	DEC_SHORT = 7,
	DEC_TRAILING = 8,
	DEC_CODE = 9
};

struct DecodeStatus {
	uint32_t err;
	uint32_t pos;
	unsigned long long events;
	unsigned long long consumed;
};

struct DecodeArgs {
	const uint8_t* data;
	uint32_t n;
	const uint8_t* stream;
	unsigned long long len;
	uint32_t known_size;
	uint64_t* slab;
	DecodeStatus* status;
};

constexpr uint32_t DEC_BUF = 16384;
constexpr uint32_t DEC_MARGIN = 256;

struct RangeDecoder {
	uint16_t* probs;
	const uint8_t* buf;
	unsigned long long base, at, len;
	uint32_t range, code;
	uint32_t short_read;
	unsigned long long events;
};

__device__ __forceinline__ void rd_shift(RangeDecoder& d)
{
	d.range <<= 8;
	uint32_t b = 0;
	if (d.at < d.len && d.at - d.base < DEC_BUF) b = d.buf[d.at++ - d.base];
	else d.short_read = 1;
	d.code = (d.code << 8) | b;
}

__device__ __forceinline__ uint32_t rd_bit(RangeDecoder& d, uint32_t slot)
{
	uint32_t v = d.probs[slot];
	const uint32_t bound = (d.range >> 11) * v;
	uint32_t bit;
	if (d.code < bound) {
		d.range = bound;
		v += (2048u - v) >> 5;
		bit = 0;
	} else {
		d.code -= bound;
		d.range -= bound;
		v -= v >> 5;
		bit = 1;
	}
	d.probs[slot] = (uint16_t)v;
	d.events++;
	if ((d.range & 0xFF000000u) == 0) rd_shift(d);
	return bit;
}

__device__ __forceinline__ uint32_t rd_direct(RangeDecoder& d, uint32_t nbits)
{
	uint32_t value = 0;
	d.events++;
	while (nbits--) {
		d.range >>= 1;
		const uint32_t bit = d.code >= d.range ? 1u : 0u;
		if (bit) d.code -= d.range;
		value = (value << 1) | bit;
		if ((d.range & 0xFF000000u) == 0) rd_shift(d);
	}
	return value;
}

__device__ __forceinline__ uint32_t rd_tree(RangeDecoder& d, uint32_t base, uint32_t nbits)
{
	uint32_t node = 1;
	for (uint32_t i = 0; i < nbits; i++) node = (node << 1) | rd_bit(d, base + node);
	return node - (1u << nbits);
}

__device__ __forceinline__ uint32_t rd_tree_rev(RangeDecoder& d, uint32_t base, uint32_t nbits)
{
	uint32_t node = 1, value = 0;
	for (uint32_t i = 0; i < nbits; i++) {
		const uint32_t bit = rd_bit(d, base + node);
		node = (node << 1) | bit;
		value |= bit << i;
	}
	return value;
}

__device__ __forceinline__ uint32_t rd_length(RangeDecoder& d, uint32_t base)
{
	if (!rd_bit(d, base)) return 2 + rd_tree(d, base + DL_LOW, 3);
	if (!rd_bit(d, base + DL_CHOICE2)) return 10 + rd_tree(d, base + DL_MID, 3);
	return 18 + rd_tree(d, base + DL_HIGH, 8);
}

__device__ __forceinline__ uint32_t rd_distance(RangeDecoder& d, uint32_t len)
{
	const uint32_t lctx = len - 2 < 3 ? len - 2 : 3;
	const uint32_t pslot = rd_tree(d, DS_POSSLOT + lctx * 64, 6);
	if (pslot < 4) return pslot;
	const uint32_t nlow = (pslot >> 1) - 1;
	const uint32_t dist = (2u | (pslot & 1u)) << nlow;
	if (pslot < 14) return dist + rd_tree_rev(d, DS_POSCODER + dist - pslot, nlow);
	const uint32_t mid = rd_direct(d, nlow - 4) << 4;
	return dist + mid + rd_tree_rev(d, DS_ALIGN, 4);
}

__global__ void __launch_bounds__(32) decode_kernel(DecodeArgs a)
{
	__shared__ uint16_t probs[DS_TOTAL];
	__shared__ __align__(16) uint8_t buf[DEC_BUF];
	const uint32_t lane = threadIdx.x;
	for (uint32_t i = lane; i < DS_TOTAL; i += 32) probs[i] = 1024;
	RangeDecoder d;
	d.probs = probs;
	d.buf = buf;
	d.base = 0;
	d.at = 0;
	d.len = a.len;
	d.range = 0xFFFFFFFFu;
	d.code = 0;
	d.short_read = 0;
	d.events = 0;
	const unsigned long long first = a.len < DEC_BUF ? a.len : DEC_BUF;
	for (uint32_t i = lane; i < first; i += 32) buf[i] = a.stream[i];
	__syncwarp();
	uint32_t err = DEC_OK, pos = 0;
	uint32_t ctx = 0, rep0 = 0, rep1 = 0, rep2 = 0, rep3 = 0;
// ... 511 lines not shown
```

Before: 125,400.

## Add byte-run index to walk and bound-skip repeated-byte match candidates in finder

Builds a per-byte index of consecutive occurrence runs (positions inside runs of the same repeated byte) at context creation. When the match finder's key is a doubled byte and the bucket is much larger than the run count, it walks runs instead of individual occurrences. Whole runs whose best possible price cannot beat the current heap root are skipped using bounded distance-slot and length prices. This cuts candidate scanning on highly repetitive data, at the cost of extra index memory, a host-side run count check, and a more complex finder loop.

```diff
diff --git a/include/megalania_cuda.h b/include/megalania_cuda.h
--- a/include/megalania_cuda.h
+++ b/include/megalania_cuda.h
@@ -210,6 +210,7 @@
 } mg_model_dump;
 MG_API int mg_debug_model_after_prefix(mg_ctx* ctx, const LZMAPacket* slab, size_t stop, mg_model_dump* out);
 MG_API int mg_debug_index(mg_ctx* ctx, uint32_t* occ_start, uint32_t* occ);
+MG_API int mg_debug_runs(mg_ctx* ctx, uint32_t* run_start, uint32_t* runs, size_t cap, size_t* count);
 
 #ifdef __cplusplus
 }
diff --git a/megalania_b200/api.py b/megalania_b200/api.py
--- a/megalania_b200/api.py
+++ b/megalania_b200/api.py
@@ -69,7 +69,7 @@
     "mg_anneal_get_slab", "mg_anneal_get_trace", "mg_anneal_swap_chains", "mg_anneal_device_slab",
     "mg_anneal_refresh_chain", "mg_anneal_oneshot", "mg_debug_model_after_prefix", "mg_anneal_export_slab",
     "mg_anneal_import_slab", "mg_anneal_merge_regions", "mg_anneal_broadcast_chain", "mg_find_topk_stats",
-    "mg_anneal_merge_export", "mg_anneal_merge_import", "mg_debug_index", "mg_encode_stats", "mg_ctx_full_wave", "mg_ctx_sm_clock_khz",
+    "mg_anneal_merge_export", "mg_anneal_merge_import", "mg_debug_index", "mg_debug_runs", "mg_encode_stats", "mg_ctx_full_wave", "mg_ctx_sm_clock_khz",
     "mg_comm_unique_id", "mg_comm_init", "mg_comm_destroy", "mg_comm_rank", "mg_comm_size", "mg_comm_exchange_best",
     "mg_comm_temper_exchange", "mg_temper_decide", "mg_comm_merge_regions", "mg_comm_stats", "mg_pool_trim",
     "mg_comm_broadcast_chain", "mg_comm_allgather_u64", "mg_ctx_set_finder_limits", "mg_anneal_greedy_init",
@@ -136,6 +136,7 @@
                                     C.POINTER(u64), C.POINTER(AnnealStats)]
     L.mg_debug_model_after_prefix.argtypes = [vp, vp, sz, vp]
     L.mg_debug_index.argtypes = [vp, vp, vp]
+    L.mg_debug_runs.argtypes = [vp, vp, vp, sz, C.POINTER(sz)]
     L.mg_pool_trim.restype = None
     L.mg_comm_unique_id.argtypes = [vp]
     L.mg_comm_init.argtypes = [vp, i32, i32, vp]
@@ -330,6 +331,15 @@
         _check(self._lib.mg_debug_index(self._h, start.ctypes.data_as(C.c_void_p), occ.ctypes.data_as(C.c_void_p)))
         return start, occ[:max(0, self.n - 1)]
 
+    def run_index(self):
+        start = np.zeros(257, dtype=np.uint32)
+        cap = self.n // 2 + 256
+        runs = np.zeros((cap, 4), dtype=np.uint32)
+        count = C.c_size_t(0)
+        _check(self._lib.mg_debug_runs(self._h, start.ctypes.data_as(C.c_void_p), runs.ctypes.data_as(C.c_void_p), cap,
+                                       C.byref(count)))
+        return start, runs[:count.value]
+
     def chain_bytes(self, **params) -> int:
         p = AnnealParams(**params)
         return int(self._lib.mg_anneal_chain_bytes(self._h, C.byref(p)))
diff --git a/megalania_b200/csrc/mg_api.cu b/megalania_b200/csrc/mg_api.cu
--- a/megalania_b200/csrc/mg_api.cu
+++ b/megalania_b200/csrc/mg_api.cu
@@ -115,7 +115,7 @@
 	cudaSetDevice(device);
 }
 
-extern "C" MG_API uint32_t mg_version(void) { return (0u << 16) | 3u; }
+extern "C" MG_API uint32_t mg_version(void) { return (0u << 16) | 4u; }
 
 struct mg_comm_state;
 
@@ -127,12 +127,15 @@
 	uint8_t* d_data = nullptr;
 	uint32_t* d_occ_start = nullptr;
 	uint32_t* d_occ = nullptr;
+	uint32_t* d_run_start = nullptr;
+	uint4* d_runs = nullptr;
 	uint32_t* d_trans = nullptr;
 	uint32_t* d_recip = nullptr;
 	uint4* d_litq = nullptr;
 	Tables tables{};
 	int sm_count = 0;
 	double index_ms = 0;
+	uint32_t expected_runs = 0;
 	std::vector<mg_anneal*> annealers;
 	double last_topk_ms = 0;
 	unsigned long long last_topk_candidates = 0;
@@ -183,8 +186,11 @@
 	const uint32_t n = ctx->n;
 	CU(pool_malloc(&ctx->d_occ_start, sizeof(uint32_t) * (INDEX_KEYS + 1)));
 	CU(pool_malloc(&ctx->d_occ, sizeof(uint32_t) * (size_t)(n ? n : 1)));
+	CU(pool_malloc(&ctx->d_run_start, sizeof(uint32_t) * 257));
+	CU(pool_malloc(&ctx->d_runs, sizeof(uint4) * ((size_t)n / 2 + 256)));
 	if (n < 2) {
 		CU(cudaMemsetAsync(ctx->d_occ_start, 0, sizeof(uint32_t) * (INDEX_KEYS + 1), ctx->stream));
+		CU(cudaMemsetAsync(ctx->d_run_start, 0, sizeof(uint32_t) * 257, ctx->stream));
 		return 0;
 	}
 	const uint32_t total = n - 1;
@@ -208,9 +214,17 @@
 	index_scan_kernel<<<1, 1024, 0, ctx->stream>>>(totals.as<uint32_t>(), ctx->d_occ_start);
 	index_scatter_kernel<<<blocks, threads, 0, ctx->stream>>>(ctx->d_data, n, rows.as<uint32_t>(), per_warp,
 	                                                          ctx->d_occ_start, ctx->d_occ);
+	run_index_kernel<<<32, 256, 0, ctx->stream>>>(ctx->d_occ_start, ctx->d_occ, 0, totals.as<uint32_t>(), ctx->d_run_start,
+	                                             ctx->d_runs);
+	run_index_kernel<<<32, 256, 0, ctx->stream>>>(ctx->d_occ_start, ctx->d_occ, 1, totals.as<uint32_t>(), ctx->d_run_start,
+	                                             ctx->d_runs);
 	CU(cudaEventRecord(e1, ctx->stream));
-	CU(cudaStreamSynchronize(ctx->stream));
-	CU(cudaGetLastError());
+	uint32_t got_runs = 0;
+	CU(cudaMemcpyAsync(&got_runs, ctx->d_run_start + 256, sizeof(uint32_t), cudaMemcpyDeviceToHost, ctx->stream));
+	CU(cudaStreamSynchronize(ctx->stream));
+	CU(cudaGetLastError());
+	if (got_runs != ctx->expected_runs)
+		return fail(MG_ECUDA, "mg_ctx_create: the device found %u byte runs, %u expected", got_runs, ctx->expected_runs);
 	float ms = 0;
 	cudaEventElapsedTime(&ms, e0, e1);
 	ctx->index_ms = ms;
@@ -241,6 +255,7 @@
 	if (!ctx) return fail(MG_ENOMEM, "out of host memory");
 	ctx->device = device;
 	ctx->n = (uint32_t)n;
+	for (size_t i = 1; i < n; i++) ctx->expected_runs += data[i] == data[i - 1] && (i == 1 || data[i - 2] != data[i]);
 	cudaDeviceProp prop;
 	CU(cudaGetDeviceProperties(&prop, device));
 	ctx->sm_count = prop.multiProcessorCount;
@@ -313,6 +328,8 @@
 	pool_free(ctx->d_data);
 	pool_free(ctx->d_occ_start);
 	pool_free(ctx->d_occ);
+	pool_free(ctx->d_run_start);
+	pool_free(ctx->d_runs);
 	pool_free(ctx->d_trans);
 	pool_free(ctx->d_recip);
 	pool_free(ctx->d_litq);
@@ -357,6 +374,19 @@
 	CU(cudaSetDevice(ctx->device));
 	CU(cudaMemcpyAsync(occ_start, ctx->d_occ_start, sizeof(uint32_t) * (INDEX_KEYS + 1), cudaMemcpyDeviceToHost, ctx->stream));
 	if (ctx->n > 1) CU(cudaMemcpyAsync(occ, ctx->d_occ, sizeof(uint32_t) * (size_t)(ctx->n - 1), cudaMemcpyDeviceToHost, ctx->stream));
+	CU(cudaStreamSynchronize(ctx->stream));
+	return MG_OK;
+}
+
+extern "C" MG_API int mg_debug_runs(mg_ctx* ctx, uint32_t* run_start, uint32_t* runs, size_t cap, size_t* count)
+{
+	if (!ctx || !run_start || !count || (cap && !runs)) return fail(MG_EINVAL, "mg_debug_runs: null argument");
+	CU(cudaSetDevice(ctx->device));
+	CU(cudaMemcpyAsync(run_start, ctx->d_run_start, sizeof(uint32_t) * 257, cudaMemcpyDeviceToHost, ctx->stream));
+	CU(cudaStreamSynchronize(ctx->stream));
+	*count = run_start[256];
+	const size_t take = *count < cap ? *count : cap;
+	if (take) CU(cudaMemcpyAsync(runs, ctx->d_runs, sizeof(uint4) * take, cudaMemcpyDeviceToHost, ctx->stream));
 	CU(cudaStreamSynchronize(ctx->stream));
 	return MG_OK;
 }
@@ -564,6 +594,7 @@
 	a.n = n;
 	a.occ_start = ctx->d_occ_start;
 	a.occ = ctx->d_occ;
+	a.runs = RunIndex{ctx->d_run_start, ctx->d_runs};
 	a.slab = packed.as<uint64_t>();
 	a.state_mode = state_mode;
 	a.positions = dpos.as<uint32_t>();
@@ -1095,6 +1126,7 @@
 	a.n = ctx->n;
 	a.occ_start = ctx->d_occ_start;
 	a.occ = ctx->d_occ;
+	a.runs = RunIndex{ctx->d_run_start, ctx->d_runs};
 	a.tables = ctx->tables;
 	a.limits = ctx->limits;
 	a.chains = C;
@@ -1434,6 +1466,7 @@
 	g.n = n;
 	g.occ_start = ctx->d_occ_start;
 	g.occ = ctx->d_occ;
+	g.runs = RunIndex{ctx->d_run_start, ctx->d_runs};
 	g.tables = ctx->tables;
 	g.limits = ctx->limits;
 	g.k = an->p.top_k;
diff --git a/megalania_b200/csrc/mg_finder.cuh b/megalania_b200/csrc/mg_finder.cuh
--- a/megalania_b200/csrc/mg_finder.cuh
+++ b/megalania_b200/csrc/mg_finder.cuh
@@ -8,6 +8,12 @@
 	uint32_t window;
 	uint32_t max_occ;
 };
+struct RunIndex {
+	const uint32_t* start;
+	const uint4* runs;
+};
+constexpr uint32_t RUN_WALK_MIN_OCC = 4;
+constexpr uint32_t RUN_SKIP_MIN_DIST = 128;
 constexpr uint32_t FIND_GAVE_UP = 0xffffffffu;
 constexpr uint32_t MAX_MATCH = 273;
 #ifndef MG_FINDER_PM
@@ -147,7 +153,7 @@
 __device__ __noinline__ uint32_t warp_find(int lane, SmemU16 probs, SmemU32 price,
                                            SmemU32 recip, FindScratch* fs, const uint8_t* __restrict__ data,
                                            uint32_t n, const uint32_t* __restrict__ occ_start,
-                                           const uint32_t* __restrict__ occ, const Model m, uint64_t excluded,
+                                           const uint32_t* __restrict__ occ, const RunIndex runs, const Model m, uint64_t excluded,
                                            uint32_t k, long long give_up_at = 0, FindLimits limits = FindLimits{0, 0})
 {
 	uint32_t candidates = 0, chunks = 0;
@@ -183,23 +189,50 @@
 
 	if (pos != 0 && pos != n - 1) {
 		const uint32_t key = ((uint32_t)byte << 8) | data[pos + 1];
-		uint32_t begin = occ_start[key];
+		const uint32_t bucket = occ_start[key];
+		uint32_t begin = bucket;
 		const uint32_t end = occ_start[key + 1];
+		auto first_at_least = [&](uint32_t value) {
+			uint32_t lo = begin, hi = end;
+			while (lo < hi) {
+				const uint32_t mid = lo + (hi - lo) / 2;
+				if (occ[mid] < value) lo = mid + 1;
+				else hi = mid;
+			}
+			return lo;
+		};
+		uint32_t upper = end;
 		if (limits.window | limits.max_occ) {
-			auto first_at_least = [&](uint32_t value) {
-				uint32_t lo = begin, hi = end;
-				while (lo < hi) {
-					const uint32_t mid = lo + (hi - lo) / 2;
-					if (occ[mid] < value) lo = mid + 1;
-					else hi = mid;
-				}
-				return lo;
-			};
-			const uint32_t upper = first_at_least(pos);
+			upper = first_at_least(pos);
 			if (limits.window != 0 && pos > limits.window) begin = first_at_least(pos - limits.window);
 			if (limits.max_occ != 0 && upper - begin > limits.max_occ) begin = upper - limits.max_occ;
 		}
 		const uint32_t max_len = n - pos < MAX_MATCH ? n - pos : MAX_MATCH;
+		uint32_t r_next = 0, r_end = 0, run_r = 0, hi = end;
+		bool use_runs = false;
+		if (data[pos + 1] == byte) {
+			const uint32_t rb0 = runs.start[byte], re0 = runs.start[byte + 1];
+			use_runs = end - bucket >= RUN_WALK_MIN_OCC * (re0 - rb0);
+			if (use_runs) {
+				if (!(limits.window | limits.max_occ)) upper = first_at_least(pos);
+				auto first_run_after = [&](uint32_t lo, uint32_t value) {
+					uint32_t h = re0;
+					while (lo < h) {
+						const uint32_t mid = lo + (h - lo) / 2;
+						if (runs.runs[mid].x <= value) lo = mid + 1;
+						else h = mid;
+					}
+					return lo;
+				};
+				const uint32_t after_begin = first_run_after(rb0, begin);
+				r_next = after_begin > rb0 ? after_begin - 1 : rb0;
+				const uint32_t rp = first_run_after(r_next, upper) - 1;
+				r_end = runs.runs[rp].x == upper ? rp : rp + 1;
+				const uint32_t R = runs.runs[rp].z - pos;
+				run_r = R < max_len ? R : max_len;
+				hi = begin;
+			}
+		}
 		uint32_t have_len[2] = {1, 1};
 		uint32_t min_lp[2] = {0xffffffffu, 0xffffffffu};
 		uint32_t slot_cached = 0xffffffffu, slot_price2 = 0, slot_price3 = 0, slot_price4 = 0, slot_price5 = 0;
@@ -214,14 +247,164 @@
 		ap.rbits = 4;
 		ap.direct = 0;
 		const uint32_t align_tab = dist_tail_price(probs, price, ap);
+		auto extend_match_lengths = [&](uint32_t need) {
+			if (need > have_len[0]) {
+				uint32_t mn = 0xffffffffu;
+				for (uint32_t l = have_len[0] + 1 + (uint32_t)lane; l <= need; l += 32) {
+					const uint32_t v = length_price(probs, price, S_LEN, l);
+					fs->len_price[0][l - 2] = v;
+					mn = min(mn, v);
+				}
+				min_lp[0] = min(min_lp[0], __reduce_min_sync(FULL, mn));
+				have_len[0] = need;
+			}
+		};
+		auto refresh_pm = [&](bool full, uint32_t root) {
+			if (MG_FINDER_PM && full && (root != pm_root || have_len[0] != pm_have)) {
+				int32_t q = INT32_MIN, s5 = INT32_MIN;
+				pm_t2 = pm_t3 = pm_t4 = INT32_MAX;
+				if (root < 0x400000u) {
+					for (uint32_t j = 0; j < 9; j++) {
+						const uint32_t len = 2u + 9u * (uint32_t)lane + j;
+						if (len <= have_len[0]) q = max(q, (int32_t)((root + 1u) * len - 1u) - (int32_t)fs->len_price[0][len - 2]);
+					}
+					if (lane >= 5 && (uint32_t)lane <= have_len[0])
+						s5 = (int32_t)((root + 1u) * (uint32_t)lane - 1u) - (int32_t)fs->len_price[0][lane - 2];
+					if (have_len[0] >= 2) pm_t2 = (int32_t)((root + 1u) * 2u - 1u) - (int32_t)fs->len_price[0][0];
+					if (have_len[0] >= 3) pm_t3 = (int32_t)((root + 1u) * 3u - 1u) - (int32_t)fs->len_price[0][1];
+					if (have_len[0] >= 4) pm_t4 = (int32_t)((root + 1u) * 4u - 1u) - (int32_t)fs->len_price[0][2];
+				} else {
+					q = INT32_MAX;
+					s5 = lane >= 5 ? INT32_MAX : INT32_MIN;
+				}
+				for (int o = 1; o < 32; o <<= 1) {
+					const int32_t t = __shfl_up_sync(FULL, q, o);
+					const int32_t t5 = __shfl_up_sync(FULL, s5, o);
+					if (lane >= o) {
+						q = max(q, t);
+						s5 = max(s5, t5);
+					}
+				}
+				pm_prefix = q;
+				pm_short = s5;
+				pm_root = root;
+				pm_have = have_len[0];
+			}
+		};
+		auto may_reach = [&](bool ask, uint32_t L, uint32_t b2, uint32_t b3, uint32_t b4, uint32_t b5, uint32_t root) {
+			const int32_t at = __shfl_sync(FULL, pm_prefix, ask ? (int)((L - 2u) / 9u) : 0);
+			const int32_t sh = __shfl_sync(FULL, pm_short, ask && L < 31u ? (int)L : 31);
+			if (!ask || pm_root != root) return true;
+			if (L > 31u) return (int32_t)min(min(b2, b3), min(b4, b5)) <= at;
+			return (int32_t)b2 <= pm_t2 || (L >= 3u && (int32_t)b3 <= pm_t3) || (L >= 4u && (int32_t)b4 <= pm_t4) ||
+			       (L >= 5u && (int32_t)b5 <= sh);
+		};
 		const uint32_t q2 = load_u32_unaligned(data + pos + 2);
-		uint32_t o_next = begin + (uint32_t)lane < end ? occ[begin + (uint32_t)lane] : 0xffffffffu;
+		uint32_t lo = begin;
+		uint32_t keep = 0;
+		uint32_t run_i0 = 0, run_i1 = 0;
+		uint32_t o_next = lo + (uint32_t)lane < hi ? occ[lo + (uint32_t)lane] : 0xffffffffu;
 		uint32_t r2_next = o_next < pos ? load_u32_unaligned(data + o_next + 2) : 0u;
-		for (uint32_t chunk = begin; chunk < end; chunk += 32) {
+		for (;;) {
+			if (lo >= hi) {
+				if (!use_runs) break;
+				if (keep == 0) {
+					if (r_next >= r_end) break;
+					chunks++;
+					if (give_up_at != 0 && (chunks & 63u) == 0 && clock64() >= give_up_at) {
+						__syncwarp();
+						return FIND_GAVE_UP;
+					}
+					const uint32_t j = r_next + (uint32_t)lane;
+					const uint4 run = j < r_end ? runs.runs[j] : make_uint4(0u, 0u, 0u, 0u);
+					r_next += 32;
+					run_i0 = max(run.x, begin);
+					run_i1 = min(run.x + (run.z - run.y - 1u), upper);
+					const bool some = j < r_end && run_i0 < run_i1;
+					const uint32_t o_lo = run.y + (run_i0 - run.x), o_hi = run.y + (run_i1 - 1u - run.x);
+					const uint32_t dlo = pos - o_hi - 1u, dhi = pos - o_lo - 1u;
+					const bool full = fs->count >= k;
+					const uint32_t root = full ? fs->hkey[0] >> 5 : 0xffffffffu;
+					const bool cand = MG_FINDER_PM && some && full && dlo >= RUN_SKIP_MIN_DIST &&
+					                  !(m.rep0 >= dlo && m.rep0 <= dhi) && !(m.rep1 >= dlo && m.rep1 <= dhi) &&
+					                  !(m.rep2 >= dlo && m.rep2 <= dhi) && !(m.rep3 >= dlo && m.rep3 <= dhi);
+					const uint32_t lmax = min(run_r, run.z - o_lo);
+					const uint32_t ostar = run.z - run_r;
+					const bool star = cand && run.z >= run_r && ostar >= o_lo && ostar <= o_hi;
+					uint32_t Lstar = run_r;
+					if (star) {
+						while (Lstar < max_len) {
+							const uint32_t x = load_u32_unaligned(data + pos + Lstar) ^ load_u32_unaligned(data + ostar + Lstar);
+							if (x) {
+								Lstar += ((uint32_t)__ffs((int)x) - 1u) >> 3;
+								break;
+							}
+							Lstar += 4;
+						}
+						Lstar = min(Lstar, max_len);
+					}
+					extend_match_lengths(__reduce_max_sync(FULL, cand ? max(lmax, star ? Lstar : 0u) : 0u));
+					__syncwarp();
+					refresh_pm(full, root);
+					uint32_t s2 = 0xffffffffu, s3 = 0xffffffffu, s4 = 0xffffffffu, s5 = 0xffffffffu;
+					uint32_t classes = 0;
+					if (cand) {
+						const uint32_t slot_hi = dist_parts(dhi).pslot;
+						for (uint32_t slot = dist_parts(dlo).pslot; slot <= slot_hi; slot++) {
+							const uint32_t direct = ((slot >> 1) - 5u) << 11;
+							s2 = min(s2, tree_price(probs, price, S_POSSLOT, 6, slot) + direct);
+							s3 = min(s3, tree_price(probs, price, S_POSSLOT + 64, 6, slot) + direct);
+							s4 = min(s4, tree_price(probs, price, S_POSSLOT + 128, 6, slot) + direct);
+							s5 = min(s5, tree_price(probs, price, S_POSSLOT + 192, 6, slot) + direct);
+						}
+						classes = dhi - dlo >= 15u ? 0xffffu : (((1u << (dhi - dlo + 1u)) - 1u) << (dlo & 15u));
+						classes = (classes | (classes >> 16)) & 0xffffu;
+					}
+					uint32_t amin = 0xffffffffu;
+					for (int c = 0; c < 16; c++) {
+						const uint32_t v = __shfl_sync(FULL, align_tab, c);
+						if ((classes >> c) & 1u) amin = min(amin, v);
+					}
+					const uint32_t hb = hdr_match + (cand ? amin : 0u);
+					const bool reach = may_reach(cand, lmax, hb + s2, hb + s3, hb + s4, hb + s5, root);
+					const DistParts dps = dist_parts(star ? pos - ostar - 1u : 0u);
+					const uint32_t star_align = __shfl_sync(FULL, align_tab, (int)(dps.low & 15u));
+					uint32_t t2 = 0, t3 = 0, t4 = 0, t5 = 0;
+					if (star) {
+						const uint32_t tail = hdr_match + (dps.direct << 11) + star_align;
+						t2 = tail + tree_price(probs, price, S_POSSLOT, 6, dps.pslot);
+						t3 = tail + tree_price(probs, price, S_POSSLOT + 64, 6, dps.pslot);
+						t4 = tail + tree_price(probs, price, S_POSSLOT + 128, 6, dps.pslot);
+						t5 = tail + tree_price(probs, price, S_POSSLOT + 192, 6, dps.pslot);
+					}
+					const bool star_reach = may_reach(star, Lstar, t2, t3, t4, t5, root);
+					const bool skip = cand && !reach && !(star && star_reach);
+					if (skip) {
+						const uint32_t a = run.z - o_hi, z = run.z - o_lo;
+						uint32_t sum;
+						if (z <= run_r) sum = (a + z) * (z - a + 1u) / 2u;
+						else if (a > run_r) sum = run_r * (z - a + 1u);
+						else sum = (a + run_r) * (run_r - a + 1u) / 2u + run_r * (z - run_r);
+						candidates += sum - (z - a + 1u) + (star ? Lstar - run_r : 0u);
+					}
+					keep = __ballot_sync(FULL, some && !skip);
+					if (keep == 0) continue;
+				}
+				const int first = __ffs((int)keep) - 1;
+				const uint32_t gap = ~keep & ~((1u << first) - 1u);
+				const int last = gap ? __ffs((int)gap) - 2 : 31;
+				lo = __shfl_sync(FULL, run_i0, first);
+				hi = __shfl_sync(FULL, run_i1, last);
+				keep = last == 31 ? 0u : keep & ~((2u << last) - 1u);
+				o_next = lo + (uint32_t)lane < hi ? occ[lo + (uint32_t)lane] : 0xffffffffu;
+				r2_next = o_next < pos ? load_u32_unaligned(data + o_next + 2) : 0u;
+			}
+			const uint32_t chunk = lo;
+			lo += 32;
 			const uint32_t o = o_next, r2 = r2_next;
 			{
 				const uint32_t idxn = chunk + 32u + (uint32_t)lane;
-				o_next = idxn < end ? occ[idxn] : 0xffffffffu;
+				o_next = idxn < hi ? occ[idxn] : 0xffffffffu;
 				r2_next = o_next < pos ? load_u32_unaligned(data + o_next + 2) : 0u;
 			}
 			const bool valid = o < pos;
@@ -258,18 +441,8 @@
 				rep_mask = (dist == m.rep0 ? 1u : 0u) | (dist == m.rep1 ? 2u : 0u) | (dist == m.rep2 ? 4u : 0u) |
 				           (dist == m.rep3 ? 8u : 0u);
 			}
-			const uint32_t need0 = __reduce_max_sync(FULL, L);
+			extend_match_lengths(__reduce_max_sync(FULL, L));
 			const uint32_t need1 = __reduce_max_sync(FULL, rep_mask ? L : 0u);
-			if (need0 > have_len[0]) {
-				uint32_t mn = 0xffffffffu;
-				for (uint32_t l = have_len[0] + 1 + (uint32_t)lane; l <= need0; l += 32) {
-					const uint32_t v = length_price(probs, price, S_LEN, l);
-					fs->len_price[0][l - 2] = v;
-					mn = min(mn, v);
-				}
-				min_lp[0] = min(min_lp[0], __reduce_min_sync(FULL, mn));
-				have_len[0] = need0;
-			}
 			if (need1 > have_len[1]) {
 				uint32_t mn = 0xffffffffu;
 				for (uint32_t l = have_len[1] + 1 + (uint32_t)lane; l <= need1; l += 32) {
@@ -305,36 +478,7 @@
 			const uint32_t hdr_r0 = hdr_lrep0, hdr_r1 = hdr_lrep1, hdr_r2 = hdr_lrep2, hdr_r3 = hdr_lrep3;
 			const bool full = fs->count >= k;
 			const uint32_t root = full ? fs->hkey[0] >> 5 : 0xffffffffu;
-			if (MG_FINDER_PM && full && (root != pm_root || have_len[0] != pm_have)) {
-				int32_t q = INT32_MIN, s5 = INT32_MIN;
-				pm_t2 = pm_t3 = pm_t4 = INT32_MAX;
-				if (root < 0x400000u) {
-					for (uint32_t j = 0; j < 9; j++) {
-						const uint32_t len = 2u + 9u * (uint32_t)lane + j;
-						if (len <= have_len[0]) q = max(q, (int32_t)((root + 1u) * len - 1u) - (int32_t)fs->len_price[0][len - 2]);
-					}
-					if (lane >= 5 && (uint32_t)lane <= have_len[0])
-						s5 = (int32_t)((root + 1u) * (uint32_t)lane - 1u) - (int32_t)fs->len_price[0][lane - 2];
-					if (have_len[0] >= 2) pm_t2 = (int32_t)((root + 1u) * 2u - 1u) - (int32_t)fs->len_price[0][0];
-					if (have_len[0] >= 3) pm_t3 = (int32_t)((root + 1u) * 3u - 1u) - (int32_t)fs->len_price[0][1];
-					if (have_len[0] >= 4) pm_t4 = (int32_t)((root + 1u) * 4u - 1u) - (int32_t)fs->len_price[0][2];
-				} else {
-					q = INT32_MAX;
-					s5 = lane >= 5 ? INT32_MAX : INT32_MIN;
-				}
-				for (int o = 1; o < 32; o <<= 1) {
-					const int32_t t = __shfl_up_sync(FULL, q, o);
-					const int32_t t5 = __shfl_up_sync(FULL, s5, o);
-					if (lane >= o) {
-						q = max(q, t);
-						s5 = max(s5, t5);
-					}
-				}
-				pm_prefix = q;
-				pm_short = s5;
-				pm_root = root;
-				pm_have = have_len[0];
-			}
+			refresh_pm(full, root);
 			const int32_t pm_at = __shfl_sync(FULL, pm_prefix, valid ? (int)((L - 2u) / 9u) : 0);
 			const int32_t pm_sh = __shfl_sync(FULL, pm_short, valid && L < 31u ? (int)L : 31);
 			uint32_t cheapest = 0xffffffffu;
@@ -435,7 +579,7 @@
 				}
 				__syncwarp();
 			}
-			if (valid_mask != FULL) break;
+			if (valid_mask != FULL && !use_runs) break;
 		}
 	}
 	__syncwarp();
diff --git a/megalania_b200/csrc/mg_kernels.cuh b/megalania_b200/csrc/mg_kernels.cuh
--- a/megalania_b200/csrc/mg_kernels.cuh
+++ b/megalania_b200/csrc/mg_kernels.cuh
@@ -740,6 +740,7 @@
 	uint32_t n;
 	const uint32_t* occ_start;
 	const uint32_t* occ;
+	RunIndex runs;
 	const uint64_t* slab;
 	int state_mode;
 	const uint32_t* positions;
@@ -793,7 +794,7 @@
 		}
 		uint32_t pops = 0;
 		if (!err) {
-			pops = warp_find(lane, e.probs, e.trans, e.recip, &ws->fs, a.data, a.n, a.occ_start, a.occ,
+			pops = warp_find(lane, e.probs, e.trans, e.recip, &ws->fs, a.data, a.n, a.occ_start, a.occ, a.runs,
 			                 walker_model(e, k), a.slab[qpos], a.k, 0, a.limits);
 			cand += ws->fs.candidates;
 			for (uint32_t i = lane; i < pops; i += 32) {
@@ -817,6 +818,7 @@
 	uint32_t n;
 	const uint32_t* occ_start;
 	const uint32_t* occ;
+	RunIndex runs;
 	Tables tables;
 	FindLimits limits;
 	uint32_t k;
@@ -842,7 +844,7 @@
 		k.pos = k.delta = lo;
 		while (k.pos < hi) {
 			Model m = walker_model(e, k);
-			const uint32_t count = warp_find(lane, e.probs, e.trans, e.recip, &ws->fs, a.data, a.n, a.occ_start, a.occ, m, 0, a.k, 0,
+			const uint32_t count = warp_find(lane, e.probs, e.trans, e.recip, &ws->fs, a.data, a.n, a.occ_start, a.occ, a.runs, m, 0, a.k, 0,
 			                                 a.limits);
 			uint64_t pk = count ? ws->fs.ent_pk[ws->fs.pop_order[count - 1]] : PK_LITERAL;
 			__syncwarp();
@@ -883,6 +885,7 @@
 	uint32_t n;
 	const uint32_t* occ_start;
 	const uint32_t* occ;
+	RunIndex runs;
 	Tables tables;
 	FindLimits limits;
 	uint32_t chains, k, stride, nslots, log_cap, track_best;
@@ -1136,7 +1139,7 @@
 				const Model fm = walker_model(e, k);
 				struct Parked { Walker k; CkSink ck; EditLog lg; ChainState st; } parked = {k, ck, lg, st};
 				asm volatile("" ::"l"(&parked) : "memory");
-				const uint32_t count = warp_find(lane, e.probs, e.trans, e.recip, &ws->fs, a.data, n, a.occ_start, a.occ, fm,
+				const uint32_t count = warp_find(lane, e.probs, e.trans, e.recip, &ws->fs, a.data, n, a.occ_start, a.occ, a.runs, fm,
 				                                 excluded, a.k, (a.suspend && attempts > 1) ? deadline : 0, a.limits);
 				asm volatile("" ::"l"(&parked) : "memory");
 				k = parked.k;
@@ -2042,6 +2045,41 @@
 	if (begin >= total) return;
 	const uint32_t end = begin + per_warp < total ? begin + per_warp : total;
 	index_walk(data, n, rows + (size_t)wid * INDEX_KEYS, begin, end, start, occ);
+}
+
+__global__ void run_index_kernel(const uint32_t* __restrict__ occ_start, const uint32_t* __restrict__ occ, int pass,
+                                 uint32_t* count, uint32_t* start, uint4* runs)
+{
+	const uint32_t b = (blockIdx.x * blockDim.x + threadIdx.x) >> 5, lane = threadIdx.x & 31;
+	if (b >= 256) return;
+	const uint32_t key = b * 257u, lo = occ_start[key], hi = occ_start[key + 1];
+	uint32_t base = 0;
+	if (pass == 1) {
+		for (uint32_t i = lane; i < b; i += 32) base += count[i];
+		base = __reduce_add_sync(FULL, base);
+		if (lane == 0) start[b] = base;
+		if (b == 255 && lane == 0) start[256] = base + count[255];
+	}
+	uint32_t seen = 0;
+	for (uint32_t i0 = lo; i0 < hi; i0 += 32) {
+		const uint32_t i = i0 + lane;
+		const bool in = i < hi;
+		const uint32_t o = in ? occ[i] : 0u;
+		const bool head = in && (i == lo || occ[i - 1] + 1u != o);
+		const bool tail = in && (i + 1u == hi || occ[i + 1] != o + 1u);
+		const uint32_t heads = __ballot_sync(FULL, head);
+		if (pass == 1) {
+			const uint32_t r = base + seen + __popc(heads & ((2u << lane) - 1u)) - 1u;
+			if (head) {
+				runs[r].x = i;
+				runs[r].y = o;
+				runs[r].w = 0;
+			}
+			if (tail) runs[r].z = o + 2u;
+		}
+		seen += __popc(heads);
+	}
+	if (pass == 0 && lane == 0) count[b] = seen;
 }
 
 constexpr uint32_t DS_LIT = 0, DS_LEN = 768, DS_REPLEN = DS_LEN + 514, DS_POSSLOT = DS_REPLEN + 514;
```

After: 142,300, median of 6. 1.13x the previous value.
